# Yubo-Shankui/Bind-Your-Avatar-Implementation

Measured on AMD Instinct MI355X. Metric: denoise-steps/sec, higher is better.
Workload: dtype bf16; 1 GPU; BASELINE.json configs[1]: full transformer.forward, 49x480x720 (13x30x45 latent tokens + 226 text), 2 characters (2 ID + 2 audio), batch 1, random-init 8.6B-param architecture; layers=42, batch=1, launch=eager, parallelism=single GPU

## Files before the change

### bind_your_avatar_implementation_amd/_hip.py

```python
import ctypes
import os

from .build import LIB_PATH as _BUILT_LIB

LIB_PATH = os.environ.get("BYA_HIP_LIB") or _BUILT_LIB

_c = ctypes
_vp, _i32, _i64, _f32 = _c.c_void_p, _c.c_int32, _c.c_int64, _c.c_float


class GemmDesc(_c.Structure):
    _fields_ = [("M", _i32), ("N", _i32), ("K", _i32), ("batch", _i32),
                ("lda", _i32), ("ldw", _i32), ("ldc", _i32), ("ldres", _i32),
                ("a_batch_stride", _i64), ("c_batch_stride", _i64), ("res_batch_stride", _i64),
                ("gate_batch_stride", _i64), ("gate_split", _i32), ("act", _i32),
                ("n_split", _i32), ("c_split_stride", _i64), ("bias_rowscale", _vp), ("alpha", _f32)]


class GemmPlan(_c.Structure):
    _fields_ = [("path", _i32), ("m0", _i32), ("tail", _i32), ("split_k", _i32), ("row_chunks", _i32)]


class QkNormDesc(_c.Structure):
    _fields_ = [("qw", _vp), ("qb", _vp), ("kw", _vp), ("kb", _vp), ("cos", _vp), ("sin", _vp),
                ("text_rows", _i32), ("width", _i32), ("eps", _f32), ("k_scale", _f32)]


MX_KERNEL_FP6 = 16


class MxGemmCall(_c.Structure):
    _fields_ = [("A", _vp), ("a_scales", _vp), ("W", _vp), ("w_scales", _vp), ("bias", _vp), ("C", _vp),
                ("res", _vp), ("gate0", _vp), ("gate1", _vp), ("q_scales", _vp), ("norm", _c.POINTER(QkNormDesc)),
                ("a_fmt", _i32), ("w_fmt", _i32), ("out_fmt", _i32), ("kernel", _i32)]


class AttnDesc(_c.Structure):
    _fields_ = [("head_dim", _i32), ("heads", _i32), ("nb1", _i32), ("nb2", _i32), ("Sq", _i32), ("Skv", _i32),
                ("q_s1", _i64), ("q_s2", _i64), ("q_row", _i64),
                ("k_s1", _i64), ("k_s2", _i64), ("k_row", _i64),
                ("v_s1", _i64), ("v_s2", _i64), ("v_row", _i64),
                ("o_s1", _i64), ("o_s2", _i64), ("o_row", _i64),
                ("scale", _f32), ("scores_prescaled", _i32), ("score_bound", _f32),
                ("bound_dev", _vp), ("bound_slots", _i32), ("bound_heads", _i32), ("bound_bh0", _i32), ("fallback_flags", _vp)]


class AttnMixDesc(_c.Structure):
    _fields_ = [("head_dim", _i32), ("heads", _i32), ("n_id", _i32), ("n_grp", _i32), ("Sq", _i32), ("Skv", _i32),
                ("q_grp", _i64), ("q_row", _i64), ("k_id", _i64), ("k_grp", _i64), ("k_row", _i64),
                ("v_id", _i64), ("v_grp", _i64), ("v_row", _i64), ("z_grp", _i64), ("z_row", _i64), ("scale", _f32)]


class AttnPlan(_c.Structure):
    _fields_ = [("variant", _i32), ("grid", _i32), ("q_tile", _i32), ("stream_k", _i32), ("sk_rem", _i32), ("sk_cut", _i32),
                ("o_wide", _i32), ("second_launch", _i32)]


class AttnMixPlan(_c.Structure):
    _fields_ = [("form", _i32), ("head_dim", _i32), ("grid", _i32), ("row_chunks", _i32), ("lds_bytes", _i32), ("big_lds", _i32)]


class AttnTinyPlan(_c.Structure):
    _fields_ = [("instance", _i32), ("grid", _i32), ("waves", _i64)]


class RowGemmPlan(_c.Structure):
    _fields_ = [("form", _i32), ("ln", _i32), ("res", _i32), ("act", _i32), ("grid", _i32), ("crosses_row_block", _i32),
                ("work_items", _i64)]


class GroupAttnPlan(_c.Structure):
    _fields_ = [("P", _i32), ("G", _i32), ("wide", _i32), ("blocks", _i32), ("tiles", _i64)]


class LayerNormPlan(_c.Structure):
    _fields_ = [("kernel", _i32), ("vec", _i32), ("nv", _i32), ("modulated", _i32), ("rows_per_wave", _i32), ("grid", _i32),
                ("waves", _i64)]


class QkNormRopePlan(_c.Structure):
    _fields_ = [("stats", _i32), ("only", _i32), ("grid", _i32), ("slots", _i32), ("pairs", _i64), ("waves", _i64)]


class RouterChainPlan(_c.Structure):
    _fields_ = [("tiles", _i32), ("tp0", _i32), ("grid", _i32), ("passes", _i32), ("tiles_last", _i32), ("wgs_last", _i32)]


class StepPlan(_c.Structure):
    _fields_ = [("kernel", _i32), ("grid", _i32), ("rounds", _i32), ("reserved", _i32), ("items", _i64), ("items_per_round", _i64)]


class SchedCoef(_c.Structure):
    _fields_ = [("guidance", _f32), ("sqrt_alpha", _f32), ("sqrt_beta", _f32), ("k_sample", _f32),
                ("k_denoised", _f32), ("k_noise", _f32), ("k_cur", _f32), ("k_old", _f32)]


SIGNATURES = {
    "bya_abi_version": [],
    "bya_set_option": [_i32, _i32],
    "bya_get_option": [_i32, _c.POINTER(_i32)],
    "bya_mfma_calibration": [_vp, _i64, _vp, _i32, _vp],
    "bya_gemm_bf16": [_vp, _vp, _vp, _vp, _vp, _vp, _vp, _c.POINTER(GemmDesc), _vp],
    "bya_gemm_skinny_bf16": [_vp, _vp, _vp, _vp, _vp, _c.POINTER(GemmDesc), _vp],
    "bya_gemm_qkv_norm_rope": [_vp, _vp, _vp, _vp, _c.POINTER(GemmDesc), _c.POINTER(QkNormDesc), _vp],
    "bya_gemm_bf16_plan": [_vp, _vp, _vp, _vp, _vp, _vp, _vp, _c.POINTER(GemmDesc), _c.POINTER(GemmPlan)],
    "bya_gemm_qkv_norm_rope_plan": [_vp, _vp, _vp, _vp, _c.POINTER(GemmDesc), _c.POINTER(QkNormDesc), _c.POINTER(GemmPlan)],
    "bya_set_gemm_workspace": [_vp, _i64],
    "bya_gemm_workspace_bytes": [_c.POINTER(_i64)],
    "bya_gemm_workspace_status": [_c.POINTER(_i32), _vp],
    "bya_quantize_rows_fp8": [_vp, _vp, _vp, _i32, _i32, _i64, _i64, _vp],
    "bya_gemm_fp8": [_vp, _vp, _vp, _vp, _vp, _vp, _vp, _vp, _vp, _c.POINTER(GemmDesc), _vp],
    "bya_gemm_fp8_plan": [_vp, _vp, _vp, _vp, _vp, _vp, _vp, _vp, _vp, _c.POINTER(GemmDesc), _c.POINTER(GemmPlan)],
    "bya_gemm_fp8_qkv_norm_rope": [_vp, _vp, _vp, _vp, _vp, _vp, _c.POINTER(GemmDesc), _c.POINTER(QkNormDesc), _vp],
    "bya_gemm_fp8_qkv_norm_rope_plan": [_vp, _vp, _vp, _vp, _vp, _vp, _c.POINTER(GemmDesc), _c.POINTER(QkNormDesc),
                                        _c.POINTER(GemmPlan)],
    "bya_layernorm_fp8": [_vp, _vp, _vp, _vp, _vp, _vp, _vp, _vp, _vp, _i64, _i32, _i32, _i64, _i64, _i64, _i64, _i64, _i64,
                          _f32, _vp],
    "bya_quantize_mx": [_vp, _vp, _vp, _i32, _i32, _i64, _i32, _vp],
    "bya_layernorm_mx": [_vp, _vp, _vp, _vp, _vp, _vp, _vp, _vp, _vp, _i64, _i32, _i32, _i64, _i64, _i64, _i64, _i64, _i64,
                         _f32, _i32, _vp],
    "bya_gemm_mx": [_vp, _vp, _vp, _vp, _vp, _vp, _vp, _vp, _vp, _c.POINTER(GemmDesc), _i32, _vp],
    "bya_gemm_mx_plan": [_vp, _vp, _vp, _vp, _vp, _vp, _vp, _vp, _vp, _c.POINTER(GemmDesc), _i32, _c.POINTER(GemmPlan)],
    "bya_gemm_mx_mixed": [_vp, _vp, _vp, _vp, _vp, _vp, _vp, _vp, _vp, _c.POINTER(GemmDesc), _i32, _i32, _vp],
    "bya_gemm_mx_mixed_plan": [_vp, _vp, _vp, _vp, _vp, _vp, _vp, _vp, _vp, _c.POINTER(GemmDesc), _i32, _i32,
                               _c.POINTER(GemmPlan)],
    "bya_gemm_mx_quant": [_vp, _vp, _vp, _vp, _vp, _vp, _vp, _c.POINTER(GemmDesc), _i32, _i32, _i32, _vp],
    "bya_gemm_mx_quant_plan": [_vp, _vp, _vp, _vp, _vp, _vp, _vp, _c.POINTER(GemmDesc), _i32, _i32, _i32,
                               _c.POINTER(GemmPlan)],
    "bya_gemm_mx_qkv_norm_rope": [_vp, _vp, _vp, _vp, _vp, _vp, _i32, _i32, _c.POINTER(GemmDesc), _c.POINTER(QkNormDesc), _vp],
    "bya_gemm_mx_qkv_norm_rope_plan": [_vp, _vp, _vp, _vp, _vp, _vp, _i32, _i32, _c.POINTER(GemmDesc), _c.POINTER(QkNormDesc),
                                       _c.POINTER(GemmPlan)],
    "bya_gemm_mx_qkv_norm_rope_on": [_vp, _vp, _vp, _vp, _vp, _vp, _i32, _i32, _c.POINTER(GemmDesc), _c.POINTER(QkNormDesc), _i32,
                                     _vp],
    "bya_gemm_mx_qkv_norm_rope_on_plan": [_vp, _vp, _vp, _vp, _vp, _vp, _i32, _i32, _c.POINTER(GemmDesc), _c.POINTER(QkNormDesc),
                                          _i32, _c.POINTER(GemmPlan)],
    "bya_gemm_mx_call": [_c.POINTER(MxGemmCall), _c.POINTER(GemmDesc), _vp],
    "bya_gemm_mx_call_plan": [_c.POINTER(MxGemmCall), _c.POINTER(GemmDesc), _c.POINTER(GemmPlan)],
    "bya_linear_small_m": [_vp, _vp, _vp, _vp, _i32, _i32, _i32, _i32, _i32, _vp],
    "bya_linear_small_m_plan": [_vp, _vp, _vp, _i32, _i32, _i32, _i32, _c.POINTER(StepPlan)],
    "bya_timestep_features": [_vp, _vp, _i32, _i32, _i32, _f32, _vp],
    "bya_layernorm": [_vp, _vp, _vp, _vp, _vp, _vp, _vp, _vp, _i64, _i32, _i32, _i64, _i64, _i64, _i64, _i64, _i64,
                      _f32, _vp],
    "bya_layernorm_plan": [_vp, _vp, _vp, _vp, _vp, _vp, _vp, _vp, _i64, _i32, _i32, _i64, _i64, _i64, _i64, _i64, _i64,
                           _i32, _c.POINTER(LayerNormPlan)],
    "bya_qknorm_rope_plan": [_vp, _vp, _vp, _vp, _vp, _vp, _vp, _vp, _i32, _i32, _i32, _i64, _i64, _i32, _vp, _i32,
                             _c.POINTER(QkNormRopePlan)],
    "bya_qknorm_rope": [_vp, _vp, _vp, _vp, _vp, _vp, _vp, _vp, _i32, _i32, _i32, _i64, _i64, _i32, _f32, _f32, _vp, _i32, _vp],
    "bya_attn_fwd": [_vp, _vp, _vp, _vp, _c.POINTER(AttnDesc), _vp],
    "bya_attn_variant": [_c.POINTER(AttnDesc)],
    "bya_attn_plan": [_c.POINTER(AttnDesc), _vp, _i32, _c.POINTER(AttnPlan)],
    "bya_attn_fwd_mx": [_vp, _vp, _vp, _vp, _vp, _c.POINTER(AttnDesc), _i32, _i64, _i64, _i64, _i64, _i64, _i64, _vp],
    "bya_attn_mx_plan": [_c.POINTER(AttnDesc), _vp, _vp, _i32, _i64, _i64, _i64, _i64, _i64, _i64, _i32, _c.POINTER(AttnPlan)],
    "bya_set_attn_workspace": [_vp, _i64],
    "bya_attn_workspace_bytes": [_c.POINTER(_i64)],
    "bya_attn_workspace_status": [_c.POINTER(_i32), _vp],
    "bya_attn_kv_mix": [_vp, _vp, _vp, _vp, _vp, _vp, _vp, _c.POINTER(AttnMixDesc), _vp],
    "bya_attn_kv_mix_plan": [_vp, _vp, _c.POINTER(AttnMixDesc), _c.POINTER(AttnMixPlan)],
    "bya_attn_kv_mix_mx": [_vp, _vp, _vp, _vp, _vp, _vp, _vp, _vp, _c.POINTER(AttnMixDesc), _i32, _i64, _i64, _i64, _i64, _vp],
    "bya_attn_kv_mix_mx_plan": [_vp, _vp, _vp, _c.POINTER(AttnMixDesc), _i32, _i64, _i64, _i64, _i64, _c.POINTER(AttnMixPlan)],
    "bya_attn_tiny": [_vp, _vp, _vp, _vp, _i32, _i32, _i64, _i64, _i64, _i64, _i64, _i64, _f32, _vp],
    "bya_attn_tiny_plan": [_vp, _vp, _vp, _vp, _i32, _i32, _i64, _i64, _i64, _i64, _c.POINTER(AttnTinyPlan)],
    "bya_router_scores": [_vp, _vp, _vp, _vp, _vp, _vp, _i32, _i64, _i32, _i32, _f32, _vp],
    "bya_router_scores_plan": [_vp, _vp, _vp, _vp, _vp, _vp, _i32, _i64, _i32, _i32, _c.POINTER(StepPlan)],
    "bya_router_head": [_vp, _vp, _vp, _vp, _i32, _i64, _i32, _vp],
    "bya_forcing_max_over_frames": [_vp, _vp, _i32, _i64, _i32, _vp],
    "bya_masked_combine": [_vp, _vp, _vp, _vp, _i32, _f32, _i32, _i32, _i64, _i32, _i64, _i64, _i64, _vp],
    "bya_routed_mix": [_vp, _vp, _vp, _vp, _vp, _i32, _i32, _i32, _i64, _i32, _i64, _vp],
    "bya_patchify": [_vp, _vp, _i32, _i32, _i32, _i32, _i32, _vp],
    "bya_unpatchify": [_vp, _vp, _i32, _i32, _i32, _i32, _i32, _vp],
    "bya_act_add": [_vp, _vp, _vp, _i64, _i32, _vp],
    "bya_act_add_plan": [_vp, _vp, _vp, _i64, _i32, _c.POINTER(StepPlan)],
    "bya_rowgemm512": [_vp, _vp, _vp, _vp, _vp, _vp, _i32, _i32, _i32, _i32, _i32, _i32, _f32, _i32, _i32, _vp],
    "bya_rowgemm512_plan": [_vp, _vp, _vp, _vp, _vp, _vp, _i32, _i32, _i32, _i32, _i32, _i32, _i32, _c.POINTER(RowGemmPlan)],
    "bya_router_group_attn_plan": [_vp, _vp, _vp, _vp, _vp, _i32, _i32, _i32, _i32, _i64, _i64, _i64, _i64,
                                   _c.POINTER(GroupAttnPlan)],
    "bya_router_mlp_fused_plan": [_vp, _vp, _vp, _vp, _vp, _vp, _vp, _i32, _i32, _i32, _i32, _c.POINTER(RouterChainPlan)],
    "bya_router_group_attn_out_plan": [_vp, _vp, _vp, _vp, _vp, _vp, _vp, _i32, _i32, _i32, _i32, _i64, _i64, _i64, _i64, _i32,
                                       _c.POINTER(RouterChainPlan)],
    "bya_router_group_attn": [_vp, _vp, _vp, _vp, _vp, _i32, _i32, _i32, _i32, _i64, _i64, _i64, _i64, _f32, _f32, _vp],
    "bya_router_mlp_fused": [_vp, _vp, _vp, _vp, _vp, _vp, _vp, _i32, _i32, _i32, _f32, _i32, _vp],
    "bya_router_group_attn_out": [_vp, _vp, _vp, _vp, _vp, _vp, _vp, _i32, _i32, _i32, _i32, _i64, _i64, _i64, _i64, _f32, _f32,
                                  _i32, _vp],
    "bya_masks_to_routing_logits": [_vp, _vp, _i32, _i32, _i32, _i32, _i32, _i32, _i32, _vp],
    "bya_vae_patches": [_vp, _vp, _vp] + [_i32] * 14 + [_vp],
    "bya_vae_groupnorm_stats": [_vp, _vp, _vp, _i64, _i32, _i32, _vp],
    "bya_vae_norm_act": [_vp, _vp, _vp, _vp, _vp, _vp, _vp, _i64, _i32, _i32, _i32, _f32, _i32, _i32, _i32, _i32, _i32, _i32,
                         _i32, _i64, _i32, _vp],
    "bya_vae_conv3d": [_vp, _vp, _vp, _vp, _vp, _i32, _i32, _i32, _i32, _i32, _i32, _i64, _i64, _i64, _vp],
    "bya_vae_upsample_pad": [_vp, _vp, _i32, _i32, _i32, _i32, _i32, _vp],
    "bya_allgather_kv": [_vp, _vp, _vp, _vp, _i64, _i64, _vp, _vp],
    "bya_alltoall_router": [_vp, _vp, _vp, _vp, _i32, _vp, _vp],
    "bya_p2p_push": [_vp, _i32, _i64, _vp, _i32, _i32, _vp, _vp],
    "bya_p2p_wait": [_vp, _i32, _vp, _i64, _vp],
    "bya_p2p_exchange": [_vp, _i32, _i64, _vp, _i32, _i32, _vp, _vp, _i64, _vp],
    "bya_p2p_poison": [_vp, _i32, _vp, _i64, _vp],
    "bya_p2p_alloc": [_i64, _i32, _c.POINTER(_vp)],
    "bya_p2p_free": [_vp],
    "bya_p2p_ipc_export": [_vp, _vp],
    "bya_p2p_ipc_import": [_vp, _c.POINTER(_vp)],
    "bya_p2p_ipc_release": [_vp],
    "bya_cfg_scheduler_step": [_vp, _i32, _i64, _vp, _vp, _vp, _vp, _vp, _i64, _c.POINTER(SchedCoef), _vp],
    "bya_cfg_scheduler_step_plan": [_vp, _i32, _i64, _vp, _vp, _i64, _c.POINTER(SchedCoef), _c.POINTER(StepPlan)],
}

OPTIONS = {"gemm_splitk": 0, "gemm_splitk_min": 1, "gemm_tile": 2, "gemm_variant": 3, "attn_streamk": 4, "fp8_kernel": 5,
           "p2p_groups": 6, "reference_forms": 7, "mx_kernel": 8}
REFERENCE_FORMS = {"rowgemm_chunked": 1, "kv_mix_generic": 2, "ln_generic": 4, "router_scores_wave": 8, "attn_narrow_store": 16}
def _named_value(var, v, table):
    if v not in table:
        raise ValueError(f"{var}={v!r}: expected one of {sorted(table)}")
    return table[v]


ENV_OPTIONS = {
    "BYA_GEMM_SPLITK": ("gemm_splitk", int),
    "BYA_GEMM_SPLITK_MIN": ("gemm_splitk_min", int),
    "BYA_GEMM_TILE": ("gemm_tile", int),
    "BYA_GEMM_VARIANT": ("gemm_variant", lambda v: {"w8": 1, "no128": 2}.get(v, 0)),
    "BYA_ATTN_STREAMK": ("attn_streamk", int),
    "BYA_FP8_KERNEL": ("fp8_kernel", lambda v: 1 if v.startswith("1") else 0),
    "BYA_P2P_GROUPS": ("p2p_groups", int),
    "BYA_MX_KERNEL": ("mx_kernel", lambda v: _named_value("BYA_MX_KERNEL", v, {"0": 0, "1": 1, "p256": 1, "2": 2, "always": 2})),
}

GEMM_PATHS = {0: "t128x64", 1: "t128x128", 2: "t256x128", 3: "t256x256", 4: "p256", 5: "p128", 6: "p128s", 7: "w8_256"}

ATTN_VARIANTS = {0: "d64_running_max", 1: "d64_prescaled_running_max", 2: "d64_static_bound", 3: "d128_running_max",
                 4: "d64_static_bound_w4", 5: "d64_device_bound_w4"}
KV_MIX_FORMS = {0: "mix32", 1: "one_tile"}
TINY_INSTANCES = {0: "tiny8<2>", 1: "tiny8<3>", 2: "tiny8<13>", 3: "tiny8<25>", 4: "generic<2>", 5: "generic<4>",
                  6: "generic<16>", 7: "generic<32>"}

ROWGEMM_FORMS = {0: "chunk_balanced", 1: "w_stationary"}

ROUTER_SCORES_KERNELS = {0: "wave", 1: "lds"}

LN_KERNELS = {0: "generic", 1: "rows"}
LN_OUT_KINDS = {"bf16": 0, "fp8": 1, "mxfp8": 2, "mxfp6": 3}

ERRORS = {-1: "BYA_ERR_SHAPE", -2: "BYA_ERR_ALIGN", -3: "BYA_ERR_LAUNCH", -4: "BYA_ERR_UNSUPPORTED"}

_lib = None


def load():
    global _lib
    if _lib is not None:
        return _lib
    import torch
    if not os.path.exists(LIB_PATH):
        raise RuntimeError(
            f"{LIB_PATH} is missing: the Bind-Your-Avatar MI355X engine has no fallback path. "
            "Build it with `python -m bind_your_avatar_implementation_amd.build`.")
    lib = ctypes.CDLL(LIB_PATH)
    for name, argtypes in SIGNATURES.items():
        fn = getattr(lib, name)
        fn.argtypes = argtypes
        fn.restype = _i32
    _lib = lib
    apply_env_options()
    return lib


def set_option(name, value):
    check(load().bya_set_option(OPTIONS[name], int(value)), f"bya_set_option({name}={value})")


def get_option(name):
    v = _i32(0)
    check(load().bya_get_option(OPTIONS[name], _c.byref(v)), f"bya_get_option({name})")
    return v.value


OPTION_DEFAULTS = {"gemm_splitk": 0, "gemm_splitk_min": 0, "gemm_tile": -1, "gemm_variant": 0, "attn_streamk": 1, "fp8_kernel": 0,
                   "p2p_groups": 0, "reference_forms": 0, "mx_kernel": 0}


def apply_env_options():
    for var, (name, parse) in ENV_OPTIONS.items():
        v = os.environ.get(var)
        set_option(name, parse(v) if v not in (None, "") else OPTION_DEFAULTS[name])


class ByaError(RuntimeError):
    pass


def check(rc, what):
    if rc != 0:
        raise ByaError(f"{what} failed: {ERRORS.get(rc, rc)}")
```

### bind_your_avatar_implementation_amd/csrc/attn.hip

```cpp
#include "attn_common.h"
#include "attn_mix32.h"
#include "gemm_persistent.h"
#include "routing_weights.h"
#include <stdlib.h>
#include "options.h"

namespace {

constexpr int ATTN_RING = 2;
constexpr int Q_PER_WAVE = 32;
constexpr int Q_PER_BLOCK = 128;

template <int D, bool IS_V>
__device__ __forceinline__ void stage_kv(const bf16_t* __restrict__ src, long long row_stride, int kv0, int kv_max,
                                         char* lds_tile, int wave, int lane) {
    constexpr int ROW_BYTES = D * 2;
    constexpr int ROWS_PER_INSTR = 1024 / ROW_BYTES;
    constexpr int CHUNKS = ROW_BYTES / 16;
    constexpr int INSTR_PER_WAVE = (KV_TILE / ROWS_PER_INSTR) / 4;
#pragma unroll
    for (int q = 0; q < INSTR_PER_WAVE; ++q) {
        const int rbase = (wave * INSTR_PER_WAVE + q) * ROWS_PER_INSTR;
        const int rl = rbase + lane / CHUNKS;
        const int slot = lane % CHUNKS;
// ... 204 lines not shown
            asm volatile("s_barrier" ::: "memory");
            if (t + 2 < ntiles) stage(t + 2);
        } else {
        asm volatile("s_waitcnt vmcnt(0)" ::: "memory");
        __syncthreads();
        if (t + 1 < ntiles && (!(BYA_ATTN_ABLATE & 8) || t == 0)) stage(t + 1);
        }
        const char* kt = smem + slot * 2 * TILE_BYTES;
        uint32_t vbase[DT];
#pragma unroll
        for (int d = 0; d < DT; ++d) vbase[d] = lds0 + slot * 2 * TILE_BYTES + TILE_BYTES + voff[d];
        slot = (slot + 1 == RING) ? 0 : slot + 1;
        int tz = t;
#if defined(__HIP_DEVICE_COMPILE__)
        asm volatile("" : "+s"(tz));
#endif
        attn_tile<D, false, PRESCALED, BOUNDED>(kt, vbase, qf, oacc, ones, mfrag, m_run, l_run, tz == 0, KV_TILE, r, hf,
                                                BOUNDED ? p.score_bound : p.scale_log2);
    }
    if (nfull < ntiles) {
        asm volatile("s_waitcnt vmcnt(0)" ::: "memory");
        __syncthreads();
        const char* kt = smem + slot * 2 * TILE_BYTES;
        uint32_t vbase[DT];
#pragma unroll
        for (int d = 0; d < DT; ++d) vbase[d] = lds0 + slot * 2 * TILE_BYTES + TILE_BYTES + voff[d];
        attn_tile<D, true, PRESCALED, BOUNDED>(kt, vbase, qf, oacc, ones, mfrag, m_run, l_run, nfull == 0,
                                               p.Skv - nfull * KV_TILE, r, hf, BOUNDED ? p.score_bound : p.scale_log2);
    }

    const auto lsw = __builtin_amdgcn_permlane32_swap(__float_as_uint(l_run), __float_as_uint(l_run), false, false);
    const float l_tot = __uint_as_float(lsw[0]) + __uint_as_float(lsw[1]);
    const float inv = 1.0f / l_tot;
    if constexpr (MX) {
        static_assert(D == 64, "one MX block per 32-column tile, two per head");
        const long long row = q_valid ? q0 + r : 0;
        uint8_t* crow = reinterpret_cast<uint8_t*>(p.o) + b1 * p.o_s1 + b2 * p.o_s2 + row * p.o_row + (long long)head * 2 * mx_block_bytes(mx->fmt);
        uint8_t* srow = mx->scales + b1 * mx->s1 + b2 * mx->s2 + row * mx->row + 2 * head;
        if (mx->fmt == MX_E4M3) store_mx_head<MX_E4M3>(crow, srow, oacc[0], oacc[1], inv, hf, q_valid);
        else store_mx_head<MX_E2M3>(crow, srow, oacc[0], oacc[1], inv, hf, q_valid);
    } else {
    bf16_t* orow = O + (long long)(q_valid ? q0 + r : 0) * p.o_row;
#pragma unroll
    for (int d = 0; d < DT; ++d) store_o_tile(orow + d * 32, oacc[d], inv, hf, q_valid, p.o_wide != 0);
    }
}

template <int D>
__device__ __forceinline__ void attn_mix_body(const MixArgs& p, char* smem) {
    constexpr int ROW_BYTES = D * 2, TILE_BYTES = KV_TILE * ROW_BYTES, DSTEPS = D / 16, DT = D / 32;
    const int tid = threadIdx.x, lane = tid & 63;
    const int wave = __builtin_amdgcn_readfirstlane(tid >> 6);
    const int r = lane & 31, hf = lane >> 5;
    int bid = blockIdx.x;
    const int qt = bid % p.nqt; bid /= p.nqt;
    const int head = bid % p.heads;
    const int grp = bid / p.heads;
    const bf16_t* Q = p.q + grp * p.q_grp + (long long)head * D;
    bf16_t* Z = p.z + grp * p.z_grp + (long long)head * D;
    const int q0 = qt * Q_PER_BLOCK + wave * Q_PER_WAVE;
    int qrow = q0 + r;
    const bool q_valid = qrow < p.Sq;
    qrow = q_valid ? qrow : p.Sq - 1;
    bf16x8 qf[DSTEPS];
#pragma unroll
    for (int s = 0; s < DSTEPS; ++s)
        qf[s] = __builtin_bit_cast(bf16x8, *reinterpret_cast<const u32x4*>(Q + (long long)qrow * p.q_row + s * 16 + hf * 8));
    float w[4];
    routing_weights_of(p.mode, p.n_id, p.af, p.r + ((long long)grp * p.Sq + qrow) * p.n_id, w);
    if (p.wsum && head == 0 && hf == 0 && q_valid) {
        float ws = 0.f;
        for (int i = 0; i < p.n_id; ++i) ws += w[i];
        p.wsum[(long long)grp * p.Sq + qrow] = ws;
    }

    const int g = lane >> 4, li = lane & 15, tq = li >> 2, tp = li & 3;
    uint32_t voff[DT];
#pragma unroll
    for (int d = 0; d < DT; ++d) {
        const int row = 4 * hf + tq;
        const int chunk = 4 * d + 2 * (g & 1) + (tp >> 1);
        voff[d] = row * ROW_BYTES + ((chunk ^ vswz<D>(row)) << 4) + (tp & 1) * 8;
    }
    const uint32_t lds0 = (uint32_t)(uintptr_t)LDS_PTR(smem);
    bf16x8 ones;
#pragma unroll
    for (int e = 0; e < 8; ++e) ones[e] = (__bf16)((hf == 0 && e < 2) ? 1.0f : 0.0f);

    f32x16 zacc[DT];
#pragma unroll
    for (int d = 0; d < DT; ++d)
#pragma unroll
        for (int i = 0; i < 16; ++i) zacc[d][i] = 0.f;
    for (int id = 0; id < p.n_id; ++id) {
        char* st = smem + (id & 1) * 2 * TILE_BYTES;
        auto stage_id = [&](int j) {
            char* dst = smem + (j & 1) * 2 * TILE_BYTES;
            stage_kv<D, false>(p.k + j * p.k_id + grp * p.k_grp + (long long)head * D, p.k_row, 0, p.Skv - 1, dst, wave, lane);
            stage_kv<D, true>(p.v + j * p.v_id + grp * p.v_grp + (long long)head * D, p.v_row, 0, p.Skv - 1, dst + TILE_BYTES, wave, lane);
        };
        if (id == 0) {
            stage_id(0);
            if (p.n_id > 1) stage_id(1);
        }
        if (id != 1) {
            asm volatile("s_waitcnt vmcnt(0)" ::: "memory");
            __syncthreads();
        }
        if (id >= 1 && id + 1 < p.n_id) {
            if (id == 1) __syncthreads();
            stage_id(id + 1);
        }
        f32x16 oacc[DT];
#pragma unroll
        for (int d = 0; d < DT; ++d)
#pragma unroll
            for (int i = 0; i < 16; ++i) oacc[d][i] = 0.f;
        bf16x8 mfrag;
#pragma unroll
        for (int e = 0; e < 8; ++e) mfrag[e] = (__bf16)0.0f;
        float m_run = 0.f, l_run = 0.f;
        uint32_t vbase[DT];
#pragma unroll
        for (int d = 0; d < DT; ++d) vbase[d] = lds0 + (id & 1) * 2 * TILE_BYTES + TILE_BYTES + voff[d];
        attn_tile<D, true, false>(st, vbase, qf, oacc, ones, mfrag, m_run, l_run, true, p.Skv, r, hf, p.scale_log2);
        const auto lsw = __builtin_amdgcn_permlane32_swap(__float_as_uint(l_run), __float_as_uint(l_run), false, false);
        const float sc = w[id] / (__uint_as_float(lsw[0]) + __uint_as_float(lsw[1]));
#pragma unroll
        for (int d = 0; d < DT; ++d)
#pragma unroll
            for (int i = 0; i < 16; ++i) zacc[d][i] = fmaf(sc, oacc[d][i], zacc[d][i]);
    }
    if (q_valid) {
        bf16_t* zrow = Z + (long long)(q0 + r) * p.z_row;
#pragma unroll
        for (int d = 0; d < DT; ++d)
#pragma unroll
            for (int gq = 0; gq < 4; ++gq) {
                u32x2 o;
                o[0] = pack2bf(zacc[d][gq * 4 + 0], zacc[d][gq * 4 + 1]);
                o[1] = pack2bf(zacc[d][gq * 4 + 2], zacc[d][gq * 4 + 3]);
                *reinterpret_cast<u32x2*>(zrow + d * 32 + gq * 8 + hf * 4) = o;
            }
    }
}

__global__ __launch_bounds__(256, 2) void attn_kv_mix32_kernel_d64(MixArgs p) {
    extern __shared__ __attribute__((aligned(16))) char smem[];
    attn_mix32_body<64>(p, smem);
}
__global__ __launch_bounds__(256) void attn_kv_mix32_kernel_d128(MixArgs p) {
    extern __shared__ __attribute__((aligned(16))) char smem[];
    attn_mix32_body<128>(p, smem);
}

__global__ __launch_bounds__(256, 2) void attn_kv_mix_kernel_d64(MixArgs p) {
    extern __shared__ __attribute__((aligned(16))) char smem[];
    attn_mix_body<64>(p, smem);
}
__global__ __launch_bounds__(256) void attn_kv_mix_kernel_d128(MixArgs p) {
    extern __shared__ __attribute__((aligned(16))) char smem[];
    attn_mix_body<128>(p, smem);
}


__global__ __launch_bounds__(256, 4) void attn_fwd_kernel_d64(AttnArgs p) {
    extern __shared__ __attribute__((aligned(16))) char smem[];
    attn_fwd_body<64, false>(p, smem);
}
__global__ __launch_bounds__(256, 4) void attn_fwd_kernel_d64_prescaled(AttnArgs p) {
    extern __shared__ __attribute__((aligned(16))) char smem[];
    attn_fwd_body<64, true>(p, smem);
}
template <bool PRESCALED>
__global__ __launch_bounds__(256, 4) void attn_fwd_mx_kernel_d64(AttnMxArgs pm) {
    extern __shared__ __attribute__((aligned(16))) char smem[];
    attn_fwd_body<64, PRESCALED, false, true>(pm.a, smem, &pm.mx);
}
__global__ __launch_bounds__(256) void attn_fwd_kernel_d128(AttnArgs p) {
    extern __shared__ __attribute__((aligned(16))) char smem[];
    attn_fwd_body<128, false>(p, smem);
}

inline float static_bound_limit() { return BYA_ATTN_BOUND_LIMIT; }

inline int attn_variant_of(const bya_attn_desc* d) {
    if (d->head_dim == 128) return d->scores_prescaled ? BYA_ERR_UNSUPPORTED : BYA_ATTN_D128;
    if (d->head_dim != 64) return BYA_ERR_UNSUPPORTED;
    if (!d->scores_prescaled) return BYA_ATTN_D64_RUNNING_MAX;
    if (d->bound_dev && d->fallback_flags) return BYA_ATTN_D64_DEVICE_BOUND_W4;
    if (!(d->score_bound > 0.f && d->score_bound <= static_bound_limit())) return BYA_ATTN_D64_PRESCALED;
    return BYA_ATTN_D64_STATIC_BOUND_W4;
}

int attn_args_of(const void* q, const void* k, const void* v, void* o, const bya_attn_desc* d, AttnArgs& a) {
    if (!q || !k || !v || !o || !d) return BYA_ERR_SHAPE;
    if (d->head_dim != 64 && d->head_dim != 128) return BYA_ERR_UNSUPPORTED;
    if (d->heads <= 0 || d->nb1 <= 0 || d->nb2 <= 0 || d->Sq <= 0 || d->Skv <= 0) return BYA_ERR_SHAPE;
    if ((d->q_row | d->k_row | d->v_row | d->q_s1 | d->q_s2 | d->k_s1 | d->k_s2 | d->v_s1 | d->v_s2) % 8) return BYA_ERR_ALIGN;
    if ((d->o_row | d->o_s1 | d->o_s2) % 4) return BYA_ERR_ALIGN;
    if (((uintptr_t)q | (uintptr_t)k | (uintptr_t)v) & 15) return BYA_ERR_ALIGN;
    if ((uintptr_t)o & 7) return BYA_ERR_ALIGN;
    a.q = (const bf16_t*)q; a.k = (const bf16_t*)k; a.v = (const bf16_t*)v; a.o = (bf16_t*)o;
    a.heads = d->heads; a.nb1 = d->nb1; a.nb2 = d->nb2; a.Sq = d->Sq; a.Skv = d->Skv;
    a.nqt = (d->Sq + Q_PER_BLOCK - 1) / Q_PER_BLOCK;
    a.q_s1 = d->q_s1; a.q_s2 = d->q_s2; a.q_row = d->q_row;
    a.k_s1 = d->k_s1; a.k_s2 = d->k_s2; a.k_row = d->k_row;
    a.v_s1 = d->v_s1; a.v_s2 = d->v_s2; a.v_row = d->v_row;
    a.o_s1 = d->o_s1; a.o_s2 = d->o_s2; a.o_row = d->o_row;
    a.o_wide = !((uintptr_t)o & 15) && (d->o_s1 | d->o_s2 | d->o_row) % 8 == 0 && !bya_ref_form(BYA_REF_ATTN_NARROW_STORE);
    a.scale_log2 = d->scale * 1.4426950408889634f;
    a.prescaled = d->scores_prescaled;
    if (a.prescaled && d->head_dim != 64) return BYA_ERR_UNSUPPORTED;
    a.score_bound = (a.prescaled && d->score_bound > 0.f && d->score_bound <= static_bound_limit()) ? d->score_bound : 0.f;
    a.sk_part = nullptr; a.sk_flags = nullptr;
    a.bound_dev = nullptr; a.bound_slots = 0; a.bound_heads = 0; a.bound_bh0 = 0; a.bound_limit = BYA_ATTN_BOUND_LIMIT;
    a.fallback = nullptr; a.only_flagged = nullptr;
    if (d->bound_dev && a.prescaled) {
        if (!d->fallback_flags || d->bound_slots < 1 || d->bound_slots > 64 || d->bound_bh0 < 0 ||
            d->bound_bh0 + d->nb1 * d->nb2 * d->heads > d->bound_heads) return BYA_ERR_SHAPE;
        if (((uintptr_t)d->bound_dev | (uintptr_t)d->fallback_flags) & 3) return BYA_ERR_ALIGN;
        a.bound_dev = d->bound_dev; a.bound_slots = d->bound_slots; a.bound_heads = d->bound_heads; a.bound_bh0 = d->bound_bh0;
        a.fallback = d->fallback_flags;
    }
    return BYA_OK;
}

void attn_plan_of(const AttnArgs& a, int D, int ws_present, bya_attn_plan_info* p) {
    const int nbh = a.nb1 * a.nb2 * a.heads;
    p->grid = (nbh * a.nqt + 7) / 8 * 8;
    p->q_tile = Q_PER_BLOCK;
    p->stream_k = 0; p->sk_rem = 0; p->sk_cut = 0;
    p->o_wide = a.o_wide;
    p->second_launch = 0;
    if (D == 128) { p->variant = BYA_ATTN_D128; return; }
    if (!a.prescaled) { p->variant = BYA_ATTN_D64_RUNNING_MAX; return; }
    if (!a.bound_dev && !(a.score_bound > 0.f)) { p->variant = BYA_ATTN_D64_PRESCALED; return; }
    p->variant = a.bound_dev ? BYA_ATTN_D64_DEVICE_BOUND_W4 : BYA_ATTN_D64_STATIC_BOUND_W4;
    p->second_launch = a.bound_dev ? 1 : 0;
    bya_attn_w4_plan w;
    bya_plan_attn_w4(&a, ws_present, &w);
    p->grid = w.grid; p->q_tile = w.q_tile; p->stream_k = w.stream_k; p->sk_rem = w.sk_rem; p->sk_cut = w.sk_cut;
}

template <int D>
int launch_attn(const AttnArgs& a, hipStream_t s) {
    bya_attn_plan_info pl;
    attn_plan_of(a, D, -1, &pl);
    const int nbh = a.nb1 * a.nb2 * a.heads;
    dim3 grid((nbh * a.nqt + 7) / 8 * 8);
    const size_t lds = (size_t)ATTN_RING * 2 * KV_TILE * D * 2;
    switch (pl.variant) {
        case BYA_ATTN_D64_DEVICE_BOUND_W4: {
            const int rc = bya_launch_attn_w4(&a, s);
            if (rc != BYA_OK) return rc;
            AttnArgs b = a;
            b.bound_dev = nullptr; b.score_bound = 0.f; b.only_flagged = a.fallback; b.fallback = nullptr;
            BYA_LAUNCH(attn_fwd_kernel_d64_prescaled, grid, dim3(256), lds, s, b);
            break;
        }
        case BYA_ATTN_D64_STATIC_BOUND_W4: return bya_launch_attn_w4(&a, s);
        case BYA_ATTN_D64_PRESCALED: BYA_LAUNCH(attn_fwd_kernel_d64_prescaled, grid, dim3(256), lds, s, a); break;
        case BYA_ATTN_D64_RUNNING_MAX: BYA_LAUNCH(attn_fwd_kernel_d64, grid, dim3(256), lds, s, a); break;
        default: BYA_LAUNCH(attn_fwd_kernel_d128, grid, dim3(256), lds, s, a); break;
    }
    return hipGetLastError() == hipSuccess ? BYA_OK : BYA_ERR_LAUNCH;
}

int attn_mx_args_of(const void* q, const void* k, const void* v, void* codes, void* scales, const bya_attn_desc* d, int out_fmt,
                    int64_t c_s1, int64_t c_s2, int64_t c_row, int64_t sc_s1, int64_t sc_s2, int64_t sc_row, AttnMxArgs& m) {
    if (!q || !k || !v || !codes || !scales || !d) return BYA_ERR_SHAPE;
    if (d->head_dim != 64) return BYA_ERR_UNSUPPORTED;
    if (out_fmt != MX_E4M3 && out_fmt != MX_E2M3) return BYA_ERR_UNSUPPORTED;
    if (d->o_s1 || d->o_s2 || d->o_row) return BYA_ERR_SHAPE;
    const int rc = attn_args_of(q, k, v, reinterpret_cast<void*>((uintptr_t)16), d, m.a);
    if (rc != BYA_OK) return rc;
    const long long row_bytes = (long long)d->heads * 2 * mx_block_bytes(out_fmt);
    if (c_row < row_bytes || sc_row < 2LL * d->heads || c_s1 < 0 || c_s2 < 0 || sc_s1 < 0 || sc_s2 < 0) return BYA_ERR_SHAPE;
    if (((uintptr_t)codes | (uintptr_t)c_s1 | (uintptr_t)c_s2 | (uintptr_t)c_row) & 3) return BYA_ERR_ALIGN;
    m.a.o = static_cast<bf16_t*>(codes); m.a.o_s1 = c_s1; m.a.o_s2 = c_s2; m.a.o_row = c_row; m.a.o_wide = 0;
    m.mx.scales = static_cast<uint8_t*>(scales); m.mx.s1 = sc_s1; m.mx.s2 = sc_s2; m.mx.row = sc_row; m.mx.fmt = out_fmt;
    return BYA_OK;
}

int launch_attn_mx(const AttnMxArgs& m, int fmt, hipStream_t s) {
    const AttnArgs& a = m.a;
    bya_attn_plan_info pl;
    attn_plan_of(a, 64, -1, &pl);
    const int nbh = a.nb1 * a.nb2 * a.heads;
    const dim3 grid((nbh * a.nqt + 7) / 8 * 8), block(256);
    const size_t lds = (size_t)ATTN_RING * 2 * KV_TILE * 64 * 2;
    auto running = [&](const AttnMxArgs& x, bool prescaled) {
        if (prescaled) BYA_LAUNCH(attn_fwd_mx_kernel_d64<true>, grid, block, lds, s, x);
        else BYA_LAUNCH(attn_fwd_mx_kernel_d64<false>, grid, block, lds, s, x);
    };
    switch (pl.variant) {
        case BYA_ATTN_D64_DEVICE_BOUND_W4: {
            const int rc = bya_launch_attn_w4_mx(&m, fmt, s);
            if (rc != BYA_OK) return rc;
            AttnMxArgs b = m;
            b.a.bound_dev = nullptr; b.a.score_bound = 0.f; b.a.only_flagged = a.fallback; b.a.fallback = nullptr;
            running(b, true);
            break;
        }
        case BYA_ATTN_D64_STATIC_BOUND_W4: return bya_launch_attn_w4_mx(&m, fmt, s);
        case BYA_ATTN_D64_PRESCALED: running(m, true); break;
        case BYA_ATTN_D64_RUNNING_MAX: running(m, false); break;
        default: return BYA_ERR_UNSUPPORTED;
    }
    return hipGetLastError() == hipSuccess ? BYA_OK : BYA_ERR_LAUNCH;
}

int mix_plan_of(const void* z, const bya_attn_mix_desc* d, int has_af, uintptr_t qkv, bya_attn_kv_mix_plan_info* p) {
    if (!z || !d) return BYA_ERR_SHAPE;
    if (d->head_dim != 64 && d->head_dim != 128) return BYA_ERR_UNSUPPORTED;
    if (d->heads <= 0 || d->n_id < 1 || d->n_id > 4 || d->n_grp <= 0 || d->Sq <= 0 || d->Skv <= 0 || d->Skv > KV_TILE) return BYA_ERR_SHAPE;
    if (has_af && d->n_id < 2) return BYA_ERR_SHAPE;
    if ((d->q_grp | d->q_row | d->k_id | d->k_grp | d->k_row | d->v_id | d->v_grp | d->v_row) % 8) return BYA_ERR_ALIGN;
    if ((d->z_grp | d->z_row) % 4) return BYA_ERR_ALIGN;
    if (qkv & 15) return BYA_ERR_ALIGN;
    if ((uintptr_t)z & 7) return BYA_ERR_ALIGN;
    p->head_dim = d->head_dim;
    if (d->Skv <= 32 && !bya_ref_form(BYA_REF_KV_MIX_GENERIC) && !((uintptr_t)z & 15) && (d->z_grp | d->z_row) % 8 == 0) {
        const int n32 = (d->Sq + 31) / 32;
        const int nqc = (n32 + 11) / 12;
        p->form = BYA_KV_MIX_MIX32;
        p->row_chunks = nqc < 1 ? 1 : nqc;
        p->lds_bytes = (d->n_id * 2 + 4) * 32 * d->head_dim * 2;
        p->big_lds = p->lds_bytes > 64 * 1024;
    } else {
        p->form = BYA_KV_MIX_ONE_TILE;
        p->row_chunks = (d->Sq + Q_PER_BLOCK - 1) / Q_PER_BLOCK;
        p->lds_bytes = 2 * 2 * KV_TILE * d->head_dim * 2;
        p->big_lds = 0;
    }
    p->grid = (int32_t)((long long)p->row_chunks * d->heads * d->n_grp);
    return BYA_OK;
}

int mix_mx_plan_of(const void* codes, const void* scales, const bya_attn_mix_desc* d, int has_af, uintptr_t qkv, int out_fmt,
                   int64_t c_grp, int64_t c_row, int64_t sc_grp, int64_t sc_row, bya_attn_kv_mix_plan_info* p) {
    if (!codes || !scales || !d) return BYA_ERR_SHAPE;
    if (out_fmt != MX_E4M3 && out_fmt != MX_E2M3) return BYA_ERR_UNSUPPORTED;
    if (d->z_grp || d->z_row) return BYA_ERR_SHAPE;
    const int rc = mix_plan_of(reinterpret_cast<const void*>((uintptr_t)16), d, has_af, qkv, p);
    if (rc != BYA_OK) return rc;
    if (p->form != BYA_KV_MIX_MIX32) return BYA_ERR_UNSUPPORTED;
    const long long blocks = (long long)d->heads * d->head_dim / 32;
    if (((uintptr_t)codes | (uintptr_t)c_grp | (uintptr_t)c_row) & 3) return BYA_ERR_ALIGN;
    if (c_row < blocks * mx_block_bytes(out_fmt) || sc_row < blocks || c_grp < 0 || sc_grp < 0) return BYA_ERR_SHAPE;
    return BYA_OK;
}

}

extern "C" int bya_attn_variant(const bya_attn_desc* d) {
    if (!d) return BYA_ERR_SHAPE;
    return attn_variant_of(d);
}

extern "C" int bya_attn_plan(const bya_attn_desc* d, const void* o, int32_t workspace_assumed, bya_attn_plan_info* plan) {
    if (!plan) return BYA_ERR_SHAPE;
    AttnArgs a;
    const void* const aligned = reinterpret_cast<const void*>((uintptr_t)16);
    const int rc = attn_args_of(aligned, aligned, aligned, const_cast<void*>(o), d, a);
    if (rc != BYA_OK) return rc;
    attn_plan_of(a, d->head_dim, workspace_assumed, plan);
    return BYA_OK;
}

extern "C" int bya_attn_fwd(const void* q, const void* k, const void* v, void* o, const bya_attn_desc* d,
                            hipStream_t stream) {
    AttnArgs a;
    const int rc = attn_args_of(q, k, v, o, d, a);
    if (rc != BYA_OK) return rc;
    return d->head_dim == 64 ? launch_attn<64>(a, stream) : launch_attn<128>(a, stream);
}

extern "C" int bya_attn_mx_plan(const bya_attn_desc* d, const void* codes, const void* scales, int32_t out_fmt, int64_t c_s1,
                               int64_t c_s2, int64_t c_row, int64_t sc_s1, int64_t sc_s2, int64_t sc_row,
                               int32_t workspace_assumed, bya_attn_plan_info* plan) {
    if (!plan) return BYA_ERR_SHAPE;
    AttnMxArgs m;
    const void* const aligned = reinterpret_cast<const void*>((uintptr_t)16);
    const int rc = attn_mx_args_of(aligned, aligned, aligned, const_cast<void*>(codes), const_cast<void*>(scales), d, out_fmt,
                                   c_s1, c_s2, c_row, sc_s1, sc_s2, sc_row, m);
    if (rc != BYA_OK) return rc;
    attn_plan_of(m.a, 64, workspace_assumed, plan);
    return BYA_OK;
}

extern "C" int bya_attn_fwd_mx(const void* q, const void* k, const void* v, void* codes, void* scales, const bya_attn_desc* d,
                              int32_t out_fmt, int64_t c_s1, int64_t c_s2, int64_t c_row, int64_t sc_s1, int64_t sc_s2,
                              int64_t sc_row, hipStream_t stream) {
    AttnMxArgs m;
    const int rc = attn_mx_args_of(q, k, v, codes, scales, d, out_fmt, c_s1, c_s2, c_row, sc_s1, sc_s2, sc_row, m);
    if (rc != BYA_OK) return rc;
    return launch_attn_mx(m, out_fmt, stream);
}

extern "C" int bya_attn_kv_mix_plan(const void* z, const void* af, const bya_attn_mix_desc* d, bya_attn_kv_mix_plan_info* plan) {
    if (!plan) return BYA_ERR_SHAPE;
    bya_attn_kv_mix_plan_info p;
    const int rc = mix_plan_of(z, d, af != nullptr, 0, &p);
    if (rc == BYA_OK) *plan = p;
    return rc;
}

extern "C" int bya_attn_kv_mix(const void* q, const void* k, const void* v, const void* r, const void* af, void* z, float* wsum,
                               const bya_attn_mix_desc* d, hipStream_t stream) {
    if (!q || !k || !v || !r || !z || !d) return BYA_ERR_SHAPE;
    bya_attn_kv_mix_plan_info pl;
    const int prc = mix_plan_of(z, d, af != nullptr, (uintptr_t)q | (uintptr_t)k | (uintptr_t)v, &pl);
    if (prc != BYA_OK) return prc;
    MixArgs a;
    mix_args_of(q, k, v, r, af, wsum, d, pl.row_chunks, a);
    a.z = (bf16_t*)z; a.z_grp = d->z_grp; a.z_row = d->z_row;
    const dim3 grid((unsigned)pl.grid);
    const size_t lds = (size_t)pl.lds_bytes;
    if (pl.form == BYA_KV_MIX_MIX32) {
        if (pl.big_lds) {
            static std::atomic<unsigned long long> big64{0}, big128{0};
            const int rc = d->head_dim == 64
                ? bya_allow_big_lds(reinterpret_cast<const void*>(attn_kv_mix32_kernel_d64), 160 * 1024, big64)
                : bya_allow_big_lds(reinterpret_cast<const void*>(attn_kv_mix32_kernel_d128), 160 * 1024, big128);
            if (rc != BYA_OK) return rc;
        }
        if (d->head_dim == 64) BYA_LAUNCH(attn_kv_mix32_kernel_d64, grid, dim3(256), lds, stream, a);
        else BYA_LAUNCH(attn_kv_mix32_kernel_d128, grid, dim3(256), lds, stream, a);
        return hipGetLastError() == hipSuccess ? BYA_OK : BYA_ERR_LAUNCH;
    }
    if (d->head_dim == 64) BYA_LAUNCH(attn_kv_mix_kernel_d64, grid, dim3(256), lds, stream, a);
    else BYA_LAUNCH(attn_kv_mix_kernel_d128, grid, dim3(256), lds, stream, a);
    return hipGetLastError() == hipSuccess ? BYA_OK : BYA_ERR_LAUNCH;
}

extern "C" int bya_attn_kv_mix_mx_plan(const void* codes, const void* scales, const void* af, const bya_attn_mix_desc* d,
                                      int32_t out_fmt, int64_t c_grp, int64_t c_row, int64_t sc_grp, int64_t sc_row,
                                      bya_attn_kv_mix_plan_info* plan) {
    if (!plan) return BYA_ERR_SHAPE;
    bya_attn_kv_mix_plan_info p;
    const int rc = mix_mx_plan_of(codes, scales, d, af != nullptr, 0, out_fmt, c_grp, c_row, sc_grp, sc_row, &p);
    if (rc == BYA_OK) *plan = p;
    return rc;
}

extern "C" int bya_attn_kv_mix_mx(const void* q, const void* k, const void* v, const void* r, const void* af, void* codes,
                                  void* scales, float* wsum, const bya_attn_mix_desc* d, int32_t out_fmt, int64_t c_grp,
                                  int64_t c_row, int64_t sc_grp, int64_t sc_row, hipStream_t stream) {
    if (!q || !k || !v || !r) return BYA_ERR_SHAPE;
    bya_attn_kv_mix_plan_info pl;
    const int prc = mix_mx_plan_of(codes, scales, d, af != nullptr, (uintptr_t)q | (uintptr_t)k | (uintptr_t)v, out_fmt, c_grp,
                                   c_row, sc_grp, sc_row, &pl);
    if (prc != BYA_OK) return prc;
    ByaMixMxOut out;
    out.codes = static_cast<uint8_t*>(codes); out.scales = static_cast<uint8_t*>(scales);
    out.c_grp = c_grp; out.c_row = c_row; out.s_grp = sc_grp; out.s_row = sc_row; out.fmt = out_fmt;
    return bya_launch_attn_kv_mix32_mx(q, k, v, r, af, wsum, *d, pl, out, stream);
}
```

### bind_your_avatar_implementation_amd/csrc/attn_mix32.h

```cpp
#pragma once
#include "attn_common.h"
#include "routing_weights.h"

struct ByaMixMxOut { uint8_t* codes; uint8_t* scales; long long c_grp, c_row, s_grp, s_row; int fmt; };

namespace {

#ifndef BYA_ATTN_ABLATE
#define BYA_ATTN_ABLATE 0
#endif

template <int OFF>
__device__ __forceinline__ s16x4 lds_tr_read(uint32_t addr) {
    s16x4 v;
    asm volatile("ds_read_b64_tr_b16 %0, %1 offset:%2" : "=v"(v) : "v"(addr), "i"(OFF));
    return v;
}

template <int OFF>
__device__ __forceinline__ bf16x8 lds_read128(uint32_t addr) {
    bf16x8 v;
    asm volatile("ds_read_b128 %0, %1 offset:%2" : "=v"(v) : "v"(addr), "i"(OFF));
    return v;
}

template <int N>
__device__ __forceinline__ void lgkm_wait() {
    asm volatile("s_waitcnt lgkmcnt(%0)" ::"i"(N) : "memory");
    __builtin_amdgcn_sched_barrier(0);
}

template <int D>
struct VFrag {
    s16x4 lo[D / 32], hi[D / 32];
};

template <int D, int KS>
__device__ __forceinline__ void v_issue(VFrag<D>& f, const uint32_t (&vbase)[D / 32]) {
    constexpr int RB = D * 2;
    if ((BYA_ATTN_ABLATE & 4) && KS >= 2) return;
#pragma unroll
    for (int d = 0; d < D / 32; ++d) {
        f.lo[d] = lds_tr_read<KS * 16 * RB>(vbase[d]);
        f.hi[d] = lds_tr_read<KS * 16 * RB + 8 * RB>(vbase[d]);
    }
}

template <int D>
__device__ __forceinline__ void pv_mfma(const VFrag<D>& f, const bf16x8& pf, f32x16 (&oacc)[D / 32]) {
    typedef __attribute__((ext_vector_type(8))) short s16x8;
#pragma unroll
    for (int d = 0; d < D / 32; ++d) {
        const s16x8 both = {f.lo[d][0], f.lo[d][1], f.lo[d][2], f.lo[d][3], f.hi[d][0], f.hi[d][1], f.hi[d][2], f.hi[d][3]};
        oacc[d] = __builtin_amdgcn_mfma_f32_32x32x16_bf16(__builtin_bit_cast(bf16x8, both), pf, oacc[d], 0, 0, 0);
    }
}

struct MixArgs {
    const bf16_t* q; const bf16_t* k; const bf16_t* v; bf16_t* z; const bf16_t* r; const bf16_t* af; float* wsum;
    int heads, n_id, n_grp, Sq, Skv, nqt, mode;
    long long q_grp, q_row, k_id, k_grp, k_row, v_id, v_grp, v_row, z_grp, z_row;
    float scale_log2;
};
struct MixMxArgs { MixArgs a; ByaMixMxOut mx; };

inline void mix_args_of(const void* q, const void* k, const void* v, const void* r, const void* af, float* wsum,
                        const bya_attn_mix_desc* d, int row_chunks, MixArgs& a) {
    a.q = (const bf16_t*)q; a.k = (const bf16_t*)k; a.v = (const bf16_t*)v; a.z = nullptr;
    a.r = (const bf16_t*)r; a.af = (const bf16_t*)af; a.wsum = wsum;
    a.heads = d->heads; a.n_id = d->n_id; a.n_grp = d->n_grp; a.Sq = d->Sq; a.Skv = d->Skv;
    a.nqt = row_chunks; a.mode = af ? 1 : 0;
    a.q_grp = d->q_grp; a.q_row = d->q_row; a.k_id = d->k_id; a.k_grp = d->k_grp; a.k_row = d->k_row;
    a.v_id = d->v_id; a.v_grp = d->v_grp; a.v_row = d->v_row; a.z_grp = 0; a.z_row = 0;
    a.scale_log2 = d->scale * 1.4426950408889634f;
}

template <int D>
__device__ __forceinline__ void stage_kv32(const bf16_t* __restrict__ src, long long row_stride, int kv_max, char* lds_tile,
                                           int wave, int lane, bool is_v) {
    constexpr int ROW_BYTES = D * 2, ROWS_PER_INSTR = 1024 / ROW_BYTES, CHUNKS = ROW_BYTES / 16;
    for (int q = wave; q < 32 / ROWS_PER_INSTR; q += 4) {
        const int rbase = q * ROWS_PER_INSTR;
        const int rl = rbase + lane / CHUNKS;
        const int slot = lane % CHUNKS;
        const int chunk = slot ^ (is_v ? vswz<D>(rl) : kswz<D>(rl));
        const int gr = rl < kv_max ? rl : kv_max;
        const bf16_t* g = src + (long long)gr * row_stride + chunk * 8;
        __builtin_amdgcn_global_load_lds(GLOBAL_PTR(g), LDS_PTR(lds_tile + rbase * ROW_BYTES), 16, 0, 0);
    }
}

template <int D, bool MX = false>
__device__ __forceinline__ void attn_mix32_body(const MixArgs& p, char* smem, const ByaMixMxOut* mx = nullptr) {
    constexpr int ROW_BYTES = D * 2, KV_BYTES = 32 * ROW_BYTES, DSTEPS = D / 16, DT = D / 32;
    const int tid = threadIdx.x, lane = tid & 63;
    const int wave = __builtin_amdgcn_readfirstlane(tid >> 6);
    const int r = lane & 31, hf = lane >> 5;
    int bid = blockIdx.x;
    const int head = bid % p.heads; bid /= p.heads;
    const int chunk = bid % p.nqt;
    const int grp = bid / p.nqt;
    const int n32 = (p.Sq + 31) >> 5;
    const int t0 = (int)((long long)n32 * chunk / p.nqt), t1 = (int)((long long)n32 * (chunk + 1) / p.nqt);
    const bf16_t* Q = p.q + grp * p.q_grp + (long long)head * D;
    bf16_t* Z = nullptr;
    if constexpr (!MX) Z = p.z + grp * p.z_grp + (long long)head * D;

    for (int id = 0; id < p.n_id; ++id) {
        stage_kv32<D>(p.k + id * p.k_id + grp * p.k_grp + (long long)head * D, p.k_row, p.Skv - 1, smem + id * 2 * KV_BYTES,
                      wave, lane, false);
        stage_kv32<D>(p.v + id * p.v_id + grp * p.v_grp + (long long)head * D, p.v_row, p.Skv - 1,
                      smem + id * 2 * KV_BYTES + KV_BYTES, wave, lane, true);
    }
    const int g = lane >> 4, li = lane & 15, tq = li >> 2, tp = li & 3;
    uint32_t voff[DT];
#pragma unroll
    for (int d = 0; d < DT; ++d) {
        const int row = 4 * hf + tq;
        const int ch = 4 * d + 2 * (g & 1) + (tp >> 1);
        voff[d] = row * ROW_BYTES + ((ch ^ vswz<D>(row)) << 4) + (tp & 1) * 8;
    }
    const uint32_t lds0 = (uint32_t)(uintptr_t)LDS_PTR(smem);
    uint32_t koff[DSTEPS];
#pragma unroll
    for (int s = 0; s < DSTEPS; ++s) koff[s] = r * ROW_BYTES + (((2 * s + hf) ^ kswz<D>(r)) << 4);
    const float c = p.scale_log2;
    asm volatile("s_waitcnt vmcnt(0)" ::: "memory");
    __syncthreads();

    for (int t = t0 + wave; t < t1; t += 4) {
        int qrow = t * 32 + r;
        const bool q_valid = qrow < p.Sq;
        qrow = q_valid ? qrow : p.Sq - 1;
        bf16x8 qf[DSTEPS];
#pragma unroll
        for (int s = 0; s < DSTEPS; ++s)
            qf[s] = __builtin_bit_cast(bf16x8, *reinterpret_cast<const u32x4*>(Q + (long long)qrow * p.q_row + s * 16 + hf * 8));
        float w[4];
        routing_weights_of(p.mode, p.n_id, p.af, p.r + ((long long)grp * p.Sq + qrow) * p.n_id, w);
        if (p.wsum && head == 0 && hf == 0 && q_valid) {
            float ws = 0.f;
            for (int i = 0; i < p.n_id; ++i) ws += w[i];
            p.wsum[(long long)grp * p.Sq + qrow] = ws;
        }
        char* zb = smem + p.n_id * 2 * KV_BYTES + wave * KV_BYTES;
        constexpr int CHUNKS = ROW_BYTES / 16;
        f32x16 zacc[DT];
        for (int id = 0; id < p.n_id; ++id) {
            const uint32_t kb = lds0 + id * 2 * KV_BYTES, vb = kb + KV_BYTES;
            bf16x8 kf[DSTEPS];
#pragma unroll
            for (int s = 0; s < DSTEPS; ++s) kf[s] = lds_read128<0>(kb + koff[s]);
            f32x16 sacc;
#pragma unroll
            for (int i = 0; i < 16; ++i) sacc[i] = 0.f;
            lgkm_wait<0>();
#pragma unroll
            for (int s = 0; s < DSTEPS; ++s) sacc = __builtin_amdgcn_mfma_f32_32x32x16_bf16(kf[s], qf[s], sacc, 0, 0, 0);
            VFrag<D> fa, fb;
            uint32_t vbase[DT];
#pragma unroll
            for (int d = 0; d < DT; ++d) vbase[d] = vb + voff[d];
            v_issue<D, 0>(fa, vbase);
            v_issue<D, 1>(fb, vbase);
            float mx = -INFINITY;
#pragma unroll
            for (int i = 0; i < 16; ++i) {
                const int kv = (i & 3) + 8 * (i >> 2) + 4 * hf;
                if (kv >= p.Skv) sacc[i] = -INFINITY;
                mx = fmaxf(mx, sacc[i]);
            }
            {
                const auto sw = __builtin_amdgcn_permlane32_swap(__float_as_uint(mx), __float_as_uint(mx), false, false);
                mx = fmaxf(__uint_as_float(sw[0]), __uint_as_float(sw[1]));
            }
            const float m_hi = bf2f(f2bf(mx));
            const float m_lo = bf2f(f2bf(mx - m_hi));
            const float m_new = m_hi + m_lo;
            float psum = 0.f;
            bf16x8 pf[2];
#pragma unroll
            for (int tt = 0; tt < 2; ++tt)
#pragma unroll
                for (int e = 0; e < 8; ++e) {
                    const float pv = __builtin_amdgcn_exp2f((sacc[tt * 8 + e] - m_new) * c);
                    psum += pv;
                    pf[tt][e] = (__bf16)pv;
                }
            const auto lsw = __builtin_amdgcn_permlane32_swap(__float_as_uint(psum), __float_as_uint(psum), false, false);
            const float sc = w[id] / (__uint_as_float(lsw[0]) + __uint_as_float(lsw[1]));
            f32x16 oacc[DT];
#pragma unroll
            for (int d = 0; d < DT; ++d)
#pragma unroll
                for (int i = 0; i < 16; ++i) oacc[d][i] = 0.f;
            lgkm_wait<2 * DT>();
            pv_mfma<D>(fa, pf[0], oacc);
            lgkm_wait<0>();
            pv_mfma<D>(fb, pf[1], oacc);
#pragma unroll
            for (int d = 0; d < DT; ++d)
#pragma unroll
                for (int i = 0; i < 16; ++i) zacc[d][i] = id == 0 ? fmaf(sc, oacc[d][i], 0.f) : fmaf(sc, oacc[d][i], zacc[d][i]);
        }
#pragma unroll
        for (int d = 0; d < DT; ++d)
#pragma unroll
            for (int gq = 0; gq < 4; ++gq) {
                u32x2 o;
                o[0] = pack2bf(zacc[d][gq * 4 + 0], zacc[d][gq * 4 + 1]);
                o[1] = pack2bf(zacc[d][gq * 4 + 2], zacc[d][gq * 4 + 3]);
                *reinterpret_cast<u32x2*>(zb + r * ROW_BYTES + (((4 * d + gq) ^ (r & 7)) << 4) + 8 * hf) = o;
            }
        __builtin_amdgcn_fence(__ATOMIC_RELEASE, "wavefront");
        __builtin_amdgcn_wave_barrier();
        __builtin_amdgcn_fence(__ATOMIC_ACQUIRE, "wavefront");
        if constexpr (MX) {
#pragma nounroll
            for (int j = 0; j < 32 * CHUNKS / 64; ++j) {
                const int idx = j * 64 + lane, row = idx / CHUNKS, ch = idx % CHUNKS;
                float v[8];
                unpack8(*reinterpret_cast<const u32x4*>(zb + row * ROW_BYTES + ((ch ^ (row & 7)) << 4)), v);
                float amax = 0.f;
#pragma unroll
                for (int e = 0; e < 8; ++e) amax = fmaxf(amax, fabsf(v[e]));
                amax = quad_amax(amax);
                if (t * 32 + row < p.Sq) {
                    const long long grow = t * 32 + row;
                    uint8_t* crow = mx->codes + grp * mx->c_grp + grow * mx->c_row;
                    uint32_t sb;
                    if (mx->fmt == MX_E4M3) sb = mx_quant8<MX_E4M3>(v, amax, crow + head * D + 8 * ch);
                    else sb = mx_quant8<MX_E2M3>(v, amax, crow + head * (D * 3 / 4) + 6 * ch);
                    if ((ch & 3) == 0) mx->scales[grp * mx->s_grp + grow * mx->s_row + head * (D / 32) + (ch >> 2)] = (uint8_t)sb;
                }
            }
        } else {
#pragma unroll
        for (int j = 0; j < 32 * CHUNKS / 64; ++j) {
            const int idx = j * 64 + lane, row = idx / CHUNKS, ch = idx % CHUNKS;
            const u32x4 o = *reinterpret_cast<const u32x4*>(zb + row * ROW_BYTES + ((ch ^ (row & 7)) << 4));
            if (t * 32 + row < p.Sq) *reinterpret_cast<u32x4*>(Z + (long long)(t * 32 + row) * p.z_row + ch * 8) = o;
        }
        }
        __builtin_amdgcn_wave_barrier();
    }
}

}

int bya_launch_attn_kv_mix32_mx(const void* q, const void* k, const void* v, const void* r, const void* af, float* wsum,
                                const bya_attn_mix_desc& desc, const bya_attn_kv_mix_plan_info& plan, const ByaMixMxOut& out,
                                hipStream_t stream);
```

### bind_your_avatar_implementation_amd/csrc/router.hip

```cpp
#include "bya_common.h"
#include "../../include/bya.h"
#include <stdlib.h>
#include "options.h"

namespace {

constexpr int R_HEADS = 16, R_TOK = 32, R_HD = 128, R_QK = R_HEADS * R_HD, R_FEAT = R_HEADS * R_TOK;

__global__ __launch_bounds__(256) void router_scores_kernel(const bf16_t* __restrict__ qr, const bf16_t* __restrict__ kr,
                                                            const bf16_t* __restrict__ ln_w, const bf16_t* __restrict__ ln_b,
                                                            const bf16_t* __restrict__ pos, bf16_t* __restrict__ out,
                                                            int n_id, long long N, float eps) {
    const int lane = threadIdx.x & 63;
    const long long tiles = (N + 15) / 16;
    const long long wid = (long long)blockIdx.x * 4 + (threadIdx.x >> 6);
    if (wid >= tiles * n_id) return;
    const int id = (int)(wid / tiles);
    const long long n0 = (wid % tiles) * 16;
    const int c = lane & 15, g = lane >> 4;
    long long n = n0 + c;
    const bool valid = n < N;
    n = valid ? n : N - 1;
    const bf16_t* qrow = qr + n * R_QK + g * 8;
    const bf16_t* krow0 = kr + ((long long)id * R_TOK + c) * R_QK + g * 8;
// ... 152 lines not shown
                for (int h = 0; h < R_HEADS; ++h)
                    o[h] = bf2f(f2bf((acc[h][j][e] - mean) * rstd * wv[h] + bv[h])) + pv[h];
                *reinterpret_cast<u32x4*>(orow + f0) = pack8(o);
                *reinterpret_cast<u32x4*>(orow + f0 + 8) = pack8(o + 8);
            }
    }
}

__global__ __launch_bounds__(256) void router_head_kernel(const bf16_t* __restrict__ x, const bf16_t* __restrict__ w,
                                                          const bf16_t* __restrict__ b, bf16_t* __restrict__ r, int n_id,
                                                          long long N, int D) {
    const int lane = threadIdx.x & 63;
    const long long row = (long long)blockIdx.x * 4 + (threadIdx.x >> 6);
    if (row >= N * n_id) return;
    const int id = (int)(row / N);
    const long long n = row % N;
    float acc = 0.f;
    for (int k0 = lane * 8; k0 < D; k0 += 512) {
        float xv[8], wv[8];
        unpack8(*reinterpret_cast<const u32x4*>(x + row * D + k0), xv);
        unpack8(*reinterpret_cast<const u32x4*>(w + k0), wv);
#pragma unroll
        for (int e = 0; e < 8; ++e) acc += xv[e] * wv[e];
    }
    acc = wave_sum(acc);
    if (lane == 0) {
        const float z = bf2f(f2bf(acc + bf2f(b[0])));
        r[n * n_id + id] = f2bf(1.0f / (1.0f + __expf(-z)));
    }
}

template <int MAXL>
__global__ __launch_bounds__(256) void attn_tiny_kernel(const bf16_t* __restrict__ q, const bf16_t* __restrict__ k,
                                                        const bf16_t* __restrict__ v, bf16_t* __restrict__ o, int L,
                                                        int heads, long long n_outer, long long n_inner,
                                                        long long outer_stride, long long seq_stride, long long ld_qkv,
                                                        long long ld_o, float scale) {
    const int lane = threadIdx.x & 63;
    const long long wid = (long long)blockIdx.x * 4 + (threadIdx.x >> 6);
    const long long total = n_outer * n_inner * heads;
    if (wid >= total) return;
    const int h = (int)(wid % heads);
    const long long gseq = wid / heads;
    const long long row0 = (gseq / n_inner) * outer_stride + (gseq % n_inner);
    float qv[MAXL], kv[MAXL], vv[MAXL];
#pragma unroll
    for (int e = 0; e < MAXL; ++e) {
        if (e < L) {
            const long long row = row0 + e * seq_stride;
            qv[e] = bf2f(q[row * ld_qkv + h * 64 + lane]) * scale;
            kv[e] = bf2f(k[row * ld_qkv + h * 64 + lane]);
            vv[e] = bf2f(v[row * ld_qkv + h * 64 + lane]);
        }
    }
#pragma unroll
    for (int i = 0; i < MAXL; ++i) {
        if (i < L) {
            float s[MAXL];
            float mx = -INFINITY;
#pragma unroll
            for (int j = 0; j < MAXL; ++j) {
                if (j < L) { s[j] = wave_sum(qv[i] * kv[j]); mx = fmaxf(mx, s[j]); }
            }
            float den = 0.f, acc = 0.f;
#pragma unroll
            for (int j = 0; j < MAXL; ++j) {
                if (j < L) { const float pj = __expf(s[j] - mx); den += pj; acc += pj * vv[j]; }
            }
            o[(row0 + i * seq_stride) * ld_o + h * 64 + lane] = f2bf(acc / den);
        }
    }
}


__device__ __forceinline__ float reduce8(float v) {
    int t = __builtin_amdgcn_update_dpp(0, __builtin_bit_cast(int, v), 0xB1, 0xF, 0xF, true);
    v += __builtin_bit_cast(float, t);
    t = __builtin_amdgcn_update_dpp(0, __builtin_bit_cast(int, v), 0x4E, 0xF, 0xF, true);
    v += __builtin_bit_cast(float, t);
    t = __builtin_amdgcn_update_dpp(0, __builtin_bit_cast(int, v), 0x141, 0xF, 0xF, true);
    return v + __builtin_bit_cast(float, t);
}

template <int L>
__global__ __launch_bounds__(256) void attn_tiny8_kernel(const bf16_t* __restrict__ q, const bf16_t* __restrict__ k,
                                                         const bf16_t* __restrict__ v, bf16_t* __restrict__ o,
                                                         int hgroups, long long n_outer, long long n_inner,
                                                         long long outer_stride, long long seq_stride, long long ld_qkv,
                                                         long long ld_o, float scale) {
    const int lane = threadIdx.x & 63;
    const long long wid = (long long)blockIdx.x * 4 + (threadIdx.x >> 6);
    if (wid >= n_outer * n_inner * hgroups) return;
    const int hgrp = (int)(wid % hgroups);
    const long long gseq = wid / hgroups;
    const long long row0 = (gseq / n_inner) * outer_stride + (gseq % n_inner);
    const int col = hgrp * 512 + lane * 8;
    constexpr bool Q_IN_REGS = L <= 16;
    uint32_t kq[L][4], vq[L][4], qq[Q_IN_REGS ? L : 1][4];
#pragma unroll
    for (int e = 0; e < L; ++e) {
        const long long off = (row0 + e * seq_stride) * ld_qkv + col;
        const u32x4 b = *reinterpret_cast<const u32x4*>(k + off);
        const u32x4 c = *reinterpret_cast<const u32x4*>(v + off);
#pragma unroll
        for (int w = 0; w < 4; ++w) { kq[e][w] = b[w]; vq[e][w] = c[w]; }
        if (Q_IN_REGS) {
            const u32x4 a = *reinterpret_cast<const u32x4*>(q + off);
#pragma unroll
            for (int w = 0; w < 4; ++w) qq[e][w] = a[w];
        }
    }
#pragma unroll
    for (int i = 0; i < L; ++i) {
        if (!Q_IN_REGS) {
            const u32x4 a = *reinterpret_cast<const u32x4*>(q + (row0 + i * seq_stride) * ld_qkv + col);
#pragma unroll
            for (int w = 0; w < 4; ++w) qq[0][w] = a[w];
        }
        float s[L];
        float mx = -INFINITY;
#pragma unroll
        for (int j = 0; j < L; ++j) {
            float d = 0.f;
#pragma unroll
            for (int w = 0; w < 4; ++w)
            {
                const uint32_t qa = qq[Q_IN_REGS ? i : 0][w], kb = kq[j][w];
                d = __builtin_amdgcn_fdot2_f32_bf16(__builtin_bit_cast(bf16x2, qa), __builtin_bit_cast(bf16x2, kb), d,
                                                    false);
            }
            s[j] = reduce8(d) * scale;
            mx = fmaxf(mx, s[j]);
        }
        float den = 0.f, acc[8];
#pragma unroll
        for (int e = 0; e < 8; ++e) acc[e] = 0.f;
#pragma unroll
        for (int j = 0; j < L; ++j) {
            const float pj = __expf(s[j] - mx);
            den += pj;
#pragma unroll
            for (int w = 0; w < 4; ++w) {
                acc[2 * w] = fmaf(pj, bflo(vq[j][w]), acc[2 * w]);
                acc[2 * w + 1] = fmaf(pj, bfhi(vq[j][w]), acc[2 * w + 1]);
            }
        }
        const float inv = 1.0f / den;
#pragma unroll
        for (int e = 0; e < 8; ++e) acc[e] *= inv;
        *reinterpret_cast<u32x4*>(o + (row0 + i * seq_stride) * ld_o + col) = pack8(acc);
    }
}

inline int ok() { const hipError_t e = hipGetLastError(); return e == hipSuccess ? BYA_OK : -(1000 + (int)e); }

}

static int scores_plan_of(const void* qr, const void* kr, const void* ln_w, const void* ln_b, const void* pos_emb, const void* out,
                          int32_t n_id, int64_t N, int32_t heads, int32_t face_tokens, bya_step_plan_info* p) {
    if (!qr || !kr || !ln_w || !ln_b || !pos_emb || !out || n_id <= 0 || N <= 0) return BYA_ERR_SHAPE;
    if (heads != R_HEADS || face_tokens != R_TOK) return BYA_ERR_UNSUPPORTED;
    if (((uintptr_t)qr | (uintptr_t)kr | (uintptr_t)ln_w | (uintptr_t)ln_b | (uintptr_t)pos_emb | (uintptr_t)out) & 15)
        return BYA_ERR_ALIGN;
    p->items = (N + 15) / 16;
    p->reserved = 0;
    if (N >= 4096 && n_id <= 256 && !bya_ref_form(BYA_REF_ROUTER_SCORES_WAVE)) {
        p->kernel = BYA_ROUTER_SCORES_LDS;
        p->grid = 256 / n_id * n_id;
        p->items_per_round = (long long)(p->grid / n_id) * 8;
        p->rounds = (int32_t)((p->items + p->items_per_round - 1) / p->items_per_round);
    } else {
        p->kernel = BYA_ROUTER_SCORES_WAVE;
        p->grid = (int32_t)((p->items * n_id + 3) / 4);
        p->items_per_round = p->items;
        p->rounds = 1;
    }
    return BYA_OK;
}

extern "C" int bya_router_scores_plan(const void* qr, const void* kr, const void* ln_w, const void* ln_b, const void* pos_emb,
                                      const void* out, int32_t n_id, int64_t N, int32_t heads, int32_t face_tokens,
                                      bya_step_plan_info* plan) {
    if (!plan) return BYA_ERR_SHAPE;
    bya_step_plan_info p;
    const int rc = scores_plan_of(qr, kr, ln_w, ln_b, pos_emb, out, n_id, N, heads, face_tokens, &p);
    if (rc == BYA_OK) *plan = p;
    return rc;
}

extern "C" int bya_router_scores(const void* qr, const void* kr, const void* ln_w, const void* ln_b,
                                 const void* pos_emb, void* out, int32_t n_id, int64_t N, int32_t heads,
                                 int32_t face_tokens, float eps, hipStream_t stream) {
    bya_step_plan_info pl;
    const int rc = scores_plan_of(qr, kr, ln_w, ln_b, pos_emb, out, n_id, N, heads, face_tokens, &pl);
    if (rc != BYA_OK) return rc;
    if (pl.kernel == BYA_ROUTER_SCORES_LDS) {
        static std::atomic<unsigned long long> big{0};
        if (bya_allow_big_lds(reinterpret_cast<const void*>(router_scores_lds_kernel), 160 * 1024, big) != BYA_OK) return BYA_ERR_LAUNCH;
        BYA_LAUNCH(router_scores_lds_kernel, dim3((unsigned)pl.grid), dim3(512), (size_t)R_TOK * R_QK * 2, stream,
                   (const bf16_t*)qr, (const bf16_t*)kr, (const bf16_t*)ln_w, (const bf16_t*)ln_b,
                   (const bf16_t*)pos_emb, (bf16_t*)out, n_id, (long long)N, eps);
        return ok();
    }
    BYA_LAUNCH(router_scores_kernel, dim3((unsigned)pl.grid), dim3(256), 0, stream,
                       (const bf16_t*)qr, (const bf16_t*)kr, (const bf16_t*)ln_w, (const bf16_t*)ln_b,
                       (const bf16_t*)pos_emb, (bf16_t*)out, n_id, (long long)N, eps);
    return ok();
}

extern "C" int bya_router_head(const void* x, const void* w, const void* b, void* r, int32_t n_id, int64_t N,
                               int32_t D, hipStream_t stream) {
    if (!x || !w || !b || !r || n_id <= 0 || N <= 0 || D <= 0 || D % 512) return BYA_ERR_SHAPE;
    if (((uintptr_t)x | (uintptr_t)w) & 15) return BYA_ERR_ALIGN;
    const long long rows = (long long)N * n_id;
    BYA_LAUNCH(router_head_kernel, dim3((unsigned)((rows + 3) / 4)), dim3(256), 0, stream, (const bf16_t*)x,
                       (const bf16_t*)w, (const bf16_t*)b, (bf16_t*)r, n_id, (long long)N, D);
    return ok();
}

static int tiny_plan_of(const void* q, const void* k, const void* v, const void* o, int32_t L, int32_t heads, int64_t n_outer,
                        int64_t n_inner, int64_t ld_qkv, int64_t ld_o, bya_attn_tiny_plan_info* p) {
    if (!q || !k || !v || !o || L <= 0 || L > 32 || heads <= 0 || n_outer <= 0 || n_inner <= 0) return BYA_ERR_SHAPE;
    if (heads % 8 == 0 && (L == 2 || L == 3 || L == 13 || L == 25) && ld_qkv % 8 == 0 && ld_o % 8 == 0 &&
        !(((uintptr_t)q | (uintptr_t)k | (uintptr_t)v | (uintptr_t)o) & 15)) {
        p->instance = L == 2 ? BYA_TINY8_2 : L == 3 ? BYA_TINY8_3 : L == 13 ? BYA_TINY8_13 : BYA_TINY8_25;
        p->waves = (long long)n_outer * n_inner * (heads / 8);
    } else {
        p->instance = L <= 2 ? BYA_TINY_GENERIC_2 : L <= 4 ? BYA_TINY_GENERIC_4 : L <= 16 ? BYA_TINY_GENERIC_16 : BYA_TINY_GENERIC_32;
        p->waves = (long long)n_outer * n_inner * heads;
    }
    p->grid = (int32_t)((p->waves + 3) / 4);
    return BYA_OK;
}

extern "C" int bya_attn_tiny_plan(const void* q, const void* k, const void* v, const void* o, int32_t L, int32_t heads,
                                  int64_t n_outer, int64_t n_inner, int64_t ld_qkv, int64_t ld_o, bya_attn_tiny_plan_info* plan) {
    if (!plan) return BYA_ERR_SHAPE;
    bya_attn_tiny_plan_info p;
    const int rc = tiny_plan_of(q, k, v, o, L, heads, n_outer, n_inner, ld_qkv, ld_o, &p);
    if (rc == BYA_OK) *plan = p;
    return rc;
}

extern "C" int bya_attn_tiny(const void* q, const void* k, const void* v, void* o, int32_t L, int32_t heads,
                             int64_t n_outer, int64_t n_inner, int64_t outer_stride, int64_t seq_stride,
                             int64_t ld_qkv, int64_t ld_o, float scale, hipStream_t stream) {
    bya_attn_tiny_plan_info pl;
    const int rc = tiny_plan_of(q, k, v, o, L, heads, n_outer, n_inner, ld_qkv, ld_o, &pl);
    if (rc != BYA_OK) return rc;
#define TINY_ARGS (const bf16_t*)q, (const bf16_t*)k, (const bf16_t*)v, (bf16_t*)o
#define TINY_TAIL (long long)n_outer, (long long)n_inner, (long long)outer_stride, (long long)seq_stride, \
                  (long long)ld_qkv, (long long)ld_o, scale
    const dim3 grid((unsigned)pl.grid);
    const int hgroups = heads / 8;
    switch (pl.instance) {
        case BYA_TINY8_2: BYA_LAUNCH((attn_tiny8_kernel<2>), grid, dim3(256), 0, stream, TINY_ARGS, hgroups, TINY_TAIL); break;
        case BYA_TINY8_3: BYA_LAUNCH((attn_tiny8_kernel<3>), grid, dim3(256), 0, stream, TINY_ARGS, hgroups, TINY_TAIL); break;
        case BYA_TINY8_13: BYA_LAUNCH((attn_tiny8_kernel<13>), grid, dim3(256), 0, stream, TINY_ARGS, hgroups, TINY_TAIL); break;
        case BYA_TINY8_25: BYA_LAUNCH((attn_tiny8_kernel<25>), grid, dim3(256), 0, stream, TINY_ARGS, hgroups, TINY_TAIL); break;
        case BYA_TINY_GENERIC_2: BYA_LAUNCH((attn_tiny_kernel<2>), grid, dim3(256), 0, stream, TINY_ARGS, L, heads, TINY_TAIL); break;
        case BYA_TINY_GENERIC_4: BYA_LAUNCH((attn_tiny_kernel<4>), grid, dim3(256), 0, stream, TINY_ARGS, L, heads, TINY_TAIL); break;
        case BYA_TINY_GENERIC_16: BYA_LAUNCH((attn_tiny_kernel<16>), grid, dim3(256), 0, stream, TINY_ARGS, L, heads, TINY_TAIL); break;
        default: BYA_LAUNCH((attn_tiny_kernel<32>), grid, dim3(256), 0, stream, TINY_ARGS, L, heads, TINY_TAIL); break;
    }
#undef TINY_ARGS
#undef TINY_TAIL
    return ok();
}
```

### bind_your_avatar_implementation_amd/engine.py

```python
import contextlib
import os

import torch

from . import ops
from .parallel import RouterPartition, SeqShard


def _key(tensors):
    return tuple((t.data_ptr(), t._version, tuple(t.shape)) for t in tensors)


FP8_LINEARS = ("qkv", "out", "ff1", "ff2", "pq", "aq")
FP8_DEFAULT = ("qkv", "out", "ff1", "ff2")
MX_CROSS_OUT = ("po", "ao")


def _linears_of(keep, allowed, what):
    keep = set(FP8_LINEARS if keep == "all" else keep.split(",")) if isinstance(keep, str) else set(keep)
    unknown = keep - set(allowed)
    if unknown:
        raise ValueError(f"{what} linears {sorted(unknown)}: expected a subset of {allowed}")
    return keep


def fp8_linears_of(model):
    return _linears_of(getattr(model, "_fp8_linears", None) or os.environ.get("BYA_FP8_LINEARS") or FP8_DEFAULT, FP8_LINEARS, "fp8")


def mx_linears_of(model):
    return _linears_of(getattr(model, "_mx_linears", None) or FP8_DEFAULT, FP8_LINEARS + MX_CROSS_OUT, "MX")


def mx_call_kernel(fmt, w_fmt, persistent_gemm, persistent_gemm_mxfp6=False):
    if fmt == "mxfp6" and persistent_gemm_mxfp6:
        return 16 + (2 if persistent_gemm_mxfp6 == "always" else 1)
    if not persistent_gemm or (fmt, w_fmt) != ("mxfp8", "mxfp4"):
        return 0
    return 2 if persistent_gemm == "always" else 1


class DenoiseEngine:
    MAX_ID = 4
    n_id = None

    def _count_ids(self, id_cond, audio_embeds):
        if self.m.is_train_face and id_cond is not None:
            n = len(id_cond)
        elif audio_embeds is not None and audio_embeds.ndim == 5:
            n = audio_embeds.shape[1]
        else:
            n = 2
        if not 2 <= n <= self.MAX_ID:
            raise ValueError(f"{n} identities: the engine runs 2..{self.MAX_ID} (the reference itself exactly 2)")
        return n

    def __init__(self, model):
        p = model.proj_out.weight
        if not p.is_cuda:
            raise RuntimeError("the Bind-Your-Avatar MI355X engine needs its parameters on a GPU "
                               "(there is no CPU fallback); call model.to('cuda')")
        if p.dtype != torch.bfloat16:
            raise RuntimeError(f"engine computes in bf16 (MFMA, fp32 accumulate); parameters are {p.dtype}")
        ops._hip.load()
        ops.ensure_gemm_workspace(p.device)
        self.m = model
        self.cfg = model.config
        self.dev = p.device
        self.D = model.inner_dim
        self.H = self.cfg.num_attention_heads
        self.L = len(model.transformer_blocks)
        self.Tt_max = self.cfg.max_text_seq_length
        self.cache_invariants = False
        self.k_scale = (self.cfg.attention_head_dim ** -0.5) * 1.4426950408889634
        self.mix_before_projection = os.environ.get("BYA_MIX_BEFORE_PROJECTION", "1") != "0"
        self.fused_attn_mix = self.mix_before_projection and os.environ.get("BYA_FUSED_ATTN_MIX", "1") != "0"
        self.fp8_weights = bool(getattr(model, "_fp8_weights", False)) or os.environ.get("BYA_FP8_WEIGHTS") == "1"
        self.fuse_ln_quant = os.environ.get("BYA_FP8_FUSED_LN", "1") != "0"
        self.fp8_fuse_qk_norm = self.fp8_weights and bool(getattr(model, "_fp8_fuse_qk_norm", False))
        self.mx_fmt = getattr(model, "_mx_weights", None)
        self.mx_wfmt = None
        if self.mx_fmt is not None:
            self.mx_wfmt = getattr(model, "_mx_weight_format", None) or self.mx_fmt
            ops.mx_fmt_pair(self.mx_fmt, self.mx_wfmt)
            if self.fp8_weights:
                raise ValueError("fp8 weights (enable_fp8_weights / BYA_FP8_WEIGHTS) and MX weights (enable_mx_weights) "
                                 "are both requested: enable one of them")
        self.mx_fuse_quant = self.mx_fmt is not None and bool(getattr(model, "_mx_fuse_activation_quant", True))
        self.mx_fuse_attn_quant = self.mx_fmt is not None and bool(getattr(model, "_mx_fuse_attention_quant", False))
        self.mx_fuse_qk_norm = self.mx_fmt is not None and bool(getattr(model, "_mx_fuse_qk_norm", False))
        self.mx_fuse_cross_quant = self.mx_fmt is not None and bool(getattr(model, "_mx_fuse_cross_attention_quant", True))
        pg = getattr(model, "_mx_persistent_gemm", False)
        mx8 = self.mx_fmt == "mxfp8" and self.mx_wfmt == "mxfp8"
        self.mx_kernel = (2 if pg == "always" else 1) if (pg and mx8) else 0
        self.mx_call_kernel = mx_call_kernel(self.mx_fmt, self.mx_wfmt, pg, getattr(model, "_mx_persistent_gemm_mxfp6", False))
        self.side_stream_conditioning = os.environ.get("BYA_INVARIANTS_SIDE_STREAM", "1") != "0"
        self.sp_allgather = os.environ.get("BYA_SP_ALLGATHER", "0") == "1"
        self.router_fused_attn = os.environ.get("BYA_ROUTER_FUSED_ATTN", "1") != "0"
        self.router_chain = os.environ.get("BYA_ROUTER_CHAIN", "1")
        self.verify_exchanges = os.environ.get("BYA_SP_VERIFY", "0") == "1"
        self.sp_overlap_v = os.environ.get("BYA_SP_OVERLAP_V", "1") != "0"
        self.sp_shard_mods = os.environ.get("BYA_SP_SHARD_MODS", "1") != "0"
        if os.environ.get("BYA_SP_OVERLAP_V") == "all":
            self.SP_OVERLAP_V_MIN_ROWS = 0
        self.router_replicated = os.environ.get("BYA_ROUTER_REPLICATED", "0") == "1"
        self.qkn_epilogue = os.environ.get("BYA_QKN_EPILOGUE", "1") != "0"
        self._inv_cache = {}
        self._side = None
        self._ws_key, self._ws = None, None
        self._parts = {}
        if model.is_train_audio and not model.is_train_face:
            raise RuntimeError("audio injection needs the face router's logits (models/transformer.py:860)")
        self._pack()

    def _fingerprint(self):
        ptrs = vers = n = 0
        for group in (self.m.parameters(), self.m.buffers()):
            for t in group:
                n += 1
                ptrs += t.data_ptr()
                if not t.is_inference():
                    vers += t._version
        return (n, ptrs, vers)

    def refresh_if_stale(self):
        if self._fingerprint() == self._fp:
            return False
        self._pack()
        self._inv_cache = {}
        self.m._graphs = {}
        return True

    def _pack(self):
        m, D = self.m, self.D
        cat = torch.cat
        self._fp = self._fingerprint()
        self.score_bound = []
        for blk in m.transformer_blocks:
            nq, nk = blk.attn1.norm_q, blk.attn1.norm_k
            bq = 8.0 * nq.weight.float().abs().max().item() + nq.bias.float().norm().item()
            bk = 8.0 * nk.weight.float().abs().max().item() + nk.bias.float().norm().item()
            self.score_bound.append(1.02 * bq * bk * self.k_scale if os.environ.get("BYA_ATTN_BOUNDED", "1") != "0" else 0.0)
        self.device_bound = os.environ.get("BYA_ATTN_DEVICE_BOUND", "1") != "0"
        mods_w, mods_b = [], []
        for blk in m.transformer_blocks:
            for nz in (blk.norm1, blk.norm2):
                mods_w.append(nz.linear.weight)
                mods_b.append(nz.linear.bias)
        mods_w.append(m.norm_out.linear.weight)
        mods_b.append(m.norm_out.linear.bias)
        self.mod_w = cat(mods_w).contiguous()
        self.mod_b = cat(mods_b).contiguous()
        self.patch_w = m.patch_embed.proj.weight.reshape(D, -1)
        self.qkv_w = [cat([b.attn1.to_q.weight, b.attn1.to_k.weight, b.attn1.to_v.weight]).contiguous()
                      for b in m.transformer_blocks]
        self.qkv_b = [cat([b.attn1.to_q.bias, b.attn1.to_k.bias, b.attn1.to_v.bias]).contiguous()
                      for b in m.transformer_blocks]
        self.w8 = None
        blocks = m.transformer_blocks
        source = {"qkv": lambda: self.qkv_w,
                  "out": lambda: [b.attn1.to_out[0].weight for b in blocks],
                  "ff1": lambda: [b.ff.net[0].proj.weight for b in blocks],
                  "ff2": lambda: [b.ff.net[2].weight for b in blocks],
                  "pq": lambda: [pc.to_q.weight for pc in m.perceiver_cross_attention] if m.is_train_face else None,
                  "aq": lambda: [al["attn"].to_q.weight for al in m.audio_model.layers] if m.is_train_audio else None,
                  "po": lambda: [pc.to_out.weight for pc in m.perceiver_cross_attention] if m.is_train_face else None,
                  "ao": lambda: [al["attn"].to_out[0].weight for al in m.audio_model.layers] if m.is_train_audio else None}
        if self.fp8_weights:
            keep = fp8_linears_of(m)
            self.w8 = {}
            for k in FP8_LINEARS:
                ws = source[k]() if k in keep else None
                if ws is not None:
                    self.w8[k] = [ops.quantize_rows_fp8(w) for w in ws]
        self.wmx = None
        if self.mx_fmt is not None:
            keep = mx_linears_of(m)
            self.wmx = {}
            for k in FP8_LINEARS + MX_CROSS_OUT:
                ws = source[k]() if k in keep else None
                if ws is not None:
                    self.wmx[k] = [ops.quantize_mx(w.contiguous(), self.mx_wfmt) for w in ws]
        pe = getattr(m.patch_embed, "pos_embedding", None)
        use_pe = (not self.cfg.use_rotary_positional_embeddings) or self.cfg.use_learned_positional_embeddings
        self.pos_embedding = pe[0] if (pe is not None and use_pe) else None
        if m.is_train_face:
            r = m.router
            qk = r.norm_q.weight.numel()
            hd = qk // r.heads
            j = torch.arange(qk, device=self.dev)
            perm = (j % hd) * r.heads + j // hd
            self.r_nq_w, self.r_nq_b = r.norm_q.weight[perm].contiguous(), r.norm_q.bias[perm].contiguous()
            self.r_nk_w, self.r_nk_b = r.norm_k.weight[perm].contiguous(), r.norm_k.bias[perm].contiguous()
            self.r_to_q = [l.weight[:, perm].contiguous() for l in r.to_q]
            self.r_to_k = [l.weight[:, perm].contiguous() for l in r.to_k]
            self.r_pos = r.pos_emb.reshape(-1, r.feat_dim).contiguous()
            self.r_qkv = []
            for st in r.spatial_temporal_layers:
                packed = {}
                for name in ("spatial_attn", "temporal_attn", "multi_id_attn"):
                    a = getattr(st, name)
                    packed[name] = (cat([a.to_q.weight, a.to_k.weight, a.to_v.weight]).contiguous(),
                                    cat([a.to_q.bias, a.to_k.bias, a.to_v.bias]).contiguous())
                if r.feat_dim == 512 and os.environ.get("BYA_ROUTER_ROWGEMM", "1") != "0":
                    for name, ln in (("spatial_attn", st.norm1), ("temporal_attn", st.norm2), ("multi_id_attn", st.norm3)):
                        a = getattr(st, name)
                        w, b = packed[name]
                        if name == "spatial_attn":
                            c = (64 ** -0.5) * 1.4426950408889634
                            F_ = r.feat_dim
                            w, b = w.float().clone(), b.float().clone()
                            w[F_:2 * F_] *= c
                            b[F_:2 * F_] *= c
                        packed["rg_" + name] = (ops.pack_rowgemm512(w, b, ln.weight, ln.bias), ln.eps,
                                                ops.pack_rowgemm512(a.to_out[0].weight, a.to_out[0].bias))
                    packed["rg_mlp"] = (ops.pack_rowgemm512(st.mlp[0].weight, st.mlp[0].bias, st.norm4.weight, st.norm4.bias),
                                        st.norm4.eps, ops.pack_rowgemm512(st.mlp[2].weight, st.mlp[2].bias))
                self.r_qkv.append(packed)
            self.lfe_proj_t = m.local_facial_extractor.proj_out.t().contiguous()
        if m.is_train_audio:
            cw = m.audio_model.audio_proj_model.conv1.weight
            self.conv_w = cw.permute(0, 2, 1).reshape(cw.shape[0], -1).contiguous()
            att = [l["attn"] for l in m.audio_model.layers]
            self.audio_kv_w = cat([w for a in att for w in (a.to_k.weight, a.to_v.weight)]).contiguous()
            self.audio_kv_b = cat([b for a in att for b in (a.to_k.bias, a.to_v.bias)]).contiguous()

    def _shard(self, rank, world, S, Tt, group):
        key = ("seq", rank, world, S, Tt, id(group))
        sh = self._parts.get(key)
        if sh is None:
            sh = self._parts[key] = SeqShard(rank, world, S, Tt, group, getattr(self.m, "_seq_p2p", None) if group is not None else None)
        return sh

    def _router_partition(self, sh, pairs, per_frame):
        key = ("router", sh.rank, sh.world, pairs, per_frame, id(sh.group))
        rp = self._parts.get(key)
        if rp is None:
            rp = self._parts[key] = RouterPartition(sh.rank, sh.world, pairs, per_frame, sh.group, sh.p2p)
        return rp

    def _buf(self, name, *shape):
        t = self._ws.get(name)
        if t is None or tuple(t.shape) != tuple(shape):
            t = torch.empty(*shape, dtype=torch.bfloat16, device=self.dev)
            self._ws[name] = t
        return t

    def _attn_bound(self, i, n_bh, slots=64):
        wc = self.score_bound[i]
        if wc <= ops.ATTN_BOUND_LIMIT or not self.device_bound or wc == 0.0:
            return wc, None
        key = ("qk_stats", slots, n_bh)
        st = self._ws.get(key)
        if st is None:
            st = self._ws[key] = torch.empty(slots, 2, n_bh, dtype=torch.float32, device=self.dev)
            self._ws["qk_flags"] = torch.zeros(max(n_bh, 64), dtype=torch.int32, device=self.dev)
        st.zero_()
        return 0.0, st

    def _qkv_norm_rope(self, i, at, xn, out, split, xq, cos, sin, text_rows, heads, q_view, k_view, stats):
        fused = self.qkn_epilogue and stats is None and not self._quantised("qkv") and xq is None
        if fused and ops.gemm_qkv_norm_rope(xn, self.qkv_w[i], out, self.qkv_b[i], split, at.norm_q.weight, at.norm_q.bias,
                                            at.norm_k.weight, at.norm_k.bias, cos, sin, text_rows, eps=at.norm_q.eps,
                                            k_scale=self.k_scale):
            return
        if self.mx_fuse_qk_norm and stats is None and xq is not None and self.wmx is not None and "qkv" in self.wmx:
            wc, sw = self.wmx["qkv"][i]
            if self.mx_call_kernel:
                norm = dict(qw=at.norm_q.weight, qb=at.norm_q.bias, kw=at.norm_k.weight, kb=at.norm_k.bias, cos=cos, sin=sin,
                            text_rows=text_rows, eps=at.norm_q.eps, k_scale=self.k_scale)
                if ops.gemm_mx_call(xq[0], xq[1].view(*xn.shape[:-1], -1), wc, sw, out, self.mx_call_kernel, self.mx_fmt,
                                    self.mx_wfmt, bias=self.qkv_b[i], split=split, norm=norm):
                    return
            elif ops.gemm_mx_qkv_norm_rope(xq[0], xq[1].view(*xn.shape[:-1], -1), wc, sw, out, self.qkv_b[i], split,
                                         at.norm_q.weight, at.norm_q.bias, at.norm_k.weight, at.norm_k.bias, cos, sin, text_rows,
                                         eps=at.norm_q.eps, k_scale=self.k_scale, fmt=self.mx_fmt, w_fmt=self.mx_wfmt,
                                         kernel=self.mx_kernel):
                return
        if self.fp8_fuse_qk_norm and stats is None and xq is not None and self.w8 is not None and "qkv" in self.w8:
            w8, sw = self.w8["qkv"][i]
            if ops.gemm_fp8_qkv_norm_rope(xq[0].view(*xn.shape), xq[1].view(*xn.shape[:-1]), w8, sw, out, self.qkv_b[i], split,
                                          at.norm_q.weight, at.norm_q.bias, at.norm_k.weight, at.norm_k.bias, cos, sin,
                                          text_rows, eps=at.norm_q.eps, k_scale=self.k_scale):
                return
        self._dit_linear("qkv", i, xn, self.qkv_w[i], out, bias=self.qkv_b[i], split=split, quantised=xq)
        ops.qknorm_rope(q_view, k_view, at.norm_q.weight, at.norm_q.bias, at.norm_k.weight, at.norm_k.bias, cos, sin,
                        heads=heads, text_rows=text_rows, eps=at.norm_q.eps, k_scale=self.k_scale, stats=stats)

    def _dit_linear(self, which, i, a, w, out, quantised=None, **kw):
        if self.wmx is not None and which in self.wmx:
            if quantised is None:
                quantised = ops.quantize_mx(a, self.mx_fmt, *self._amx(a.shape))
            return self._mx_linear(which, i, quantised, a.shape[:-1], out, **kw)
        if self.w8 is None or which not in self.w8:
            return ops.gemm(a, w, out, **kw)
        if quantised is None:
            quantised = ops.quantize_rows_fp8(a, *self._a8(a.shape))
        a8, sa = quantised
        w8, sw = self.w8[which][i]
        return ops.gemm_fp8(a8.view(*a.shape), sa.view(*a.shape[:-1]), w8, sw, out, **kw)

    def _mx_linear(self, which, i, quantised, lead, out, **kw):
        codes, sa = quantised
        wc, sw = self.wmx[which][i]
        if self.mx_call_kernel:
            return ops.gemm_mx_call(codes, sa.view(*lead, -1), wc, sw, out, self.mx_call_kernel, self.mx_fmt, self.mx_wfmt, **kw)
        with self._mx_kernel_option():
            return ops.gemm_mx(codes, sa.view(*lead, -1), wc, sw, out, self.mx_fmt, w_fmt=self.mx_wfmt, **kw)

    def _cross_out(self, which, i, name, shape, mix, w, out, **kw):
        if self.wmx is None or which not in self.wmx:
            z = self._buf(name, *shape)
            mix(z, None)
            return ops.gemm(z, w, out, **kw)
        zq = self._amx(shape)
        if not (self.mx_fuse_cross_quant and mix(None, zq) is not False):
            z = self._buf(name, *shape)
            mix(z, None)
            zq = ops.quantize_mx(z, self.mx_fmt, *zq)
        return self._mx_linear(which, i, zq, shape[:-1], out, **kw)

    def _mx_kernel_option(self):
        return ops.options(mx_kernel=self.mx_kernel) if self.mx_kernel else contextlib.nullcontext()

    def _ff_pair_fused(self):
        return self.mx_fuse_quant and self.wmx is not None and "ff1" in self.wmx and "ff2" in self.wmx

    def _attn_out_fused(self):
        return self.mx_fuse_attn_quant and self.wmx is not None and "out" in self.wmx

    def _joint_attention(self, q, k, v, out, **kw):
        if not self._attn_out_fused():
            ops.self_attention(q, k, v, out, **kw)
            return None
        return ops.self_attention(q, k, v, None, mx_out=(*self._amx(out.shape), self.mx_fmt), **kw)

    def _ff1_mx_quant(self, i, a, out_shape, bias, quantised=None):
        if quantised is None:
            quantised = ops.quantize_mx(a, self.mx_fmt, *self._amx(a.shape))
        codes, sa = quantised
        wc, sw = self.wmx["ff1"][i]
        oc, osc = self._amx(out_shape)
        if self.mx_call_kernel:
            return ops.gemm_mx_call(codes, sa.view(*a.shape[:-1], -1), wc, sw, oc, self.mx_call_kernel, self.mx_fmt, self.mx_wfmt,
                                    out_scales=osc, out_fmt=self.mx_fmt, bias=bias, act="gelu_tanh")
        with self._mx_kernel_option():
            return ops.gemm_mx_quant(codes, sa.view(*a.shape[:-1], -1), wc, sw, oc, osc, self.mx_fmt, w_fmt=self.mx_wfmt,
                                     out_fmt=self.mx_fmt, bias=bias, act="gelu_tanh")

    def _ln_linear(self, which, i, x, xn, norm, w, out, **kw):
        if self._quantised(which) and self.fuse_ln_quant:
            xq = self._layernorm_quant(which, x, xn.shape, norm.weight, norm.bias, eps=norm.eps)
            return self._dit_linear(which, i, xn, w, out, quantised=xq, **kw)
        ops.layernorm(x, xn, norm.weight, norm.bias, eps=norm.eps)
        return self._dit_linear(which, i, xn, w, out, **kw)

    def _quantised(self, which):
        return (self.w8 is not None and which in self.w8) or (self.wmx is not None and which in self.wmx)

    def _layernorm_quant(self, which, x, shape, weight, bias, **kw):
        if self.wmx is not None and which in self.wmx:
            return ops.layernorm_mx(x, *self._amx(shape), self.mx_fmt, weight, bias, **kw)
        return ops.layernorm_fp8(x, *self._a8(shape), weight, bias, **kw)

    def _amx(self, shape):
        key = ("amx", self.mx_fmt, tuple(shape))
        hold = self._ws.get(key)
        if hold is None:
            hold = self._ws[key] = (torch.empty(*shape[:-1], ops.mx_code_bytes(shape[-1], self.mx_fmt), dtype=torch.uint8,
                                                device=self.dev),
                                    torch.empty(*shape[:-1], shape[-1] // 32, dtype=torch.uint8, device=self.dev))
        return hold

    def _a8(self, shape):
        key = ("a8", tuple(shape))
        hold = self._ws.get(key)
        if hold is None:
            hold = self._ws[key] = (torch.empty(*shape, dtype=torch.uint8, device=self.dev),
                                    torch.empty(*shape[:-1], dtype=torch.float32, device=self.dev))
        return hold

    def _linear(self, x, lin_w, lin_b, out, act=None, res=None):
        if x.dim() == 2 and x.shape[0] <= 8 and res is None and act in (None, "silu") and x.is_contiguous() \
                and out.is_contiguous():
            return ops.linear_small_m(x, lin_w, lin_b, out, act_out=act)
        return ops.gemm(x, lin_w, out, bias=lin_b, act=act, res=res)

    @staticmethod
    def _ln(x, out, ln, eps=None):
        return ops.layernorm(x, out, ln.weight, ln.bias, eps=ln.eps if eps is None else eps)

    def _bf(self, t):
        return t.to(device=self.dev, dtype=torch.bfloat16).contiguous()

    def _face_invariants(self, id_cond, id_vit_hidden, B, n_id, after_layer=None):
        with ops.weight_streaming():
            return self._face_invariants_body(id_cond, id_vit_hidden, B, n_id, after_layer)

    def _face_invariants_body(self, id_cond, id_vit_hidden, B, n_id, after_layer=None):
        m = self.m
        lfe = m.local_facial_extractor
        G, dim = n_id * B, lfe.dim
        nq, nt = lfe.num_queries, lfe.num_id_token
        idc = self._bf(torch.cat([id_cond[i] for i in range(n_id)], 0))
        vit = [self._bf(torch.cat([id_vit_hidden[i][k] for i in range(n_id)], 0)) for k in range(5)]
        n_vit = vit[0].shape[1]
        E = lambda *s: torch.empty(*s, dtype=torch.bfloat16, device=self.dev)

        def mapper(seq, x, out_last):
            h = x
            for a, b in ((0, 1), (3, 4)):
                t = E(*h.shape[:-1], seq[a].weight.shape[0])
                self._linear(h, seq[a].weight, seq[a].bias, t)
                self._ln(t, t, seq[b])
                ops.act_add(t, t, act="leaky_relu")
                h = t
            return self._linear(h, seq[6].weight, seq[6].bias, out_last)

        x_tok = mapper(lfe.id_embedding_mapping, idc, E(G, nt * dim)).view(G, nt, dim)
        lat = E(G, nq + nt, dim)
        lat[:, :nq] = lfe.latents.to(torch.bfloat16)
        lat[:, nq:] = x_tok
        n_ctx, n_lat = nt + n_vit, nq + nt
        ctx = E(G, n_ctx, dim)
        ctx[:, :nt] = x_tok
        kvin = E(G, n_ctx + n_lat, dim)
        inner = lfe.heads * lfe.dim_head
        q, kv = E(G, n_lat, inner), E(G, n_ctx + n_lat, 2 * inner)
        ao, f = E(G, n_lat, inner), E(G, n_lat, dim)
        hid = E(G, n_lat, lfe.layers[0][1][1].weight.shape[0])
        for lvl in range(5):
            mapper(getattr(lfe, f"mapping_{lvl}"), vit[lvl], ctx[:, nt:])
            for attn, ff in lfe.layers[lvl * lfe.depth:(lvl + 1) * lfe.depth]:
                self._ln(ctx, kvin[:, :n_ctx], attn.norm1)
                self._ln(lat, kvin[:, n_ctx:], attn.norm2)
                ops.gemm(kvin[:, n_ctx:], attn.to_q.weight, q)
                ops.gemm(kvin, attn.to_kv.weight, kv)
                ops.self_attention(q, kv[:, :, :inner], kv[:, :, inner:], ao, heads=lfe.heads,
                                   head_dim=lfe.dim_head)
                ops.gemm(ao, attn.to_out.weight, lat, res=lat)
                self._ln(lat, f, ff[0])
                ops.gemm(f, ff[1].weight, hid, act="gelu_erf")
                ops.gemm(hid, ff[3].weight, lat, res=lat)
        face_all = E(G, nq, self.lfe_proj_t.shape[0])
        ops.gemm(lat[:, :nq], self.lfe_proj_t, face_all)
        face = face_all.view(n_id, B, nq, -1).transpose(0, 1).contiguous()
        self.last_face_emb = face

        kvs, krs = [], []
        face2d = face.view(B * n_id * nq, -1)
        fn = E(*face2d.shape)
        for l, pc in enumerate(m.perceiver_cross_attention):
            self._ln(face2d, fn, pc.norm1)
            kv_l = E(B * n_id * nq, pc.to_kv.weight.shape[0])
            ops.gemm(fn.view(B * n_id, nq, -1), pc.to_kv.weight, kv_l.view(B * n_id, nq, -1))
            inner_p = pc.to_q.weight.shape[0]
            kn = E(B * n_id * nq, inner_p)
            ops.layernorm(kv_l[:, :inner_p], kn, self.r_nk_w, self.r_nk_b, eps=m.router.norm_k.eps)
            kr_l = E(B * n_id * nq, inner_p)
            ops.gemm(kn.view(B * n_id, nq, -1), self.r_to_k[l], kr_l.view(B * n_id, nq, -1))
            kvs.append(kv_l.view(B, n_id, nq, -1))
            krs.append(kr_l.view(B, n_id, nq, -1))
            if after_layer is not None:
                after_layer(l)
        return kvs, krs

    def _audio_invariants(self, audio_embeds, T, B, n_id):
        with ops.weight_streaming():
            return self._audio_invariants_body(audio_embeds, T, B, n_id)

    def _audio_invariants_body(self, audio_embeds, T, B, n_id):
        am = self.m.audio_model
        ap = am.audio_proj_model
        mono = audio_embeds.dim() == 4
        if mono:
            mute = am.mute_audio_embeds
            if mute is None:
                mute = torch.load("tests/input/ae_mute.pt")
            mute = self._bf(mute[:T * 4 + 1].to(self.dev))
            if mute.shape != audio_embeds.shape[1:]:
                raise AssertionError(f"cur_audio_context_tokens.shape: {tuple(audio_embeds.shape[1:])} frames x blocks x "
                                     f"channels, mute_context_tokens.shape: {tuple(mute.shape)}")
            audio_embeds = torch.stack([self._bf(audio_embeds), mute.unsqueeze(0).expand_as(audio_embeds)], dim=1)
        a = self._bf(audio_embeds).contiguous()
        bs, ni, F, blk, ch = a.shape
        assert bs == B and ni == n_id
        assert 1 + (T - 1) * 4 + (am.window_size - am.window_stride) == F, \
            f"hidden_states_num_frames: {T}, window_size: {am.window_size}, window_stride: {am.window_stride}, " \
            f"audio_embeds.shape[1]: {F}"
        G, per = B * n_id, blk * ch
        nwin = F - am.window_size + 1
        E = lambda *s: torch.empty(*s, dtype=torch.bfloat16, device=self.dev)
        win = torch.as_strided(a, (G, nwin, am.window_size * per), (F * per, per, 1))
        h1, h2 = E(G, nwin, ap.proj1.weight.shape[0]), E(G, nwin, ap.proj2.weight.shape[0])
        ops.gemm(win, ap.proj1.weight, h1, bias=ap.proj1.bias, act="relu")
        ops.gemm(h1, ap.proj2.weight, h2, bias=ap.proj2.bias, act="relu")
        C = ap.proj3.weight.shape[0]
        cur = E(G, nwin, C)
        ops.gemm(h2, ap.proj3.weight, cur, bias=ap.proj3.bias)
        for _ in range(2):
            n = cur.shape[1]
            keep = n % 2
            n_out = (n - keep) // 2
            nxt = E(G, keep + n_out, C)
            if keep:
                nxt[:, 0] = cur[:, 0]
            if n_out > 0:
                pairs = torch.as_strided(cur, (G, n_out, 2 * C), (n * C, 2 * C, 1), cur.storage_offset() + keep * C)
                ops.gemm(pairs, self.conv_w, nxt[:, keep:], bias=ap.conv1.bias)
            cur = nxt
        assert cur.shape[1] == T
        tok = ap.context_tokens
        ctx = E(G * T * tok, ap.output_dim)
        self._ln(cur.view(G * T * tok, ap.output_dim), ctx, ap.norm)
        if mono:
            ctx.view(B, n_id, T, tok, ap.output_dim)[:, 1] += am.mute_learnable_tokens.view(1, 1, tok, ap.output_dim)
        self.last_audio_ctx = ctx.view(B, n_id, T, tok, ap.output_dim)
        rows, inner = G * T * tok, am.layers[0]["attn"].to_k.weight.shape[0]
        kv = E(2 * len(am.layers), rows, inner)
        ops.gemm(ctx, self.audio_kv_w, kv[0], bias=self.audio_kv_b, split=(inner, rows * inner))
        ks = [kv[2 * l].view(B, n_id, T, tok, -1) for l in range(len(am.layers))]
        vs = [kv[2 * l + 1].view(B, n_id, T, tok, -1) for l in range(len(am.layers))]
        return ks, vs

    def _cached(self, name, tensors, fn):
        if not self.cache_invariants:
            return fn()
        key = _key(tensors)
        hit = self._inv_cache.get(name)
        if hit is not None and hit[0] == key:
            return hit[2]
        val = fn()
        self._inv_cache[name] = (key, list(tensors), val)
        return val

    @torch.no_grad()
    def precompute(self, id_cond=None, id_vit_hidden=None, audio_embeds=None, latent_frames=13):
        self.cache_invariants = True
        self._inv_cache = {}
        n_id = self._count_ids(id_cond, audio_embeds)
        if self.m.is_train_face and id_cond is not None:
            B = id_cond[0].shape[0]
            flat = list(id_cond[:n_id]) + [t for i in range(n_id) for t in id_vit_hidden[i]]
            self._cached("face", flat, lambda: self._face_invariants(id_cond, id_vit_hidden, B, n_id))
        if self.m.is_train_audio and audio_embeds is not None:
            self._cached("audio", [audio_embeds],
                         lambda: self._audio_invariants(audio_embeds, latent_frames, audio_embeds.shape[0], n_id))
        return self

    def release(self):
        self.cache_invariants = False
        self._inv_cache = {}

    @torch.no_grad()
    def step(self, *args, **kwargs):
        self.refresh_if_stale()
        with ops.pinned_stream():
            return self._step(*args, **kwargs)

    def _step(self, hidden_states, encoder_hidden_states, timestep, image_rotary_emb, id_cond, id_vit_hidden,
              audio_embeds, af_matrix, routing_logits_forcing, taps=None):
        n_id = self.n_id = self._count_ids(id_cond, audio_embeds)
        m, cfg, D, H = self.m, self.cfg, self.D, self.H
        B, T, C, Hh, Ww = hidden_states.shape
        ht, wt = Hh // 2, Ww // 2
        per_frame, N = ht * wt, T * ht * wt
        Tt = encoder_hidden_states.shape[1]
        S = Tt + N
        sh = self._shard(getattr(m, "_seq_rank", 0), getattr(m, "_seq_world", 1), S, Tt, getattr(m, "_seq_group", None))
        if sh.active and B != 1:
            raise NotImplementedError("sequence-parallel execution shards ONE sample; split a CFG batch over rank groups")
        S_loc, Tt_loc, N_loc, v0, v1 = sh.S_loc, sh.Tt_loc, sh.N_loc, sh.v0, sh.v1
        key = (B, T, C, Hh, Ww, Tt, sh.rank, sh.world, n_id)
        if self._ws_key != key:
            self._ws_key, self._ws = key, {}
            if sh.p2p is not None:
                sh.p2p.drop_tables()
        sh.begin_step()
        buf = self._buf
        hs = self._bf(hidden_states)
        enc_in = self._bf(encoder_hidden_states)
        if not torch.is_tensor(timestep):
            timestep = torch.tensor([timestep] * B)
        ts = timestep.to(device=self.dev, dtype=torch.int64).reshape(-1)
        if ts.numel() == 1 and B > 1:
            ts = ts.expand(B)
        ts = ts.contiguous()
        use_face = m.is_train_face
        use_audio = m.is_train_audio and audio_embeds is not None
        if use_face and m.router.frames * m.router.height * m.router.width != N:
            raise ValueError(f"router positional table is {m.router.frames}x{m.router.height}x{m.router.width} "
                             f"but the latents give {T}x{wt}x{ht} tokens")
        cos = sin = None
        if image_rotary_emb is not None:
            cos = image_rotary_emb[0].to(device=self.dev, dtype=torch.float32)[v0:v1].contiguous()
            sin = image_rotary_emb[1].to(device=self.dev, dtype=torch.float32)[v0:v1].contiguous()

        inv_side, face_marks, audio_mark = None, {}, [None]
        if (use_face or use_audio) and ops._TIMERS is None and self.side_stream_conditioning:
            if self._side is None:
                self._side = torch.cuda.Stream(self.dev)
            inv_side = ops.on_stream(self._side)
        with (inv_side if inv_side is not None else contextlib.nullcontext()):
            audio_res = []

            def audio_now():
                if use_audio and not audio_res:
                    audio_res.append(self._cached("audio", [audio_embeds], lambda: self._audio_invariants(audio_embeds, T, B, n_id)))
                    if inv_side is not None:
                        audio_mark[0] = inv_side.mark()

            def after_face_layer(l):
                if inv_side is not None:
                    face_marks[l] = inv_side.mark()
                if l == 0:
                    audio_now()
            if use_face:
                flat_face = list(id_cond[:n_id]) + [t for i in range(n_id) for t in id_vit_hidden[i]]
                face_kv, router_k = self._cached("face", flat_face,
                                                 lambda: self._face_invariants(id_cond, id_vit_hidden, B, n_id, after_face_layer))
            audio_now()
            if use_audio:
                audio_k, audio_v = audio_res[0]
        if use_audio:
            af = self._bf(af_matrix)
        forced = None
        if routing_logits_forcing is not None and use_face:
            f_in = self._bf(routing_logits_forcing).reshape(T, per_frame, n_id)
            forced = ops.forcing_max_over_frames(f_in, buf("forced", 1, N, n_id).view(T, per_frame, n_id), T, per_frame,
                                                 n_id).view(1, N, n_id)[:, v0:v1].contiguous()

        tfeat = ops.timestep_features(ts, buf("tfeat", B, D), cfg.flip_sin_to_cos, float(cfg.freq_shift))
        te = m.time_embedding
        e1 = ops.linear_small_m(tfeat, te.linear_1.weight, te.linear_1.bias, buf("e1", B, te.linear_1.weight.shape[0]),
                                act_out="silu")
        emb = ops.linear_small_m(e1, te.linear_2.weight, te.linear_2.bias, buf("emb", B, te.linear_2.weight.shape[0]))
        Nm = self.mod_w.shape[0]
        if sh.active and sh.p2p is not None and B == 1 and self.sp_shard_mods:
            W, r = sh.world, sh.rank
            cut = [(Nm * j // W) // 8 * 8 for j in range(W)] + [Nm]
            part = buf("mods_part", 1, cut[r + 1] - cut[r])
            ops.linear_small_m(emb, self.mod_w[cut[r]:cut[r + 1]], self.mod_b[cut[r]:cut[r + 1]], part, silu_in=True)
            mods = sh.p2p.symmetric(f"mods:{(1, Nm)}", (1, Nm), torch.bfloat16)
            sh._exchange(("mods", Nm), [(part[0], j, f"mods:{(1, Nm)}", cut[r]) for j in range(W)])
        else:
            mods = ops.linear_small_m(emb, self.mod_w, self.mod_b, buf("mods", B, Nm), silu_in=True)
        mbs = mods.stride(0)

        x = buf("x", B, S_loc, D)
        xv = x[:, Tt_loc:]
        pe = self.pos_embedding
        if pe is not None and pe.shape[0] != S:
            raise ValueError("learned positional embeddings need the configured sample height/width/frames")
        if Tt_loc:
            tp = m.patch_embed.text_proj
            ops.gemm(enc_in[:, sh.r0:sh.r0 + Tt_loc], tp.weight, x[:, :Tt_loc], bias=tp.bias,
                     res=None if pe is None else pe[sh.r0:sh.r0 + Tt_loc])
        cols = ops.patchify(hs, buf("cols", B, N, C * 4))
        ops.gemm(cols[:, v0:v1], self.patch_w, xv, bias=m.patch_embed.proj.bias,
                 res=None if pe is None else pe[Tt + v0:Tt + v1])
        if taps is not None:
            taps["emb"], taps["embed"] = emb.clone(), x.clone()

        xn = buf("xn", B, S_loc, D)
        qkv = buf("qkv", 3, B, S_loc, D)
        q, k, v = qkv[0], qkv[1], qkv[2]
        ff = buf("ff", B, S_loc, 4 * D)
        head_parallel = sh.active and H % sh.world == 0 and not self.sp_allgather
        if head_parallel:
            W = sh.world
            Dl = D // W
            qkvb = buf("qkv_blocks", 3 * W, S_loc, Dl)
            qh, kh, vh = buf("q_heads", S, Dl), buf("k_heads", S, Dl), buf("v_heads", S, Dl)
            oh = buf("o_heads", S, Dl)
        elif sh.active:
            k_full, v_full = buf("k_full", 1, S, D), buf("v_full", 1, S, D)
        r_logits = None
        for i, blk in enumerate(m.transformer_blocks):
            for half, nz in enumerate((blk.norm1, blk.norm2)):
                mo = mods[:, (2 * i + half) * 6 * D:]
                ln_kw = dict(eps=nz.norm.eps, shift0=mo[:, 3 * D:], scale0=mo[:, 4 * D:], shift1=mo, scale1=mo[:, D:],
                             split=Tt_loc, mod_batch_stride=mbs)
                xq = None
                if self._quantised(("qkv", "ff1")[half]) and self.fuse_ln_quant:
                    xq = self._layernorm_quant(("qkv", "ff1")[half], x, xn.shape, nz.norm.weight, nz.norm.bias, **ln_kw)
                else:
                    ops.layernorm(x, xn, nz.norm.weight, nz.norm.bias, **ln_kw)
                if half == 0:
                    at = blk.attn1
                    if head_parallel:
                        if sh.p2p is None:
                            self._dit_linear("qkv", i, xn[0], self.qkv_w[i], qkvb[0], bias=self.qkv_b[i], split=(Dl, S_loc * Dl),
                                             quantised=None if xq is None else (xq[0][0], xq[1][0]))
                        qk_kw = dict(heads=H // W, text_rows=Tt_loc if cos is not None else S_loc, eps=at.norm_q.eps,
                                     k_scale=self.k_scale)
                        if sh.p2p is not None:
                            sb, st = self._attn_bound(i, H, slots=max(1, 64 // W))
                            if (self.sp_overlap_v and st is None and xq is None and not self._quantised("qkv")
                                    and S_loc >= self.SP_OVERLAP_V_MIN_ROWS):
                                ops.gemm(xn[0], self.qkv_w[i][2 * D:], qkvb[2 * W], bias=self.qkv_b[i][2 * D:], split=(Dl, S_loc * Dl))
                                sh.push_v_heads(qkvb[2 * W:])
                                if not (self.qkn_epilogue and ops.gemm_qkv_norm_rope(
                                        xn[0], self.qkv_w[i][:2 * D], qkvb[0], self.qkv_b[i][:2 * D], (Dl, S_loc * Dl), at.norm_q.weight,
                                        at.norm_q.bias, at.norm_k.weight, at.norm_k.bias, cos, sin, qk_kw["text_rows"], eps=at.norm_q.eps,
                                        k_scale=self.k_scale, tensors=2)):
                                    ops.gemm(xn[0], self.qkv_w[i][:2 * D], qkvb[0], bias=self.qkv_b[i][:2 * D], split=(Dl, S_loc * Dl))
                                    ops.qknorm_rope(qkvb[:W], qkvb[W:2 * W], at.norm_q.weight, at.norm_q.bias, at.norm_k.weight,
                                                    at.norm_k.bias, cos, sin, heads=H // W, text_rows=qk_kw["text_rows"],
                                                    eps=at.norm_q.eps, k_scale=self.k_scale)
                                qh_, kh_, vh_ = sh.rows_to_heads_qk(qkvb[:2 * W])
                                st_all = None
                            else:
                                self._qkv_norm_rope(i, at, xn[0], qkvb[0], (Dl, S_loc * Dl), None if xq is None else (xq[0][0], xq[1][0]),
                                                    cos, sin, qk_kw["text_rows"], H // W, qkvb[:W], qkvb[W:2 * W], st)
                                qh_, kh_, vh_, st_all = sh.rows_to_heads_qkv(qkvb, st)
                            ops.self_attention(qh_[None], kh_[None], vh_[None], oh[None], heads=H // W, tag="joint", prescaled=True,
                                               score_bound=sb, bound=None if st is None else (st_all, sh.rank * (H // W), self._ws["qk_flags"]))
                            xo = sh.heads_to_rows(oh)
                            self._dit_linear("out", i, xo[None], at.to_out[0].weight, x, bias=at.to_out[0].bias, res=x,
                                             gate0=mo[:, 5 * D:], gate1=mo[:, 2 * D:], gate_split=Tt_loc, gate_batch_stride=mbs)
                            continue
                        pending = [sh.rows_to_heads(qkvb[2 * W:], vh, async_op=True)]
                        ops.qknorm_rope(qkvb[:W], None, at.norm_q.weight, at.norm_q.bias, at.norm_k.weight, at.norm_k.bias,
                                        cos, sin, **qk_kw)
                        pending.append(sh.rows_to_heads(qkvb[:W], qh, async_op=True))
                        ops.qknorm_rope(None, qkvb[W:2 * W], at.norm_q.weight, at.norm_q.bias, at.norm_k.weight,
                                        at.norm_k.bias, cos, sin, **qk_kw)
                        pending.append(sh.rows_to_heads(qkvb[W:2 * W], kh, async_op=True))
                        for h in pending:
                            if h is not None:
                                h.wait()
                        ops.self_attention(qh[None], kh[None], vh[None], oh[None], heads=H // W, tag="joint", prescaled=True,
                                           score_bound=self.score_bound[i])
                        sh.heads_to_rows(oh, xn[0])
                        self._dit_linear("out", i, xn, at.to_out[0].weight, x, bias=at.to_out[0].bias, res=x, gate0=mo[:, 5 * D:],
                                 gate1=mo[:, 2 * D:], gate_split=Tt_loc, gate_batch_stride=mbs)
                        continue
                    sb, st = self._attn_bound(i, B * H) if not sh.active else (self.score_bound[i], None)
                    self._qkv_norm_rope(i, at, xn, q, (D, B * S_loc * D), xq, cos, sin, Tt_loc if cos is not None else S_loc,
                                        H, q, k, st)
                    if sh.active:
                        if sh.p2p is not None:
                            sh.gather_rows_many([k[0], v[0]], [k_full[0], v_full[0]])
                        else:
                            sh.gather_rows(k[0], k_full[0])
                            sh.gather_rows(v[0], v_full[0])
                        oq = self._joint_attention(q, k_full, v_full, xn, heads=H, tag="joint", prescaled=True,
                                                   score_bound=self.score_bound[i])
                    else:
                        oq = self._joint_attention(q, k, v, xn, heads=H, tag="joint", prescaled=True, score_bound=sb,
                                                   bound=None if st is None else (st, 0, self._ws["qk_flags"]))
                    self._dit_linear("out", i, xn, at.to_out[0].weight, x, bias=at.to_out[0].bias, res=x, gate0=mo[:, 5 * D:],
                             gate1=mo[:, 2 * D:], gate_split=Tt_loc, gate_batch_stride=mbs, quantised=oq)
                else:
                    fq = None
                    if self._ff_pair_fused():
                        fq = self._ff1_mx_quant(i, xn, ff.shape, blk.ff.net[0].proj.bias, xq)
                    else:
                        self._dit_linear("ff1", i, xn, blk.ff.net[0].proj.weight, ff, bias=blk.ff.net[0].proj.bias,
                                         act="gelu_tanh", quantised=xq)
                    self._dit_linear("ff2", i, ff, blk.ff.net[2].weight, x, bias=blk.ff.net[2].bias, res=x, gate0=mo[:, 5 * D:],
                             gate1=mo[:, 2 * D:], gate_split=Tt_loc, gate_batch_stride=mbs, quantised=fq)
            if taps is not None:
                taps[f"block{i}"] = x.clone()

            if use_face and i % m.cross_attn_interval == 0:
                ca = i // m.cross_attn_interval
                ops.on_stream.need(face_marks.pop(ca, None))
                pc = m.perceiver_cross_attention[ca]
                inner_p = pc.to_q.weight.shape[0]
                hd_p = inner_p // 16
                lat = buf("lat", B, N_loc, D)
                qp = self._ln_linear("pq", ca, xv, lat, pc.norm2, pc.to_q.weight, buf("qp", B, N_loc, inner_p))
                kv_l = face_kv[ca]
                ntok = kv_l.shape[2]
                fuse_face = self.fused_attn_mix and taps is None
                pout = None if fuse_face else buf("pout", B, n_id, N_loc, inner_p)

                def perceiver_attention():
                    if fuse_face:
                        return
                    ops.attention(qp, kv_l, kv_l[..., inner_p:], pout, head_dim=hd_p, heads=16, nb1=B, nb2=n_id, Sq=N_loc,
                                  Skv=ntok, q_strides=(N_loc * inner_p, 0, inner_p),
                                  k_strides=(n_id * ntok * 2 * inner_p, ntok * 2 * inner_p, 2 * inner_p),
                                  v_strides=(n_id * ntok * 2 * inner_p, ntok * 2 * inner_p, 2 * inner_p),
                                  o_strides=(n_id * N_loc * inner_p, N_loc * inner_p, inner_p), scale=hd_p ** -0.5)
                if forced is None:
                    r_logits = self._router(qp, router_k[ca], ca, B, T, per_frame, n_id, sh, taps, perceiver_attention)
                else:
                    perceiver_attention()
                    r_logits = forced
                if fuse_face:
                    kvs_p = (ntok * 2 * inner_p, 0, 2 * inner_p)

                    def face_mix(z, mx):
                        for b in range(B):
                            rb = r_logits[b if r_logits.shape[0] > 1 else 0]
                            to = dict(z_strides=(0, inner_p)) if mx is None else dict(mx_out=(mx[0][b], mx[1][b], self.mx_fmt))
                            if ops.attn_kv_mix(qp[b], kv_l[b], kv_l[b][..., inner_p:], rb, None, None if z is None else z[b],
                                               head_dim=hd_p, heads=16, n_id=n_id, n_grp=1, Sq=N_loc, Skv=ntok,
                                               q_strides=(0, inner_p), k_strides=kvs_p, v_strides=kvs_p, scale=hd_p ** -0.5,
                                               **to) is False:
                                return False
                    self._cross_out("po", ca, "zmix_p", (B, N_loc, inner_p), face_mix, pc.to_out.weight, xv, res=xv,
                                    alpha=m.local_face_scale)
                elif self.mix_before_projection:
                    z = ops.routed_mix(pout, r_logits, None, "face", buf("zmix_p", B, N_loc, inner_p))
                    self._dit_linear("po", ca, z, pc.to_out.weight, xv, res=xv, alpha=m.local_face_scale)
                else:
                    feat = buf("feat", B, n_id, N_loc, D)
                    self._dit_linear("po", ca, pout.view(B * n_id, N_loc, inner_p), pc.to_out.weight, feat.view(B * n_id, N_loc, D))
                    if taps is not None:
                        taps[f"id_feat{ca}"] = feat[0].clone()
                    ops.masked_combine(xv, feat, r_logits, None, "face", alpha=m.local_face_scale)
                if taps is not None:
                    taps[f"face{i}"] = xv.clone()

            if use_audio and i % m.audio_attn_interval == 0:
                ops.on_stream.need(audio_mark[0])
                audio_mark[0] = None
                al = m.audio_model.layers[i // m.audio_attn_interval]
                at = al["attn"]
                an = buf("lat", B, N_loc, D)
                qa = self._ln_linear("aq", i // m.audio_attn_interval, xv, an, al["norm_q"], at.to_q.weight,
                                     buf("qa", B, N_loc, D), bias=at.to_q.bias)
                ka, va = audio_k[i // m.audio_attn_interval], audio_v[i // m.audio_attn_interval]
                ntok = ka.shape[3]
                fuse_audio = self.fused_attn_mix and taps is None
                kvs = (T * ntok * D, ntok * D, D)
                if fuse_audio:
                    wsum = self._ws.get("wsum")
                    if wsum is None or wsum.numel() != B * N_loc:
                        wsum = self._ws["wsum"] = torch.empty(B, N_loc, dtype=torch.float32, device=self.dev)
                    ai = i // m.audio_attn_interval

                    def audio_mix(z, mx):
                        for b in range(B):
                            rb = r_logits[b if r_logits.shape[0] > 1 else 0]
                            if not sh.active:
                                to = dict(z_strides=(per_frame * D, D)) if mx is None else dict(mx_out=(mx[0][b], mx[1][b], self.mx_fmt))
                                if ops.attn_kv_mix(qa[b], ka[b], va[b], rb, af[b], None if z is None else z[b], wsum[b],
                                                   head_dim=64, heads=H, n_id=n_id, n_grp=T, Sq=per_frame, Skv=ntok,
                                                   q_strides=(per_frame * D, D), k_strides=kvs, v_strides=kvs, scale=64 ** -0.5,
                                                   **to) is False:
                                    return False
                                continue
                            for f, start, length in sh.frame_segments(per_frame):
                                to = dict(z_strides=(0, D)) if mx is None else \
                                    dict(mx_out=(mx[0][b, start:], mx[1][b, start:], self.mx_fmt))
                                if ops.attn_kv_mix(qa[b, start:], ka[b, :, f], va[b, :, f], rb[start:start + length], af[b],
                                                   None if z is None else z[b, start:], wsum[b, start:], head_dim=64, heads=H,
                                                   n_id=n_id, n_grp=1, Sq=length, Skv=ntok, q_strides=(0, D),
                                                   k_strides=(kvs[0], 0, D), v_strides=(kvs[0], 0, D), scale=64 ** -0.5,
                                                   **to) is False:
                                    return False
                    self._cross_out("ao", ai, "zmix_a", (B, N_loc, D), audio_mix, at.to_out[0].weight, xv,
                                    bias=at.to_out[0].bias, res=xv, bias_rowscale=wsum)
                    continue
                ao = buf("ao", B, n_id, N_loc, D)
                for b in range(B):
                    if not sh.active:
                        ops.attention(qa[b], ka[b], va[b], ao[b], head_dim=64, heads=H, nb1=n_id, nb2=T, Sq=per_frame,
                                      Skv=ntok, q_strides=(0, per_frame * D, D), k_strides=kvs, v_strides=kvs,
                                      o_strides=(N_loc * D, per_frame * D, D), scale=64 ** -0.5)
                    else:
                        for f, start, length in sh.frame_segments(per_frame):
                            ops.attention(qa[b, start:], ka[b, :, f], va[b, :, f], ao[b, :, start:], head_dim=64,
                                          heads=H, nb1=n_id, nb2=1, Sq=length, Skv=ntok, q_strides=(0, 0, D),
                                          k_strides=kvs, v_strides=kvs, o_strides=(N_loc * D, 0, D), scale=64 ** -0.5)
                if self.mix_before_projection:
                    wsum = self._ws.get("wsum")
                    if wsum is None or wsum.numel() != B * N_loc:
                        wsum = self._ws["wsum"] = torch.empty(B, N_loc, dtype=torch.float32, device=self.dev)
                    z = ops.routed_mix(ao, r_logits, af, "audio", buf("zmix_a", B, N_loc, D), wsum)
                    self._dit_linear("ao", i // m.audio_attn_interval, z, at.to_out[0].weight, xv, bias=at.to_out[0].bias, res=xv,
                                     bias_rowscale=wsum)
                else:
                    feat = buf("feat", B, n_id, N_loc, D)
                    self._dit_linear("ao", i // m.audio_attn_interval, ao.view(B * n_id, N_loc, D), at.to_out[0].weight,
                                     feat.view(B * n_id, N_loc, D), bias=at.to_out[0].bias)
                    ops.masked_combine(xv, feat, r_logits, af, "audio")
                if taps is not None:
                    taps[f"audio{i}"] = xv.clone()

        if inv_side is not None:
            inv_side.join()
        xf = buf("lat", B, N_loc, D)
        ops.layernorm(xv, xf, m.norm_final.weight, m.norm_final.bias, eps=m.norm_final.eps)
        mo = mods[:, 2 * self.L * 6 * D:]
        xo = buf("qa", B, N_loc, D)
        ops.layernorm(xf, xo, m.norm_out.norm.weight, m.norm_out.norm.bias, eps=m.norm_out.norm.eps, shift0=mo,
                      scale0=mo[:, D:], shift1=mo, scale1=mo[:, D:], split=0, mod_batch_stride=mbs)
        co = m.proj_out.weight.shape[0]
        y = ops.gemm(xo, m.proj_out.weight, buf("y", B, N_loc, co), bias=m.proj_out.bias)
        if sh.active:
            y = sh.gather_video_rows(y, out=buf("y_full", B, N, co), in_place=True)
            if self.verify_exchanges:
                sh.verify_gathered(y)
        out = torch.empty(B, T, co // 4, Hh, Ww, dtype=torch.bfloat16, device=self.dev)
        ops.unpatchify(y, out)
        if sh.p2p is not None:
            sh.p2p.poison(out)
        return out

    def _r_lnlin(self, x, tmp, ln, pk, key, w, b, out, act=None):
        rg = pk.get(key)
        if rg is not None:
            return ops.rowgemm512(x, rg[0], out, act=act, eps=rg[1])
        self._ln(x, tmp, ln)
        return ops.gemm(tmp, w, out, bias=b, act=act)

    def _r_group_attn(self, x, tmp, qkv, out, ln, pk, name, L, heads, n_outer, n_inner, outer_stride, seq_stride):
        rg = pk.get("rg_" + name)
        hd = 64
        if rg is not None and L <= 32 and heads == 8 and self.router_fused_attn:
            return ops.router_group_attn(x, rg[0], out, L, n_outer, n_inner, outer_stride, seq_stride, eps=rg[1],
                                         scale=hd ** -0.5)
        F = x.shape[1]
        self._r_lnlin(x, tmp, ln, pk, "rg_" + name, *pk[name], qkv)
        return ops.attn_tiny(qkv, qkv[:, F:], qkv[:, 2 * F:], out, L, heads, n_outer, n_inner, outer_stride, seq_stride,
                             3 * F, F, hd ** -0.5)

    SP_OVERLAP_V_MIN_ROWS = 4096

    ROUTER_CHAIN_ROWS = {"mlp": (6000, 24000), "multi_id_attn": (6000, 24000), "temporal_attn": (1, 0)}

    def _chain_ok(self, rows, kind):
        lo, hi = self.ROUTER_CHAIN_ROWS[kind]
        return self.router_chain == "all" or (self.router_chain != "0" and lo <= rows <= hi)

    def _r_attn_block(self, x, tmp, qkv, a, ln, pk, name, to_out, L, heads, n_outer, n_inner, outer_stride, seq_stride):
        rg = pk.get("rg_" + name)
        if rg is not None and L <= 16 and heads == 8 and self.router_fused_attn and self._chain_ok(x.shape[0], name):
            return ops.router_group_attn_out(x, rg[0], rg[2], L, n_outer, n_inner, outer_stride, seq_stride, eps=rg[1],
                                             scale=64 ** -0.5)
        self._r_group_attn(x, tmp, qkv, a, ln, pk, name, L, heads, n_outer, n_inner, outer_stride, seq_stride)
        return self._r_linres(a, pk, "rg_" + name, to_out, x)

    def _r_mlp_block(self, x, tmp, h, st, pk):
        rg = pk.get("rg_mlp")
        if rg is not None and rg[0]["w"].shape[0] == 512 and self._chain_ok(x.shape[0], "mlp"):
            return ops.router_mlp_fused(x, rg[0], rg[2], eps=rg[1])
        self._r_lnlin(x, tmp, st.norm4, pk, "rg_mlp", st.mlp[0].weight, st.mlp[0].bias, h, act="gelu_erf")
        return self._r_linres(h, pk, "rg_mlp", st.mlp[2], x)

    def _r_linres(self, a, pk, key, lin, x):
        rg = pk.get(key)
        if rg is not None:
            return ops.rowgemm512(a, rg[2], x, res=x)
        return ops.gemm(a, lin.weight, x, bias=lin.bias, res=x)

    def _router(self, qp, kr, ca, B, T, per_frame, n_id, sh, taps, overlap):
        m, buf = self.m, self._buf
        r = m.router
        N, N_loc = T * per_frame, sh.N_loc
        F = r.feat_dim
        qk = qp.shape[-1]
        if sh.active and n_id * T >= sh.world and per_frame >= sh.world and not self.router_replicated:
            return self._router_sharded(qp, kr, ca, T, per_frame, n_id, sh, taps, overlap)
        overlap()
        qn = buf("r_qn", B, N_loc, qk)
        ops.layernorm(qp, qn, self.r_nq_w, self.r_nq_b, eps=r.norm_q.eps)
        qr = ops.gemm(qn, self.r_to_q[ca], buf("r_qr", B, N_loc, qk))
        rs = buf("r_s_loc", B, n_id, N_loc, F)
        pos = self.r_pos[sh.v0:sh.v1]
        for b in range(B):
            ops.router_scores(qr[b], kr[b].contiguous(), r.norm.weight, r.norm.bias, pos, rs[b], n_id, N_loc,
                              eps=r.norm.eps)
        if sh.active:
            rs = sh.gather_video_rows(rs, out=buf("r_s_full", B, n_id, N, F))
        R = B * n_id * N
        rs2, rn = rs.view(R, F), buf("r_n", R, F)
        qkv, ra, rh = buf("r_qkv", R, 3 * F), buf("r_a", R, F), buf("r_h", R, F)
        hd = 64
        heads = F // hd
        for st, pk in zip(r.spatial_temporal_layers, self.r_qkv):
            self._r_lnlin(rs2, rn, st.norm1, pk, "rg_spatial_attn", *pk["spatial_attn"], qkv)
            ops.attention(qkv, qkv[:, F:], qkv[:, 2 * F:], ra, head_dim=hd, heads=heads, nb1=B * n_id * T, nb2=1,
                          Sq=per_frame, Skv=per_frame, q_strides=(per_frame * 3 * F, 0, 3 * F),
                          k_strides=(per_frame * 3 * F, 0, 3 * F), v_strides=(per_frame * 3 * F, 0, 3 * F),
                          o_strides=(per_frame * F, 0, F), scale=hd ** -0.5, prescaled="rg_spatial_attn" in pk)
            self._r_linres(ra, pk, "rg_spatial_attn", st.spatial_attn.to_out[0], rs2)
            self._r_attn_block(rs2, rn, qkv, ra, st.norm2, pk, "temporal_attn", st.temporal_attn.to_out[0], T, heads,
                               B * n_id, per_frame, N, per_frame)
            self._r_attn_block(rs2, rn, qkv, ra, st.norm3, pk, "multi_id_attn", st.multi_id_attn.to_out[0], n_id, heads,
                               B, N, n_id * N, N)
            self._r_mlp_block(rs2, rn, rh, st, pk)
        logits = buf("r_logits", B, N, n_id)
        fp = r.final_proj[0]
        rs4 = rs2.view(B, n_id, N, F)
        for b in range(B):
            ops.router_head(rs4[b], fp.weight, fp.bias, logits[b], n_id, N)
        if taps is not None:
            for b in range(B):
                taps[f"router{ca}_b{b}"] = logits[b:b + 1].clone()
        return logits if not sh.active else logits[:, sh.v0:sh.v1].contiguous()

    def _router_sharded(self, qp, kr, ca, T, per_frame, n_id, sh, taps, overlap):
        m, buf = self.m, self._buf
        r = m.router
        N, N_loc, F = T * per_frame, sh.N_loc, r.feat_dim
        pairs = n_id * T
        rp = self._router_partition(sh, pairs, per_frame)
        qk = qp.shape[-1]
        qn = buf("r_qn", 1, N_loc, qk)
        ops.layernorm(qp, qn, self.r_nq_w, self.r_nq_b, eps=r.norm_q.eps)
        qr = ops.gemm(qn, self.r_to_q[ca], buf("r_qr", 1, N_loc, qk))
        rs_loc = buf("r_s_loc", 1, n_id, N_loc, F)
        ops.router_scores(qr[0], kr[0].contiguous(), r.norm.weight, r.norm.bias, self.r_pos[sh.v0:sh.v1], rs_loc[0],
                          n_id, N_loc, eps=r.norm.eps)
        if rp.p2p is not None:
            xa = rp.tokens_to_a(rs_loc[0], sh.v0, T)
        else:
            rs_full = sh.gather_video_rows(rs_loc, out=buf("r_s_full", 1, n_id, N, F))
            xa = buf("rp_xa", rp.nPA, per_frame, F)
            xa.copy_(rs_full.view(pairs, per_frame, F)[rp.pa0:rp.pa1])
        RA, RB = rp.nPA * per_frame, pairs * rp.nLB
        rn_a, qkv_a, ra_a = buf("rp_rn_a", RA, F), buf("rp_qkv_a", RA, 3 * F), buf("rp_ra_a", RA, F)
        xb = rp.recv_buf("rp_xb", (pairs, rp.nLB, F), xa)
        rn_b, qkv_b, ra_b, rh_b = buf("rp_rn_b", RB, F), buf("rp_qkv_b", RB, 3 * F), buf("rp_ra_b", RB, F), buf("rp_rh_b", RB, F)
        hd = 64
        heads = F // hd
        nblk = len(r.spatial_temporal_layers)
        for bi, (st, pk) in enumerate(zip(r.spatial_temporal_layers, self.r_qkv)):
            xa2 = xa.view(RA, F)
            self._r_lnlin(xa2, rn_a, st.norm1, pk, "rg_spatial_attn", *pk["spatial_attn"], qkv_a)
            ops.attention(qkv_a, qkv_a[:, F:], qkv_a[:, 2 * F:], ra_a, head_dim=hd, heads=heads, nb1=rp.nPA, nb2=1,
                          Sq=per_frame, Skv=per_frame, q_strides=(per_frame * 3 * F, 0, 3 * F),
                          k_strides=(per_frame * 3 * F, 0, 3 * F), v_strides=(per_frame * 3 * F, 0, 3 * F),
                          o_strides=(per_frame * F, 0, F), scale=hd ** -0.5, prescaled="rg_spatial_attn" in pk)
            self._r_linres(ra_a, pk, "rg_spatial_attn", st.spatial_attn.to_out[0], xa2)
            rp.a_to_b(xa, xb, overlap=overlap if bi == 0 else None)
            xb2 = xb.view(RB, F)
            self._r_attn_block(xb2, rn_b, qkv_b, ra_b, st.norm2, pk, "temporal_attn", st.temporal_attn.to_out[0], T, heads,
                               n_id, rp.nLB, T * rp.nLB, rp.nLB)
            self._r_attn_block(xb2, rn_b, qkv_b, ra_b, st.norm3, pk, "multi_id_attn", st.multi_id_attn.to_out[0], n_id, heads,
                               1, T * rp.nLB, 0, T * rp.nLB)
            self._r_mlp_block(xb2, rn_b, rh_b, st, pk)
            if bi + 1 < nblk:
                xa = rp.b_to_a(xb, xa)
        fp = r.final_proj[0]
        lb = buf("rp_logits_b", T * rp.nLB, n_id)
        ops.router_head(xb.view(n_id, T * rp.nLB, F), fp.weight, fp.bias, lb, n_id, T * rp.nLB)
        logits = rp.gather_b_rows(lb.view(T, rp.nLB, n_id), out=buf("rp_logits", T, per_frame, n_id)).view(1, N, n_id)
        if taps is not None:
            taps[f"router{ca}_b0"] = logits.clone()
        return logits[:, sh.v0:sh.v1].contiguous()
```

### bind_your_avatar_implementation_amd/ops.py

```python
import ctypes
import os

import torch

from . import _hip
from ._hip import AttnDesc, AttnMixDesc, GemmDesc, check

ACT = {None: 0, "none": 0, "gelu_tanh": 1, "gelu_erf": 2, "relu": 3, "silu": 4, "leaky_relu": 5,
       "gelu_tanh_ieee": 6}


_PINNED_STREAM = None


def _stream():
    if _PINNED_STREAM is not None:
        return _PINNED_STREAM
    return torch.cuda.current_stream().cuda_stream


class pinned_stream:

    def __enter__(self):
        global _PINNED_STREAM
# ... 1054 lines not shown
            "sk_rem": p.sk_rem, "sk_cut": p.sk_cut, "o_wide": p.o_wide, "second_launch": p.second_launch}
    if mx is not None:
        plan["mx_out"] = mx_out[2]
    return plan


def attention_plan_key(plan):
    tail = "/" + plan["mx_out"] if plan.get("mx_out") else ("/wide" if plan["o_wide"] else "/narrow")
    return plan["variant"] + ("+streamk" if plan["stream_k"] else "") + tail


def attn_kv_mix_plan(z, af=None, *, head_dim, heads, n_id, n_grp, Sq, Skv, q_strides, k_strides, v_strides, z_strides=None,
                     scale=1.0, mx_out=None):
    lib = _hip.load()
    p = _hip.AttnMixPlan()
    if mx_out is not None:
        mx = _mix_mx_out(mx_out, z, z_strides, heads, head_dim, n_grp, Sq, plan=True)
        d = _mix_desc(head_dim, heads, n_id, n_grp, Sq, Skv, q_strides, k_strides, v_strides, (0, 0), scale)
        rc = lib.bya_attn_kv_mix_mx_plan(_plan_p(mx[0]), _plan_p(mx[1]), _plan_p(af), ctypes.byref(d), mx[2], *mx[3], ctypes.byref(p))
        if rc == -4:
            return None
        check(rc, "bya_attn_kv_mix_mx_plan")
    else:
        d = _mix_desc(head_dim, heads, n_id, n_grp, Sq, Skv, q_strides, k_strides, v_strides, z_strides, scale)
        check(lib.bya_attn_kv_mix_plan(_plan_p(z), _plan_p(af), ctypes.byref(d), ctypes.byref(p)), "bya_attn_kv_mix_plan")
    plan = {"form": KV_MIX_FORMS[p.form], "head_dim": p.head_dim, "grid": p.grid, "row_chunks": p.row_chunks,
            "lds_bytes": p.lds_bytes, "big_lds": p.big_lds}
    if mx_out is not None:
        plan["mx_out"] = mx_out[2]
    return plan


def _mix_mx_out(mx_out, z, z_strides, heads, head_dim, n_grp, Sq, plan=False):
    if z is not None or z_strides is not None:
        raise ValueError("attn_kv_mix: with mx_out there is no bf16 output -- pass z=None and no z_strides")
    codes, scales, fmt = mx_out
    code = mx_fmt_code(fmt)
    strides = []
    for t, name, width in ((codes, "codes", mx_code_bytes(heads * head_dim, fmt)), (scales, "scales", heads * head_dim // 32)):
        if t.dtype != torch.uint8:
            raise TypeError(f"attn_kv_mix: mx_out {name}: expected uint8, got {t.dtype}")
        if not (t.is_cuda or (plan and t.is_meta)):
            raise ValueError(f"attn_kv_mix: mx_out {name}: expected a device tensor")
        ok = t.dim() in (2, 3) and t.stride(-1) == 1 and t.shape[-1] >= width
        if ok and t.dim() == 2:
            ok = t.shape[0] >= n_grp * Sq
            grp, row = Sq * t.stride(0), t.stride(0)
        elif ok:
            ok = t.shape[0] >= n_grp and t.shape[1] >= Sq
            grp, row = t.stride(0), t.stride(1)
        if not ok:
            raise ValueError(f"attn_kv_mix: mx_out {name} must be uint8 [{n_grp * Sq}, >= {width}] or [{n_grp}, {Sq}, >= {width}] "
                             f"with a contiguous last dimension, got {tuple(t.shape)} strides {tuple(t.stride())}")
        strides += [grp, row]
    return codes, scales, code, tuple(strides)


def attn_tiny_plan(q, k, v, out, L, heads, n_outer, n_inner, ld_qkv, ld_o):
    lib = _hip.load()
    p, a = _hip.AttnTinyPlan(), _plan_p
    check(lib.bya_attn_tiny_plan(a(q), a(k), a(v), a(out), L, heads, n_outer, n_inner, ld_qkv, ld_o, ctypes.byref(p)),
          "bya_attn_tiny_plan")
    return {"instance": TINY_INSTANCES[p.instance], "grid": p.grid, "waves": p.waves}


def _mix_desc(head_dim, heads, n_id, n_grp, Sq, Skv, q_strides, k_strides, v_strides, z_strides, scale):
    d = AttnMixDesc()
    d.head_dim, d.heads, d.n_id, d.n_grp, d.Sq, d.Skv = head_dim, heads, n_id, n_grp, Sq, Skv
    d.q_grp, d.q_row = q_strides
    d.k_id, d.k_grp, d.k_row = k_strides
    d.v_id, d.v_grp, d.v_row = v_strides
    d.z_grp, d.z_row = z_strides
    d.scale = float(scale)
    return d


def attention(q, k, v, out, *, head_dim, heads, nb1, nb2, Sq, Skv, q_strides, k_strides, v_strides, o_strides=None,
              scale, tag="other", prescaled=False, score_bound=0.0, bound=None, mx_out=None):
    lib = _hip.load()
    mx = None
    if mx_out is not None:
        if out is not None:
            raise ValueError("attention: with mx_out there is no bf16 output -- pass out=None")
        mx = _attn_mx_out(mx_out, heads, head_dim, nb1, nb2, Sq, o_strides)
        o_strides = (0, 0, 0)
    for t in (q, k, v) + (() if mx is not None else (out,)):
        assert t.dtype == torch.bfloat16 and t.is_cuda
    d = _attn_desc(head_dim, heads, nb1, nb2, Sq, Skv, q_strides, k_strides, v_strides, o_strides, scale, prescaled,
                   score_bound, bound)
    if prescaled and (score_bound > 0 or bound is not None) and q.device.index not in _ATTN_WS:
        ensure_attn_workspace(q.device)
    var = ATTN_VARIANT_NAMES.get(lib.bya_attn_variant(ctypes.byref(d)), "rejected")
    ATTN_VARIANTS[tag, var] = ATTN_VARIANTS.get((tag, var), 0) + 1
    label = ("bya_attn_fwd_mx:" if mx is not None else "bya_attn_fwd:") + tag
    if _SHAPE_LABELS:
        label += f":{nb1}x{nb2}x{heads}h_q{Sq}_kv{Skv}_d{head_dim}" + (f">{mx_out[2]}" if mx is not None else "")
    tok = _begin(label, 4.0 * nb1 * nb2 * heads * Sq * Skv * head_dim)
    if mx is not None:
        check(lib.bya_attn_fwd_mx(_p(q), _p(k), _p(v), _p(mx[0]), _p(mx[1]), ctypes.byref(d), mx[2], *mx[3], _stream()),
              "bya_attn_fwd_mx")
    else:
        check(lib.bya_attn_fwd(_p(q), _p(k), _p(v), _p(out), ctypes.byref(d), _stream()), "bya_attn_fwd")
    _end(tok)
    return (mx[0], mx[1]) if mx is not None else out


def self_attention(q, k, v, out, heads, head_dim=64, scale=None, tag="other", prescaled=False, score_bound=0.0, bound=None,
                   mx_out=None):
    b, S, _, q_bs, q_ld = _mat(q, "q")
    _, Skv, _, k_bs, k_ld = _mat(k, "k")
    _, _, _, v_bs, v_ld = _mat(v, "v")
    o_strides = None
    if mx_out is None:
        _, _, _, o_bs, o_ld = _mat(out, "out")
        o_strides = (o_bs, 0, o_ld)
    scale = head_dim ** -0.5 if scale is None else scale
    return attention(q, k, v, out, head_dim=head_dim, heads=heads, nb1=b, nb2=1, Sq=S, Skv=Skv,
                     q_strides=(q_bs, 0, q_ld), k_strides=(k_bs, 0, k_ld), v_strides=(v_bs, 0, v_ld),
                     o_strides=o_strides, scale=scale, tag=tag, prescaled=prescaled, score_bound=score_bound, bound=bound,
                     mx_out=mx_out)


def attn_kv_mix(q, k, v, r, af, z, wsum=None, *, head_dim, heads, n_id, n_grp, Sq, Skv, q_strides, k_strides, v_strides,
                z_strides=None, scale, mx_out=None):
    lib = _hip.load()
    mx = None
    if mx_out is not None:
        mx = _mix_mx_out(mx_out, z, z_strides, heads, head_dim, n_grp, Sq)
        z_strides = (0, 0)
    d = _mix_desc(head_dim, heads, n_id, n_grp, Sq, Skv, q_strides, k_strides, v_strides, z_strides, scale)
    for t in (q, k, v, r) + (() if mx is not None else (z,)):
        assert t.dtype == torch.bfloat16 and t.is_cuda
    assert r.is_contiguous() and r.numel() == n_grp * Sq * n_id
    assert af is None or (af.is_contiguous() and af.dtype == torch.bfloat16 and af.numel() == n_id * n_id)
    assert wsum is None or (wsum.dtype == torch.float32 and wsum.is_contiguous() and wsum.numel() >= n_grp * Sq)
    flops = 4.0 * n_id * n_grp * heads * Sq * Skv * head_dim
    if mx is not None:
        tok = _begin("bya_attn_kv_mix_mx")
        rc = lib.bya_attn_kv_mix_mx(_p(q), _p(k), _p(v), _p(r), _p(af), _p(mx[0]), _p(mx[1]), _p(wsum), ctypes.byref(d), mx[2],
                                    *mx[3], _stream())
        if rc == -4:
            return False
        check(rc, "bya_attn_kv_mix_mx")
        if tok is not None:
            _FLOPS[tok[0]] = _FLOPS.get(tok[0], 0.0) + flops
        _end(tok)
        return mx[0], mx[1]
    tok = _begin("bya_attn_kv_mix", flops)
    check(lib.bya_attn_kv_mix(_p(q), _p(k), _p(v), _p(r), _p(af), _p(z), _p(wsum), ctypes.byref(d), _stream()), "bya_attn_kv_mix")
    _end(tok)
    return z


def attn_tiny(q, k, v, out, L, heads, n_outer, n_inner, outer_stride, seq_stride, ld_qkv, ld_o, scale):
    lib = _hip.load()
    tok = _begin("bya_attn_tiny")
    check(lib.bya_attn_tiny(_p(q), _p(k), _p(v), _p(out), L, heads, n_outer, n_inner, outer_stride, seq_stride,
                            ld_qkv, ld_o, float(scale), _stream()), "bya_attn_tiny")
    _end(tok)
    return out


def router_scores(qr, kr, ln_w, ln_b, pos_emb, out, n_id, N, eps=1e-5):
    lib = _hip.load()
    for t in (qr, kr, ln_w, ln_b, pos_emb, out):
        assert t.is_contiguous() and t.dtype == torch.bfloat16
    tok = _begin("bya_router_scores", 2.0 * n_id * N * 32 * qr.shape[-1])
    check(lib.bya_router_scores(_p(qr), _p(kr), _p(ln_w), _p(ln_b), _p(pos_emb), _p(out), n_id, N, 16, 32,
                                float(eps), _stream()), "bya_router_scores")
    _end(tok)
    return out


def router_scores_plan(qr, kr, ln_w, ln_b, pos_emb, out, n_id, N):
    lib = _hip.load()
    p, a = _hip.StepPlan(), _plan_p
    check(lib.bya_router_scores_plan(a(qr), a(kr), a(ln_w), a(ln_b), a(pos_emb), a(out), n_id, N, 16, 32, ctypes.byref(p)),
          "bya_router_scores_plan")
    return _step_plan(p, _hip.ROUTER_SCORES_KERNELS[p.kernel])


def router_head(x, w, b, r, n_id, N):
    lib = _hip.load()
    assert x.is_contiguous() and r.is_contiguous()
    tok = _begin("bya_router_head")
    check(lib.bya_router_head(_p(x), _p(w), _p(b), _p(r), n_id, N, x.shape[-1], _stream()), "bya_router_head")
    _end(tok)
    return r


def forcing_max_over_frames(forcing, out, frames, per_frame, n_id):
    lib = _hip.load()
    assert forcing.is_contiguous() and out.is_contiguous() and forcing.dtype == out.dtype == torch.bfloat16
    tok = _begin("bya_forcing_max_over_frames")
    check(lib.bya_forcing_max_over_frames(_p(forcing), _p(out), frames, per_frame, n_id, _stream()),
          "bya_forcing_max_over_frames")
    _end(tok)
    return out


def masked_combine(x, feat, r, af, mode, alpha=1.0):
    lib = _hip.load()
    b, N, D, x_bs, x_row = _mat(x, "x")
    assert feat.is_contiguous() and feat.shape[0] == b and feat.shape[2] == N and feat.shape[3] == D
    n_id = feat.shape[1]
    assert r.is_contiguous() and r.shape[-2:] == (N, n_id) and r.dtype == torch.bfloat16
    r_bs = 0 if r.shape[0] == 1 else N * n_id
    if af is not None:
        assert af.is_contiguous() and af.dtype == torch.bfloat16 and af.shape == (b, n_id, n_id)
    tok = _begin("bya_masked_combine")
    check(lib.bya_masked_combine(_p(x), _p(feat), _p(r), _p(af), {"face": 0, "audio": 1}[mode], float(alpha), b,
                                 n_id, N, D, x_row, x_bs, r_bs, _stream()), "bya_masked_combine")
    _end(tok)
    return x


def routed_mix(feat, r, af, mode, z, wsum=None):
    lib = _hip.load()
    b, n_id, N, D = feat.shape
    assert feat.is_contiguous() and z.is_contiguous() and z.shape == (b, N, D)
    assert r.is_contiguous() and r.shape[-2:] == (N, n_id) and r.dtype == torch.bfloat16
    r_bs = 0 if r.shape[0] == 1 else N * n_id
    if wsum is not None:
        assert wsum.dtype == torch.float32 and wsum.is_contiguous() and wsum.numel() == b * N
    tok = _begin("bya_routed_mix")
    check(lib.bya_routed_mix(_p(feat), _p(r), _p(af), _p(z), _p(wsum), {"face": 0, "audio": 1}[mode], b, n_id, N, D,
                             r_bs, _stream()), "bya_routed_mix")
    _end(tok)
    return z


def patchify(x, cols):
    lib = _hip.load()
    b, t, c, h, w = x.shape
    assert x.is_contiguous() and cols.is_contiguous() and x.dtype == cols.dtype == torch.bfloat16
    tok = _begin("bya_patchify")
    check(lib.bya_patchify(_p(x), _p(cols), b, t, c, h, w, _stream()), "bya_patchify")
    _end(tok)
    return cols


def unpatchify(y, out):
    lib = _hip.load()
    b, t, c, h, w = out.shape
    assert y.is_contiguous() and out.is_contiguous() and y.dtype == out.dtype == torch.bfloat16
    tok = _begin("bya_unpatchify")
    check(lib.bya_unpatchify(_p(y), _p(out), b, t, c, h, w, _stream()), "bya_unpatchify")
    _end(tok)
    return out


def act_add(x, out, act=None, res=None):
    lib = _hip.load()
    assert x.is_contiguous() and out.is_contiguous() and (res is None or res.is_contiguous())
    tok = _begin("bya_act_add")
    check(lib.bya_act_add(_p(x), _p(res), _p(out), x.numel(), ACT[act], _stream()), "bya_act_add")
    _end(tok)
    return out


def act_add_plan(x, out, act=None, res=None):
    lib = _hip.load()
    p, a = _hip.StepPlan(), _plan_p
    check(lib.bya_act_add_plan(a(x), a(res), a(out), x.numel(), ACT[act], ctypes.byref(p)), "bya_act_add_plan")
    return _step_plan(p, "act_add")


def _sched_pred(pred, n):
    n_pred = pred.shape[0] if pred.numel() != n else 1
    assert pred.dtype == torch.bfloat16 and n_pred in (1, 2) and pred.numel() == n_pred * n
    if n_pred == 1:
        assert pred.is_contiguous()
        return 1, n
    assert pred[0].is_contiguous() and pred.stride(0) >= n
    return 2, pred.stride(0)


def cfg_scheduler_step_plan(pred, sample, coef, out=None):
    lib = _hip.load()
    p, a = _hip.StepPlan(), _plan_p
    n = sample.numel()
    n_pred, stride = _sched_pred(pred, n)
    c = _hip.SchedCoef(**{k: float(v) for k, v in coef.items()})
    check(lib.bya_cfg_scheduler_step_plan(a(pred), n_pred, stride, a(sample), a(sample if out is None else out), n, ctypes.byref(c),
                                          ctypes.byref(p)), "bya_cfg_scheduler_step_plan")
    return _step_plan(p, "cfg_scheduler_step")


def cfg_scheduler_step(pred, sample, coef, old_x0=None, noise=None, x0_out=None, out=None):
    import ctypes
    lib = _hip.load()
    n = sample.numel()
    n_pred, pred_stride = _sched_pred(pred, n)
    assert sample.dtype == torch.bfloat16 and sample.is_contiguous()
    for t, dt in ((old_x0, torch.float32), (noise, torch.bfloat16), (x0_out, torch.float32)):
        assert t is None or (t.dtype == dt and t.is_contiguous() and t.numel() == n)
    if out is None:
        out = torch.empty_like(sample)
    c = _hip.SchedCoef(**{k: float(v) for k, v in coef.items()})
    tok = _begin("bya_cfg_scheduler_step")
    check(lib.bya_cfg_scheduler_step(_p(pred), n_pred, pred_stride, _p(sample), _p(old_x0), _p(noise), _p(out), _p(x0_out), n,
                                     ctypes.byref(c), _stream()), "bya_cfg_scheduler_step")
    _end(tok)
    return out


def masks_to_routing_logits(masks, frames=13, h=30, w=45, out=None):
    lib = _hip.load()
    assert masks.dtype == torch.uint8 and masks.is_contiguous() and masks.dim() == 4
    n_id, Ti, Hi, Wi = masks.shape
    if out is None:
        out = torch.empty(1, frames * h * w, n_id, dtype=torch.bfloat16, device=masks.device)
    tok = _begin("bya_masks_to_routing_logits")
    check(lib.bya_masks_to_routing_logits(_p(masks), _p(out), n_id, Ti, Hi, Wi, frames, h, w, _stream()),
          "bya_masks_to_routing_logits")
    _end(tok)
    return out


def pack_rowgemm512(weight, bias, ln_weight=None, ln_bias=None):
    w32 = weight.float()
    b32 = bias.float() if bias is not None else torch.zeros(weight.shape[0], device=weight.device)
    if ln_weight is None:
        return dict(w=weight.to(torch.bfloat16).contiguous(), colsum=None, cvec=b32.contiguous(), ln=False)
    wg = (w32 * ln_weight.float()[None, :]).to(torch.bfloat16).contiguous()
    return dict(w=wg, colsum=wg.float().sum(1).contiguous(), cvec=(w32 @ ln_bias.float() + b32).contiguous(), ln=True)


def rowgemm512(x, pack, out, res=None, act=None, eps=1e-5, nsplit=0):
    lib = _hip.load()
    M, K = x.shape
    N = pack["w"].shape[0]
# ... 186 lines not shown
```

### include/bya.h

```cpp
#ifndef BYA_H
#define BYA_H

#include <stdint.h>

#ifdef __cplusplus
extern "C" {
#endif
#if defined(__GNUC__) || defined(__clang__)
#pragma GCC visibility push(default)
#endif

#ifndef __HIP_PLATFORM_AMD__
typedef struct ihipStream_t* hipStream_t;
#endif

enum { BYA_ACT_NONE = 0, BYA_ACT_GELU_TANH = 1, BYA_ACT_GELU_ERF = 2, BYA_ACT_RELU = 3, BYA_ACT_SILU = 4,
       BYA_ACT_LEAKY_RELU = 5,
       BYA_ACT_GELU_TANH_IEEE = 6  };

int bya_abi_version(void);

enum bya_option {
    BYA_OPT_GEMM_SPLITK = 0,
    BYA_OPT_GEMM_SPLITK_MIN = 1,
// ... 117 lines not shown
int bya_gemm_mx_qkv_norm_rope(const void* A, const void* a_scales, const void* W, const void* w_scales, const void* bias,
                              void* C, int32_t fmt, int32_t w_fmt, const bya_gemm_desc* desc, const bya_qknorm_desc* norm,
                              hipStream_t stream);
int bya_gemm_mx_qkv_norm_rope_plan(const void* A, const void* a_scales, const void* W, const void* w_scales,
                                   const void* bias, const void* C, int32_t fmt, int32_t w_fmt, const bya_gemm_desc* desc,
                                   const bya_qknorm_desc* norm, bya_gemm_plan* plan);
int bya_gemm_mx_qkv_norm_rope_on(const void* A, const void* a_scales, const void* W, const void* w_scales, const void* bias,
                                 void* C, int32_t fmt, int32_t w_fmt, const bya_gemm_desc* desc, const bya_qknorm_desc* norm,
                                 int32_t kernel, hipStream_t stream);
int bya_gemm_mx_qkv_norm_rope_on_plan(const void* A, const void* a_scales, const void* W, const void* w_scales,
                                      const void* bias, const void* C, int32_t fmt, int32_t w_fmt, const bya_gemm_desc* desc,
                                      const bya_qknorm_desc* norm, int32_t kernel, bya_gemm_plan* plan);
#define BYA_MX_KERNEL_FP6 16
typedef struct bya_mx_gemm_call {
    const void *A, *a_scales, *W, *w_scales, *bias;
    void* C;
    const void *res, *gate0, *gate1;
    void* q_scales;
    const bya_qknorm_desc* norm;
    int32_t a_fmt, w_fmt, out_fmt, kernel;
} bya_mx_gemm_call;
int bya_gemm_mx_call(const bya_mx_gemm_call* call, const bya_gemm_desc* desc, hipStream_t stream);
int bya_gemm_mx_call_plan(const bya_mx_gemm_call* call, const bya_gemm_desc* desc, bya_gemm_plan* plan);

int bya_linear_small_m(const void* x, const void* W, const void* bias, void* out, int32_t M, int32_t N,
                       int32_t K, int32_t silu_in, int32_t act_out, hipStream_t stream);

#define BYA_ROUTER_SCORES_WAVE 0
#define BYA_ROUTER_SCORES_LDS 1
typedef struct bya_step_plan_info {
    int32_t kernel;
    int32_t grid;
    int32_t rounds;
    int32_t reserved;
    int64_t items;
    int64_t items_per_round;
} bya_step_plan_info;
int bya_linear_small_m_plan(const void* x, const void* W, const void* out, int32_t M, int32_t N, int32_t K, int32_t act_out,
                            bya_step_plan_info* plan);

int bya_timestep_features(const int64_t* timesteps, void* out, int32_t batch, int32_t dim,
                          int32_t flip_sin_to_cos, float freq_shift, hipStream_t stream);

int bya_layernorm(const void* x, void* y, const void* w, const void* b, const void* shift0, const void* scale0,
                  const void* shift1, const void* scale1, int64_t rows_per_batch, int32_t batch, int32_t D,
                  int64_t ldx, int64_t ldy, int64_t x_batch_stride, int64_t y_batch_stride,
                  int64_t mod_batch_stride, int64_t split, float eps, hipStream_t stream);
#define BYA_LN_OUT_BF16 0
#define BYA_LN_OUT_FP8 1
#define BYA_LN_OUT_MX_E4M3 2
#define BYA_LN_OUT_MX_E2M3 3
#define BYA_LN_KERNEL_GENERIC 0
#define BYA_LN_KERNEL_ROWS 1
typedef struct bya_layernorm_plan_info {
    int32_t kernel;
    int32_t vec, nv;
    int32_t modulated;
    int32_t rows_per_wave;
    int32_t grid;
    int64_t waves;
} bya_layernorm_plan_info;
int bya_layernorm_plan(const void* x, const void* y, const void* w, const void* b, const void* shift0, const void* scale0,
                       const void* shift1, const void* scale1, int64_t rows_per_batch, int32_t batch, int32_t D, int64_t ldx,
                       int64_t ldy, int64_t x_batch_stride, int64_t y_batch_stride, int64_t mod_batch_stride, int64_t split,
                       int32_t out_kind, bya_layernorm_plan_info* plan);

int bya_qknorm_rope(void* q, void* k, const void* qw, const void* qb, const void* kw, const void* kb,
                    const float* cos, const float* sin, int32_t batch, int32_t S, int32_t heads, int64_t ld,
                    int64_t batch_stride, int32_t text_rows, float eps, float k_scale, float* stats, int32_t stats_slots,
                    hipStream_t stream);
typedef struct bya_qknorm_rope_plan_info {
    int32_t stats;
    int32_t only;
    int32_t grid;
    int32_t slots;
    int64_t pairs;
    int64_t waves;
} bya_qknorm_rope_plan_info;
int bya_qknorm_rope_plan(const void* q, const void* k, const void* qw, const void* qb, const void* kw, const void* kb,
                         const float* cos, const float* sin, int32_t batch, int32_t S, int32_t heads, int64_t ld,
                         int64_t batch_stride, int32_t text_rows, const float* stats, int32_t stats_slots,
                         bya_qknorm_rope_plan_info* plan);

typedef struct bya_attn_desc {
    int32_t head_dim;
    int32_t heads;
    int32_t nb1, nb2;
    int32_t Sq, Skv;
    int64_t q_s1, q_s2, q_row;
    int64_t k_s1, k_s2, k_row;
    int64_t v_s1, v_s2, v_row;
    int64_t o_s1, o_s2, o_row;
    float scale;
    int32_t scores_prescaled;
    float score_bound;
    const float* bound_dev;
    int32_t bound_slots, bound_heads, bound_bh0;
    int32_t* fallback_flags;
} bya_attn_desc;
#define BYA_ATTN_BOUND_LIMIT 90.0f

int bya_attn_fwd(const void* q, const void* k, const void* v, void* o, const bya_attn_desc* desc,
                 hipStream_t stream);

#define BYA_ATTN_D64_RUNNING_MAX 0
#define BYA_ATTN_D64_PRESCALED 1
#define BYA_ATTN_D64_STATIC_BOUND 2
#define BYA_ATTN_D128 3
#define BYA_ATTN_D64_STATIC_BOUND_W4 4
#define BYA_ATTN_D64_DEVICE_BOUND_W4 5
int bya_attn_variant(const bya_attn_desc* desc);

typedef struct bya_attn_plan_info {
    int32_t variant;
    int32_t grid;
    int32_t q_tile;
    int32_t stream_k;
    int32_t sk_rem;
    int32_t sk_cut;
    int32_t o_wide;
    int32_t second_launch;
} bya_attn_plan_info;
int bya_attn_plan(const bya_attn_desc* desc, const void* o, int32_t workspace_assumed, bya_attn_plan_info* plan);

int bya_attn_fwd_mx(const void* q, const void* k, const void* v, void* codes, void* scales, const bya_attn_desc* desc,
                    int32_t out_fmt, int64_t c_s1, int64_t c_s2, int64_t c_row, int64_t sc_s1, int64_t sc_s2, int64_t sc_row,
                    hipStream_t stream);
int bya_attn_mx_plan(const bya_attn_desc* desc, const void* codes, const void* scales, int32_t out_fmt, int64_t c_s1,
                     int64_t c_s2, int64_t c_row, int64_t sc_s1, int64_t sc_s2, int64_t sc_row, int32_t workspace_assumed,
                     bya_attn_plan_info* plan);

int bya_set_attn_workspace(void* ws, int64_t bytes);
int bya_attn_workspace_bytes(int64_t* bytes);
int bya_attn_workspace_status(int32_t* timeouts, hipStream_t stream);

typedef struct bya_attn_mix_desc {
    int32_t head_dim, heads, n_id, n_grp, Sq, Skv;
    int64_t q_grp, q_row, k_id, k_grp, k_row, v_id, v_grp, v_row, z_grp, z_row;
    float scale;
} bya_attn_mix_desc;
int bya_attn_kv_mix(const void* q, const void* k, const void* v, const void* r, const void* af, void* z, float* wsum,
                    const bya_attn_mix_desc* desc, hipStream_t stream);
#define BYA_KV_MIX_MIX32 0
#define BYA_KV_MIX_ONE_TILE 1
typedef struct bya_attn_kv_mix_plan_info {
    int32_t form;
    int32_t head_dim;
    int32_t grid;
    int32_t row_chunks;
    int32_t lds_bytes;
    int32_t big_lds;
} bya_attn_kv_mix_plan_info;
int bya_attn_kv_mix_plan(const void* z, const void* af, const bya_attn_mix_desc* desc, bya_attn_kv_mix_plan_info* plan);

int bya_attn_kv_mix_mx(const void* q, const void* k, const void* v, const void* r, const void* af, void* codes, void* scales,
                       float* wsum, const bya_attn_mix_desc* desc, int32_t out_fmt, int64_t c_grp, int64_t c_row,
                       int64_t sc_grp, int64_t sc_row, hipStream_t stream);
int bya_attn_kv_mix_mx_plan(const void* codes, const void* scales, const void* af, const bya_attn_mix_desc* desc,
                            int32_t out_fmt, int64_t c_grp, int64_t c_row, int64_t sc_grp, int64_t sc_row,
                            bya_attn_kv_mix_plan_info* plan);

int bya_attn_tiny(const void* q, const void* k, const void* v, void* o, int32_t L, int32_t heads,
                  int64_t n_outer, int64_t n_inner, int64_t outer_stride, int64_t seq_stride, int64_t ld_qkv,
                  int64_t ld_o, float scale, hipStream_t stream);
#define BYA_TINY8_2 0
#define BYA_TINY8_3 1
#define BYA_TINY8_13 2
#define BYA_TINY8_25 3
#define BYA_TINY_GENERIC_2 4
#define BYA_TINY_GENERIC_4 5
#define BYA_TINY_GENERIC_16 6
#define BYA_TINY_GENERIC_32 7
typedef struct bya_attn_tiny_plan_info {
    int32_t instance;
    int32_t grid;
    int64_t waves;
} bya_attn_tiny_plan_info;
int bya_attn_tiny_plan(const void* q, const void* k, const void* v, const void* o, int32_t L, int32_t heads, int64_t n_outer,
                       int64_t n_inner, int64_t ld_qkv, int64_t ld_o, bya_attn_tiny_plan_info* plan);

int bya_router_scores(const void* qr, const void* kr, const void* ln_w, const void* ln_b, const void* pos_emb,
                      void* out, int32_t n_id, int64_t N, int32_t heads, int32_t face_tokens, float eps,
                      hipStream_t stream);
int bya_router_scores_plan(const void* qr, const void* kr, const void* ln_w, const void* ln_b, const void* pos_emb,
                           const void* out, int32_t n_id, int64_t N, int32_t heads, int32_t face_tokens,
                           bya_step_plan_info* plan);
int bya_router_head(const void* x, const void* w, const void* b, void* r, int32_t n_id, int64_t N, int32_t D,
                    hipStream_t stream);

int bya_forcing_max_over_frames(const void* forcing, void* out, int32_t frames, int64_t per_frame,
                                int32_t n_id, hipStream_t stream);

int bya_masked_combine(void* x, const void* feat, const void* r, const void* af, int32_t mode, float alpha,
                       int32_t batch, int32_t n_id, int64_t N, int32_t D, int64_t x_row, int64_t x_batch_stride,
                       int64_t r_batch_stride, hipStream_t stream);

int bya_routed_mix(const void* feat, const void* r, const void* af, void* z, float* wsum, int32_t mode, int32_t batch,
                   int32_t n_id, int64_t N, int32_t D, int64_t r_batch_stride, hipStream_t stream);

int bya_patchify(const void* x, void* cols, int32_t batch, int32_t frames, int32_t channels, int32_t H, int32_t W,
                 hipStream_t stream);
int bya_unpatchify(const void* y, void* out, int32_t batch, int32_t frames, int32_t channels, int32_t H, int32_t W,
                   hipStream_t stream);

int bya_act_add(const void* x, const void* r, void* y, int64_t n, int32_t act, hipStream_t stream);
int bya_act_add_plan(const void* x, const void* r, const void* y, int64_t n, int32_t act,
                     bya_step_plan_info* plan);

int bya_rowgemm512(const void* X, const void* W, const float* colsum, const float* cvec, const void* res, void* C,
                   int32_t M, int32_t N, int32_t ldx, int32_t ldc, int32_t ldres, int32_t ln, float eps, int32_t act,
                   int32_t nsplit, hipStream_t stream);
#define BYA_ROWGEMM_CHUNK_BALANCED 0
#define BYA_ROWGEMM_W_STATIONARY 1
typedef struct bya_rowgemm512_plan_info {
    int32_t form;
    int32_t ln, res, act;
    int32_t grid;
    int32_t crosses_row_block;
    int64_t work_items;
} bya_rowgemm512_plan_info;
int bya_rowgemm512_plan(const void* X, const void* W, const float* colsum, const float* cvec, const void* res, const void* C,
                        int32_t M, int32_t N, int32_t ldx, int32_t ldc, int32_t ldres, int32_t ln, int32_t act,
                        bya_rowgemm512_plan_info* plan);

int bya_router_group_attn(const void* X, const void* Wqkv, const float* colsum, const float* cvec, void* O,
                          int32_t M, int32_t ldx, int32_t ldo, int32_t L, int64_t n_outer, int64_t n_inner,
                          int64_t outer_stride, int64_t seq_stride, float eps, float scale, hipStream_t stream);
typedef struct bya_router_group_attn_plan_info {
    int32_t P, G, wide;
    int32_t blocks;
    int64_t tiles;
} bya_router_group_attn_plan_info;
int bya_router_group_attn_plan(const void* X, const void* Wqkv, const float* colsum, const float* cvec, const void* O,
                               int32_t M, int32_t ldx, int32_t ldo, int32_t L, int64_t n_outer, int64_t n_inner,
                               int64_t outer_stride, int64_t seq_stride, bya_router_group_attn_plan_info* plan);

int bya_router_mlp_fused(const void* X, const void* W1, const float* colsum1, const float* cvec1, const void* W2,
                         const float* cvec2, void* C, int32_t M, int32_t ldx, int32_t ldc, float eps, int32_t tiles_pass0,
                         hipStream_t stream);
int bya_router_group_attn_out(const void* X, const void* Wqkv, const float* colsum, const float* cvec, const void* Wo,
                              const float* cvec_o, void* C, int32_t M, int32_t ldx, int32_t ldc, int32_t L, int64_t n_outer,
                              int64_t n_inner, int64_t outer_stride, int64_t seq_stride, float eps, float scale,
                              int32_t tiles_pass0, hipStream_t stream);
typedef struct bya_router_chain_plan_info {
    int32_t tiles, tp0, grid, passes, tiles_last, wgs_last;
} bya_router_chain_plan_info;
int bya_router_mlp_fused_plan(const void* X, const void* W1, const float* colsum1, const float* cvec1, const void* W2,
                              const float* cvec2, const void* C, int32_t M, int32_t ldx, int32_t ldc, int32_t tiles_pass0,
                              bya_router_chain_plan_info* plan);
int bya_router_group_attn_out_plan(const void* X, const void* Wqkv, const float* colsum, const float* cvec, const void* Wo,
                                   const float* cvec_o, const void* C, int32_t M, int32_t ldx, int32_t ldc, int32_t L,
                                   int64_t n_outer, int64_t n_inner, int64_t outer_stride, int64_t seq_stride,
                                   int32_t tiles_pass0, bya_router_chain_plan_info* plan);

typedef struct bya_sched_coef {
    float guidance, sqrt_alpha, sqrt_beta, k_sample, k_denoised, k_noise, k_cur, k_old;
} bya_sched_coef;

int bya_cfg_scheduler_step(const void* pred, int32_t n_pred, int64_t pred_stride, const void* sample,
                           const float* old_x0, const void* noise, void* prev_sample, float* x0_out,
                           int64_t n, const bya_sched_coef* coef, hipStream_t stream);
int bya_cfg_scheduler_step_plan(const void* pred, int32_t n_pred, int64_t pred_stride, const void* sample,
                                const void* prev_sample, int64_t n, const bya_sched_coef* coef,
                                bya_step_plan_info* plan);

int bya_masks_to_routing_logits(const void* masks, void* logits, int32_t n_id, int32_t in_frames, int32_t in_h,
                                int32_t in_w, int32_t frames, int32_t h, int32_t w, hipStream_t stream);

int bya_vae_patches(const void* x, const void* cache, void* out, int32_t Ts, int32_t Hs, int32_t Ws, int32_t C, int32_t KT,
                    int32_t stride, int32_t pad, int32_t up, int32_t tmode, int32_t Ho, int32_t Wo, int32_t t0, int32_t nt,
                    int32_t Kpad, hipStream_t stream);
int bya_vae_groupnorm_stats(const void* x, float* sums, float* partial, int64_t rows, int32_t C, int32_t groups,
                            hipStream_t stream);
int bya_vae_norm_act(const void* x, void* y, const float* sums, const void* gamma, const void* beta, const void* zy,
                     const void* zb, int64_t rows, int32_t C, int32_t groups, int32_t act, float eps, int32_t T, int32_t H,
                     int32_t W, int32_t Tz, int32_t hz, int32_t wz, int32_t tmode, int64_t ldz, int32_t out_pad,
                     hipStream_t stream);

int bya_vae_conv3d(const void* xpad, const void* w, const void* bias, const void* res, void* out, int32_t To, int32_t H,
                   int32_t W, int32_t C, int32_t Cout, int32_t KT, int64_t ldw, int64_t ldc, int64_t ldres,
                   hipStream_t stream);

int bya_vae_upsample_pad(const void* x, void* ypad, int32_t T, int32_t H, int32_t W, int32_t C, int32_t tmode,
                         hipStream_t stream);

int bya_allgather_kv(const void* k_local, const void* v_local, void* k_full, void* v_full, int64_t rows_local,
                     int64_t row_elems, void* comm, hipStream_t stream);
int bya_alltoall_router(const void* send, void* recv, const int64_t* send_counts, const int64_t* recv_counts,
                        int32_t world, void* comm, hipStream_t stream);

typedef struct bya_p2p_copy {
    const void* src;
    void* dst;
    int64_t row_bytes;
    int64_t rows;
    int64_t src_pitch, dst_pitch;
    int64_t chunk0;
} bya_p2p_copy;

int bya_p2p_push(const bya_p2p_copy* copies_dev, int32_t n_copies, int64_t total_chunks, void* const* peer_ctrl_dev,
                 int32_t world, int32_t rank, void* ctrl, hipStream_t stream);
int bya_p2p_wait(void* ctrl, int32_t world, void* group_ctrl, int64_t wait_limit_ms, hipStream_t stream);
int bya_p2p_exchange(const bya_p2p_copy* copies_dev, int32_t n_copies, int64_t total_chunks, void* const* peer_ctrl_dev,
                     int32_t world, int32_t rank, void* ctrl, void* group_ctrl, int64_t wait_limit_ms, hipStream_t stream);
int bya_p2p_poison(const void* ctrl_base, int32_t n_channels, void* out, int64_t n_elems, hipStream_t stream);
int bya_p2p_alloc(int64_t bytes, int32_t kind, void** out);
int bya_p2p_free(void* ptr);
int bya_p2p_ipc_export(void* ptr, void* handle64);
int bya_p2p_ipc_import(const void* handle64, void** out);
int bya_p2p_ipc_release(void* ptr);

#if defined(__GNUC__) || defined(__clang__)
#pragma GCC visibility pop
#endif
#ifdef __cplusplus
}
#endif
#endif
```

Baseline: 2.873 steps/s.

## Fold router query projection into keys and face output projection into values

Adds two algebraic reassociations. The router pre-multiplies its small key set by the query projection weight, so scores become one GEMM from normalized queries, followed by a new layernorm-plus-position kernel, and the full per-token query projection GEMM is dropped. The face cross-attention pre-multiplies its values by the output projection, emits scaled softmax probabilities from a new variant of the mix32 kernel, and applies them with a single GEMM into the residual, removing the PV step and the separate output projection over all video tokens. Both paths are on by default for bf16 weights, and they change rounding order in bf16.

```diff
diff --git a/bind_your_avatar_implementation_amd/_hip.py b/bind_your_avatar_implementation_amd/_hip.py
--- a/bind_your_avatar_implementation_amd/_hip.py
+++ b/bind_your_avatar_implementation_amd/_hip.py
@@ -156,6 +156,8 @@
     "bya_attn_workspace_status": [_c.POINTER(_i32), _vp],
     "bya_attn_kv_mix": [_vp, _vp, _vp, _vp, _vp, _vp, _vp, _c.POINTER(AttnMixDesc), _vp],
     "bya_attn_kv_mix_plan": [_vp, _vp, _c.POINTER(AttnMixDesc), _c.POINTER(AttnMixPlan)],
+    "bya_attn_kv_mix_probs": [_vp, _vp, _vp, _vp, _c.POINTER(AttnMixDesc), _vp],
+    "bya_face_fold_values": [_vp, _vp, _vp, _i32, _i32, _i32, _i32, _i64, _i64, _vp],
     "bya_attn_kv_mix_mx": [_vp, _vp, _vp, _vp, _vp, _vp, _vp, _vp, _c.POINTER(AttnMixDesc), _i32, _i64, _i64, _i64, _i64, _vp],
     "bya_attn_kv_mix_mx_plan": [_vp, _vp, _vp, _c.POINTER(AttnMixDesc), _i32, _i64, _i64, _i64, _i64, _c.POINTER(AttnMixPlan)],
     "bya_attn_tiny": [_vp, _vp, _vp, _vp, _i32, _i32, _i64, _i64, _i64, _i64, _i64, _i64, _f32, _vp],
@@ -163,6 +165,8 @@
     "bya_router_scores": [_vp, _vp, _vp, _vp, _vp, _vp, _i32, _i64, _i32, _i32, _f32, _vp],
     "bya_router_scores_plan": [_vp, _vp, _vp, _vp, _vp, _vp, _i32, _i64, _i32, _i32, _c.POINTER(StepPlan)],
     "bya_router_head": [_vp, _vp, _vp, _vp, _i32, _i64, _i32, _vp],
+    "bya_router_fold_keys": [_vp, _vp, _vp, _i32, _i32, _i32, _vp],
+    "bya_router_ln_pos": [_vp, _vp, _vp, _vp, _vp, _i32, _i64, _i32, _f32, _vp],
     "bya_forcing_max_over_frames": [_vp, _vp, _i32, _i64, _i32, _vp],
     "bya_masked_combine": [_vp, _vp, _vp, _vp, _i32, _f32, _i32, _i32, _i64, _i32, _i64, _i64, _i64, _vp],
     "bya_routed_mix": [_vp, _vp, _vp, _vp, _vp, _i32, _i32, _i32, _i64, _i32, _i64, _vp],
diff --git a/bind_your_avatar_implementation_amd/csrc/attn.hip b/bind_your_avatar_implementation_amd/csrc/attn.hip
--- a/bind_your_avatar_implementation_amd/csrc/attn.hip
+++ b/bind_your_avatar_implementation_amd/csrc/attn.hip
@@ -380,6 +380,10 @@
 __global__ __launch_bounds__(256) void attn_kv_mix32_kernel_d128(MixArgs p) {
     extern __shared__ __attribute__((aligned(16))) char smem[];
     attn_mix32_body<128>(p, smem);
+}
+__global__ __launch_bounds__(256) void attn_kv_mix32_probs_kernel_d128(MixArgs p) {
+    extern __shared__ __attribute__((aligned(16))) char smem[];
+    attn_mix32_body<128, false, true>(p, smem);
 }
 
 __global__ __launch_bounds__(256, 2) void attn_kv_mix_kernel_d64(MixArgs p) {
@@ -663,6 +667,22 @@
     return hipGetLastError() == hipSuccess ? BYA_OK : BYA_ERR_LAUNCH;
 }
 
+extern "C" int bya_attn_kv_mix_probs(const void* q, const void* k, const void* r, void* pr, const bya_attn_mix_desc* d,
+                                     hipStream_t stream) {
+    if (!q || !k || !r || !pr || !d) return BYA_ERR_SHAPE;
+    bya_attn_kv_mix_plan_info pl;
+    const int prc = mix_plan_of(pr, d, 0, (uintptr_t)q | (uintptr_t)k, &pl);
+    if (prc != BYA_OK) return prc;
+    if (pl.form != BYA_KV_MIX_MIX32 || d->head_dim != 128 || d->Skv != 32) return BYA_ERR_UNSUPPORTED;
+    if (d->z_row < (int64_t)d->heads * d->n_id * 32) return BYA_ERR_SHAPE;
+    MixArgs a;
+    mix_args_of(q, k, k, r, nullptr, nullptr, d, pl.row_chunks, a);
+    a.z = (bf16_t*)pr; a.z_grp = d->z_grp; a.z_row = d->z_row;
+    const int lds = (d->n_id + 4) * 32 * 128 * 2;
+    BYA_LAUNCH(attn_kv_mix32_probs_kernel_d128, dim3((unsigned)pl.grid), dim3(256), (size_t)lds, stream, a);
+    return hipGetLastError() == hipSuccess ? BYA_OK : BYA_ERR_LAUNCH;
+}
+
 extern "C" int bya_attn_kv_mix_mx_plan(const void* codes, const void* scales, const void* af, const bya_attn_mix_desc* d,
                                       int32_t out_fmt, int64_t c_grp, int64_t c_row, int64_t sc_grp, int64_t sc_row,
                                       bya_attn_kv_mix_plan_info* plan) {
diff --git a/bind_your_avatar_implementation_amd/csrc/attn_mix32.h b/bind_your_avatar_implementation_amd/csrc/attn_mix32.h
--- a/bind_your_avatar_implementation_amd/csrc/attn_mix32.h
+++ b/bind_your_avatar_implementation_amd/csrc/attn_mix32.h
@@ -90,9 +90,11 @@
     }
 }
 
-template <int D, bool MX = false>
+template <int D, bool MX = false, bool PR = false>
 __device__ __forceinline__ void attn_mix32_body(const MixArgs& p, char* smem, const ByaMixMxOut* mx = nullptr) {
+    static_assert(!PR || (D == 128 && !MX), "the probability output exists on the d128 bf16 instance alone");
     constexpr int ROW_BYTES = D * 2, KV_BYTES = 32 * ROW_BYTES, DSTEPS = D / 16, DT = D / 32;
+    constexpr int ID_BYTES = PR ? KV_BYTES : 2 * KV_BYTES;
     const int tid = threadIdx.x, lane = tid & 63;
     const int wave = __builtin_amdgcn_readfirstlane(tid >> 6);
     const int r = lane & 31, hf = lane >> 5;
@@ -104,13 +106,15 @@
     const int t0 = (int)((long long)n32 * chunk / p.nqt), t1 = (int)((long long)n32 * (chunk + 1) / p.nqt);
     const bf16_t* Q = p.q + grp * p.q_grp + (long long)head * D;
     bf16_t* Z = nullptr;
-    if constexpr (!MX) Z = p.z + grp * p.z_grp + (long long)head * D;
+    if constexpr (PR) Z = p.z + grp * p.z_grp + (long long)head * (p.n_id * 32);
+    else if constexpr (!MX) Z = p.z + grp * p.z_grp + (long long)head * D;
 
     for (int id = 0; id < p.n_id; ++id) {
-        stage_kv32<D>(p.k + id * p.k_id + grp * p.k_grp + (long long)head * D, p.k_row, p.Skv - 1, smem + id * 2 * KV_BYTES,
+        stage_kv32<D>(p.k + id * p.k_id + grp * p.k_grp + (long long)head * D, p.k_row, p.Skv - 1, smem + id * ID_BYTES,
                       wave, lane, false);
-        stage_kv32<D>(p.v + id * p.v_id + grp * p.v_grp + (long long)head * D, p.v_row, p.Skv - 1,
-                      smem + id * 2 * KV_BYTES + KV_BYTES, wave, lane, true);
+        if constexpr (!PR)
+            stage_kv32<D>(p.v + id * p.v_id + grp * p.v_grp + (long long)head * D, p.v_row, p.Skv - 1,
+                          smem + id * ID_BYTES + KV_BYTES, wave, lane, true);
     }
     const int g = lane >> 4, li = lane & 15, tq = li >> 2, tp = li & 3;
     uint32_t voff[DT];
@@ -143,11 +147,11 @@
             for (int i = 0; i < p.n_id; ++i) ws += w[i];
             p.wsum[(long long)grp * p.Sq + qrow] = ws;
         }
-        char* zb = smem + p.n_id * 2 * KV_BYTES + wave * KV_BYTES;
+        char* zb = smem + p.n_id * ID_BYTES + wave * KV_BYTES;
         constexpr int CHUNKS = ROW_BYTES / 16;
         f32x16 zacc[DT];
         for (int id = 0; id < p.n_id; ++id) {
-            const uint32_t kb = lds0 + id * 2 * KV_BYTES, vb = kb + KV_BYTES;
+            const uint32_t kb = lds0 + id * ID_BYTES, vb = kb + KV_BYTES;
             bf16x8 kf[DSTEPS];
 #pragma unroll
             for (int s = 0; s < DSTEPS; ++s) kf[s] = lds_read128<0>(kb + koff[s]);
@@ -158,11 +162,13 @@
 #pragma unroll
             for (int s = 0; s < DSTEPS; ++s) sacc = __builtin_amdgcn_mfma_f32_32x32x16_bf16(kf[s], qf[s], sacc, 0, 0, 0);
             VFrag<D> fa, fb;
-            uint32_t vbase[DT];
-#pragma unroll
-            for (int d = 0; d < DT; ++d) vbase[d] = vb + voff[d];
-            v_issue<D, 0>(fa, vbase);
-            v_issue<D, 1>(fb, vbase);
+            if constexpr (!PR) {
+                uint32_t vbase[DT];
+#pragma unroll
+                for (int d = 0; d < DT; ++d) vbase[d] = vb + voff[d];
+                v_issue<D, 0>(fa, vbase);
+                v_issue<D, 1>(fb, vbase);
+            }
             float mx = -INFINITY;
 #pragma unroll
             for (int i = 0; i < 16; ++i) {
@@ -185,10 +191,21 @@
                 for (int e = 0; e < 8; ++e) {
                     const float pv = __builtin_amdgcn_exp2f((sacc[tt * 8 + e] - m_new) * c);
                     psum += pv;
-                    pf[tt][e] = (__bf16)pv;
+                    if constexpr (PR) sacc[tt * 8 + e] = pv;
+                    else pf[tt][e] = (__bf16)pv;
                 }
             const auto lsw = __builtin_amdgcn_permlane32_swap(__float_as_uint(psum), __float_as_uint(psum), false, false);
             const float sc = w[id] / (__uint_as_float(lsw[0]) + __uint_as_float(lsw[1]));
+            if constexpr (PR) {
+#pragma unroll
+                for (int j = 0; j < 4; ++j) {
+                    u32x2 o;
+                    o[0] = pack2bf(sacc[4 * j + 0] * sc, sacc[4 * j + 1] * sc);
+                    o[1] = pack2bf(sacc[4 * j + 2] * sc, sacc[4 * j + 3] * sc);
+                    *reinterpret_cast<u32x2*>(zb + r * 256 + (((4 * id + j) ^ (r & 7)) << 4) + 8 * hf) = o;
+                }
+                continue;
+            }
             f32x16 oacc[DT];
 #pragma unroll
             for (int d = 0; d < DT; ++d)
@@ -202,6 +219,19 @@
             for (int d = 0; d < DT; ++d)
 #pragma unroll
                 for (int i = 0; i < 16; ++i) zacc[d][i] = id == 0 ? fmaf(sc, oacc[d][i], 0.f) : fmaf(sc, oacc[d][i], zacc[d][i]);
+        }
+        if constexpr (PR) {
+            __builtin_amdgcn_fence(__ATOMIC_RELEASE, "wavefront");
+            __builtin_amdgcn_wave_barrier();
+            __builtin_amdgcn_fence(__ATOMIC_ACQUIRE, "wavefront");
+            const int pch = p.n_id * 4;
+            for (int idx = lane; idx < 32 * pch; idx += 64) {
+                const int row = idx / pch, ch = idx % pch;
+                const u32x4 o = *reinterpret_cast<const u32x4*>(zb + row * 256 + ((ch ^ (row & 7)) << 4));
+                if (t * 32 + row < p.Sq) *reinterpret_cast<u32x4*>(Z + (long long)(t * 32 + row) * p.z_row + ch * 8) = o;
+            }
+            __builtin_amdgcn_wave_barrier();
+            continue;
         }
 #pragma unroll
         for (int d = 0; d < DT; ++d)
diff --git a/bind_your_avatar_implementation_amd/csrc/router.hip b/bind_your_avatar_implementation_amd/csrc/router.hip
--- a/bind_your_avatar_implementation_amd/csrc/router.hip
+++ b/bind_your_avatar_implementation_amd/csrc/router.hip
@@ -328,8 +328,115 @@
     }
 }
 
+__global__ __launch_bounds__(256) void router_fold_keys_kernel(const bf16_t* __restrict__ kr, const bf16_t* __restrict__ wt,
+                                                               bf16_t* __restrict__ kt, int rows) {
+    const int lane = threadIdx.x & 63;
+    const int wid = blockIdx.x * 4 + (threadIdx.x >> 6);
+    constexpr int CT = R_QK / 16;
+    if (wid >= R_HEADS * CT) return;
+    const int h = wid / CT, ct = wid % CT;
+    const int c = lane & 15, g = lane >> 4;
+    const bf16_t* wrow = wt + (long long)(ct * 16 + c) * R_QK + h * R_HD + g * 8;
+    bf16x8 wf[4];
+#pragma unroll
+    for (int ks = 0; ks < 4; ++ks) wf[ks] = *reinterpret_cast<const bf16x8*>(wrow + ks * 32);
+    for (int rt = 0; rt < rows / 16; ++rt) {
+        const long long row = rt * 16 + c;
+        const bf16_t* krow = kr + row * R_QK + h * R_HD + g * 8;
+        f32x4 acc = f32x4{0.f, 0.f, 0.f, 0.f};
+#pragma unroll
+        for (int ks = 0; ks < 4; ++ks)
+            acc = __builtin_amdgcn_mfma_f32_16x16x32_bf16(wf[ks], *reinterpret_cast<const bf16x8*>(krow + ks * 32), acc, 0, 0, 0);
+        u32x2 o = {pack2bf(acc[0], acc[1]), pack2bf(acc[2], acc[3])};
+        *reinterpret_cast<u32x2*>(kt + (row * R_HEADS + h) * R_QK + ct * 16 + 4 * g) = o;
+    }
+}
+
+__global__ __launch_bounds__(256) void face_fold_values_kernel(const bf16_t* __restrict__ v, const bf16_t* __restrict__ wo,
+                                                               bf16_t* __restrict__ vw, int rows, int n_out, long long ldv,
+                                                               long long ldvw) {
+    const int lane = threadIdx.x & 63;
+    const int wid = blockIdx.x * 4 + (threadIdx.x >> 6);
+    const int ot_n = n_out / 16;
+    if (wid >= R_HEADS * ot_n) return;
+    const int h = wid / ot_n, ot = wid % ot_n;
+    const int c = lane & 15, g = lane >> 4;
+    const bf16_t* wrow = wo + (long long)(ot * 16 + c) * R_QK + h * R_HD + g * 8;
+    bf16x8 wf[4];
+#pragma unroll
+    for (int ks = 0; ks < 4; ++ks) wf[ks] = *reinterpret_cast<const bf16x8*>(wrow + ks * 32);
+    for (int rt = 0; rt < rows / 16; ++rt) {
+        const bf16_t* vrow = v + (long long)(rt * 16 + c) * ldv + h * R_HD + g * 8;
+        f32x4 acc = f32x4{0.f, 0.f, 0.f, 0.f};
+#pragma unroll
+        for (int ks = 0; ks < 4; ++ks)
+            acc = __builtin_amdgcn_mfma_f32_16x16x32_bf16(*reinterpret_cast<const bf16x8*>(vrow + ks * 32), wf[ks], acc, 0, 0, 0);
+        u32x2 o = {pack2bf(acc[0], acc[1]), pack2bf(acc[2], acc[3])};
+        *reinterpret_cast<u32x2*>(vw + (long long)(ot * 16 + c) * ldvw + h * rows + rt * 16 + 4 * g) = o;
+    }
+}
+
+__global__ __launch_bounds__(256) void router_ln_pos_kernel(const bf16_t* __restrict__ s, const bf16_t* __restrict__ ln_w,
+                                                            const bf16_t* __restrict__ ln_b, const bf16_t* __restrict__ pos,
+                                                            bf16_t* __restrict__ out, long long rows, long long N, float eps) {
+    const int lane = threadIdx.x & 63;
+    const long long row = (long long)blockIdx.x * 4 + (threadIdx.x >> 6);
+    if (row >= rows) return;
+    const long long n = row % N;
+    const int f0 = lane * 8;
+    float x[8], wv[8], bv[8], pv[8], o[8];
+    unpack8(*reinterpret_cast<const u32x4*>(s + row * R_FEAT + f0), x);
+    unpack8(*reinterpret_cast<const u32x4*>(pos + n * R_FEAT + f0), pv);
+    unpack8(*reinterpret_cast<const u32x4*>(ln_w + f0), wv);
+    unpack8(*reinterpret_cast<const u32x4*>(ln_b + f0), bv);
+    float sum = 0.f;
+#pragma unroll
+    for (int e = 0; e < 8; ++e) sum += x[e];
+    const float mean = wave_sum(sum) * (1.0f / R_FEAT);
+    float sq = 0.f;
+#pragma unroll
+    for (int e = 0; e < 8; ++e) { const float d = x[e] - mean; sq += d * d; }
+    const float rstd = rsqrtf(wave_sum(sq) * (1.0f / R_FEAT) + eps);
+#pragma unroll
+    for (int e = 0; e < 8; ++e) o[e] = bf2f(f2bf((x[e] - mean) * rstd * wv[e] + bv[e])) + pv[e];
+    *reinterpret_cast<u32x4*>(out + row * R_FEAT + f0) = pack8(o);
+}
+
 inline int ok() { const hipError_t e = hipGetLastError(); return e == hipSuccess ? BYA_OK : -(1000 + (int)e); }
 
+}
+
+extern "C" int bya_router_fold_keys(const void* kr, const void* wq_t, void* kt, int32_t rows, int32_t heads, int32_t head_dim,
+                                    hipStream_t stream) {
+    if (!kr || !wq_t || !kt || rows <= 0 || rows % 16) return BYA_ERR_SHAPE;
+    if (heads != R_HEADS || head_dim != R_HD) return BYA_ERR_UNSUPPORTED;
+    if (((uintptr_t)kr | (uintptr_t)wq_t | (uintptr_t)kt) & 15) return BYA_ERR_ALIGN;
+    BYA_LAUNCH(router_fold_keys_kernel, dim3(R_HEADS * (R_QK / 16) / 4), dim3(256), 0, stream, (const bf16_t*)kr,
+               (const bf16_t*)wq_t, (bf16_t*)kt, (int)rows);
+    return ok();
+}
+
+extern "C" int bya_face_fold_values(const void* v, const void* wo, void* vw, int32_t rows, int32_t n_out, int32_t heads,
+                                    int32_t head_dim, int64_t ldv, int64_t ldvw, hipStream_t stream) {
+    if (!v || !wo || !vw || rows <= 0 || rows % 16 || n_out <= 0 || n_out % 16) return BYA_ERR_SHAPE;
+    if (heads != R_HEADS || head_dim != R_HD) return BYA_ERR_UNSUPPORTED;
+    if (ldv < R_QK || ldvw < (int64_t)R_HEADS * rows) return BYA_ERR_SHAPE;
+    if ((((uintptr_t)v | (uintptr_t)wo | (uintptr_t)vw) & 15) || ldv % 8 || ldvw % 8) return BYA_ERR_ALIGN;
+    BYA_LAUNCH(face_fold_values_kernel, dim3((unsigned)(R_HEADS * (n_out / 16) / 4)), dim3(256), 0, stream, (const bf16_t*)v,
+               (const bf16_t*)wo, (bf16_t*)vw, (int)rows, (int)n_out, (long long)ldv, (long long)ldvw);
+    return ok();
+}
+
+extern "C" int bya_router_ln_pos(const void* s, const void* ln_w, const void* ln_b, const void* pos_emb, void* out, int32_t n_id,
+                                 int64_t N, int32_t feat, float eps, hipStream_t stream) {
+    if (!s || !ln_w || !ln_b || !pos_emb || !out || n_id <= 0 || N <= 0) return BYA_ERR_SHAPE;
+    if (feat != R_FEAT) return BYA_ERR_UNSUPPORTED;
+    if (((uintptr_t)s | (uintptr_t)ln_w | (uintptr_t)ln_b | (uintptr_t)pos_emb | (uintptr_t)out) & 15) return BYA_ERR_ALIGN;
+    const long long rows = (long long)n_id * N;
+    if ((rows + 3) / 4 > 0x7fffffffLL) return BYA_ERR_SHAPE;
+    BYA_LAUNCH(router_ln_pos_kernel, dim3((unsigned)((rows + 3) / 4)), dim3(256), 0, stream, (const bf16_t*)s, (const bf16_t*)ln_w,
+               (const bf16_t*)ln_b, (const bf16_t*)pos_emb, (bf16_t*)out, rows, (long long)N, eps);
+    return ok();
 }
 
 static int scores_plan_of(const void* qr, const void* kr, const void* ln_w, const void* ln_b, const void* pos_emb, const void* out,
diff --git a/bind_your_avatar_implementation_amd/engine.py b/bind_your_avatar_implementation_amd/engine.py
--- a/bind_your_avatar_implementation_amd/engine.py
+++ b/bind_your_avatar_implementation_amd/engine.py
@@ -105,6 +105,10 @@
             self.SP_OVERLAP_V_MIN_ROWS = 0
         self.router_replicated = os.environ.get("BYA_ROUTER_REPLICATED", "0") == "1"
         self.qkn_epilogue = os.environ.get("BYA_QKN_EPILOGUE", "1") != "0"
+        self.router_fold_keys = (os.environ.get("BYA_ROUTER_FOLD_KEYS", "1") != "0" and not self.fp8_weights
+                                 and self.mx_fmt is None)
+        self.face_fold_values = (os.environ.get("BYA_FACE_FOLD_VALUES", "1") != "0" and self.fused_attn_mix
+                                 and not self.fp8_weights and self.mx_fmt is None)
         self._inv_cache = {}
         self._side = None
         self._ws_key, self._ws = None, None
@@ -194,6 +198,7 @@
             self.r_nk_w, self.r_nk_b = r.norm_k.weight[perm].contiguous(), r.norm_k.bias[perm].contiguous()
             self.r_to_q = [l.weight[:, perm].contiguous() for l in r.to_q]
             self.r_to_k = [l.weight[:, perm].contiguous() for l in r.to_k]
+            self.r_to_q_t = [w.t().contiguous() for w in self.r_to_q] if self.router_fold_keys else None
             self.r_pos = r.pos_emb.reshape(-1, r.feat_dim).contiguous()
             self.r_qkv = []
             for st in r.spatial_temporal_layers:
@@ -447,7 +452,7 @@
         face = face_all.view(n_id, B, nq, -1).transpose(0, 1).contiguous()
         self.last_face_emb = face
 
-        kvs, krs = [], []
+        kvs, krs, kts, vws = [], [], [], []
         face2d = face.view(B * n_id * nq, -1)
         fn = E(*face2d.shape)
         for l, pc in enumerate(m.perceiver_cross_attention):
@@ -461,9 +466,19 @@
             ops.gemm(kn.view(B * n_id, nq, -1), self.r_to_k[l], kr_l.view(B * n_id, nq, -1))
             kvs.append(kv_l.view(B, n_id, nq, -1))
             krs.append(kr_l.view(B, n_id, nq, -1))
+            kt_l = None
+            if self.router_fold_keys:
+                kt_l = ops.router_fold_keys(kr_l, self.r_to_q_t[l], E(B * n_id * nq * 16, inner_p)).view(B, n_id * nq * 16, inner_p)
+            kts.append(kt_l)
+            vw_l = None
+            if self.face_fold_values and nq == 32 and inner_p == 16 * 128:
+                vw_l = E(B, pc.to_out.weight.shape[0], 16 * n_id * nq)
+                for b in range(B):
+                    ops.face_fold_values(kv_l.view(B, n_id * nq, -1)[b, :, inner_p:], pc.to_out.weight, vw_l[b])
+            vws.append(vw_l)
             if after_layer is not None:
                 after_layer(l)
-        return kvs, krs
+        return kvs, krs, kts, vws
 
     def _audio_invariants(self, audio_embeds, T, B, n_id):
         with ops.weight_streaming():
@@ -617,8 +632,8 @@
                     audio_now()
             if use_face:
                 flat_face = list(id_cond[:n_id]) + [t for i in range(n_id) for t in id_vit_hidden[i]]
-                face_kv, router_k = self._cached("face", flat_face,
-                                                 lambda: self._face_invariants(id_cond, id_vit_hidden, B, n_id, after_face_layer))
+                face_kv, router_k, router_kt, face_vw = self._cached(
+                    "face", flat_face, lambda: self._face_invariants(id_cond, id_vit_hidden, B, n_id, after_face_layer))
             audio_now()
             if use_audio:
                 audio_k, audio_v = audio_res[0]
@@ -786,11 +801,19 @@
                                   v_strides=(n_id * ntok * 2 * inner_p, ntok * 2 * inner_p, 2 * inner_p),
                                   o_strides=(n_id * N_loc * inner_p, N_loc * inner_p, inner_p), scale=hd_p ** -0.5)
                 if forced is None:
-                    r_logits = self._router(qp, router_k[ca], ca, B, T, per_frame, n_id, sh, taps, perceiver_attention)
+                    r_logits = self._router(qp, router_k[ca], ca, B, T, per_frame, n_id, sh, taps, perceiver_attention,
+                                            router_kt[ca] if taps is None else None)
                 else:
                     perceiver_attention()
                     r_logits = forced
-                if fuse_face:
+                if fuse_face and face_vw[ca] is not None:
+                    pr = buf("pr_p", B, N_loc, 16 * n_id * ntok)
+                    for b in range(B):
+                        ops.attn_kv_mix_probs(qp[b], kv_l[b], r_logits[b if r_logits.shape[0] > 1 else 0], pr[b], head_dim=hd_p,
+                                              heads=16, n_id=n_id, Sq=N_loc, Skv=ntok, q_strides=(0, inner_p),
+                                              k_strides=(ntok * 2 * inner_p, 0, 2 * inner_p), scale=hd_p ** -0.5)
+                        ops.gemm(pr[b], face_vw[ca][b], xv[b], res=xv[b], alpha=m.local_face_scale)
+                elif fuse_face:
                     kvs_p = (ntok * 2 * inner_p, 0, 2 * inner_p)
 
                     def face_mix(z, mx):
@@ -950,23 +973,31 @@
             return ops.rowgemm512(a, rg[2], x, res=x)
         return ops.gemm(a, lin.weight, x, bias=lin.bias, res=x)
 
-    def _router(self, qp, kr, ca, B, T, per_frame, n_id, sh, taps, overlap):
+    def _router_scores(self, qn, kr, kt, ca, rs, pos, n_id, N_loc):
+        r = self.m.router
+        B, F = qn.shape[0], r.feat_dim
+        if kt is not None:
+            for b in range(B):
+                ops.gemm(qn[b], kt[b], rs[b, 0], split=(F, N_loc * F))
+                ops.router_ln_pos(rs[b], r.norm.weight, r.norm.bias, pos, rs[b], n_id, N_loc, eps=r.norm.eps)
+            return rs
+        qr = ops.gemm(qn, self.r_to_q[ca], self._buf("r_qr", B, N_loc, qn.shape[-1]))
+        for b in range(B):
+            ops.router_scores(qr[b], kr[b].contiguous(), r.norm.weight, r.norm.bias, pos, rs[b], n_id, N_loc, eps=r.norm.eps)
+        return rs
+
+    def _router(self, qp, kr, ca, B, T, per_frame, n_id, sh, taps, overlap, kt=None):
         m, buf = self.m, self._buf
         r = m.router
         N, N_loc = T * per_frame, sh.N_loc
         F = r.feat_dim
         qk = qp.shape[-1]
         if sh.active and n_id * T >= sh.world and per_frame >= sh.world and not self.router_replicated:
-            return self._router_sharded(qp, kr, ca, T, per_frame, n_id, sh, taps, overlap)
+            return self._router_sharded(qp, kr, ca, T, per_frame, n_id, sh, taps, overlap, kt)
         overlap()
         qn = buf("r_qn", B, N_loc, qk)
         ops.layernorm(qp, qn, self.r_nq_w, self.r_nq_b, eps=r.norm_q.eps)
-        qr = ops.gemm(qn, self.r_to_q[ca], buf("r_qr", B, N_loc, qk))
-        rs = buf("r_s_loc", B, n_id, N_loc, F)
-        pos = self.r_pos[sh.v0:sh.v1]
-        for b in range(B):
-            ops.router_scores(qr[b], kr[b].contiguous(), r.norm.weight, r.norm.bias, pos, rs[b], n_id, N_loc,
-                              eps=r.norm.eps)
+        rs = self._router_scores(qn, kr, kt, ca, buf("r_s_loc", B, n_id, N_loc, F), self.r_pos[sh.v0:sh.v1], n_id, N_loc)
         if sh.active:
             rs = sh.gather_video_rows(rs, out=buf("r_s_full", B, n_id, N, F))
         R = B * n_id * N
@@ -996,7 +1027,7 @@
                 taps[f"router{ca}_b{b}"] = logits[b:b + 1].clone()
         return logits if not sh.active else logits[:, sh.v0:sh.v1].contiguous()
 
-    def _router_sharded(self, qp, kr, ca, T, per_frame, n_id, sh, taps, overlap):
+    def _router_sharded(self, qp, kr, ca, T, per_frame, n_id, sh, taps, overlap, kt=None):
         m, buf = self.m, self._buf
         r = m.router
         N, N_loc, F = T * per_frame, sh.N_loc, r.feat_dim
@@ -1005,10 +1036,7 @@
         qk = qp.shape[-1]
         qn = buf("r_qn", 1, N_loc, qk)
         ops.layernorm(qp, qn, self.r_nq_w, self.r_nq_b, eps=r.norm_q.eps)
-        qr = ops.gemm(qn, self.r_to_q[ca], buf("r_qr", 1, N_loc, qk))
-        rs_loc = buf("r_s_loc", 1, n_id, N_loc, F)
-        ops.router_scores(qr[0], kr[0].contiguous(), r.norm.weight, r.norm.bias, self.r_pos[sh.v0:sh.v1], rs_loc[0],
-                          n_id, N_loc, eps=r.norm.eps)
+        rs_loc = self._router_scores(qn, kr, kt, ca, buf("r_s_loc", 1, n_id, N_loc, F), self.r_pos[sh.v0:sh.v1], n_id, N_loc)
         if rp.p2p is not None:
             xa = rp.tokens_to_a(rs_loc[0], sh.v0, T)
         else:
diff --git a/bind_your_avatar_implementation_amd/ops.py b/bind_your_avatar_implementation_amd/ops.py
--- a/bind_your_avatar_implementation_amd/ops.py
+++ b/bind_your_avatar_implementation_amd/ops.py
@@ -1230,6 +1230,33 @@
     return z
 
 
+def attn_kv_mix_probs(q, k, r, pr, *, head_dim, heads, n_id, Sq, Skv, q_strides, k_strides, scale):
+    lib = _hip.load()
+    for t in (q, k, r, pr):
+        assert t.dtype == torch.bfloat16 and t.is_cuda
+    assert r.is_contiguous() and r.numel() == Sq * n_id
+    assert pr.is_contiguous() and tuple(pr.shape) == (Sq, heads * n_id * 32)
+    d = _mix_desc(head_dim, heads, n_id, 1, Sq, Skv, q_strides, k_strides, k_strides, (0, pr.shape[1]), scale)
+    tok = _begin("bya_attn_kv_mix", 2.0 * n_id * heads * Sq * Skv * head_dim)
+    check(lib.bya_attn_kv_mix_probs(_p(q), _p(k), _p(r), _p(pr), ctypes.byref(d), _stream()), "bya_attn_kv_mix_probs")
+    _end(tok)
+    return pr
+
+
+def face_fold_values(v, wo, vw):
+    lib = _hip.load()
+    for t in (v, wo, vw):
+        assert t.dtype == torch.bfloat16 and t.is_cuda and t.stride(-1) == 1
+    rows, qk = v.shape
+    n_out = wo.shape[0]
+    assert wo.is_contiguous() and wo.shape[1] == qk and tuple(vw.shape) == (n_out, 16 * rows)
+    tok = _begin("bya_face_fold_values", 2.0 * rows * qk * n_out)
+    check(lib.bya_face_fold_values(_p(v), _p(wo), _p(vw), rows, n_out, 16, qk // 16, v.stride(0), vw.stride(0), _stream()),
+          "bya_face_fold_values")
+    _end(tok)
+    return vw
+
+
 def attn_tiny(q, k, v, out, L, heads, n_outer, n_inner, outer_stride, seq_stride, ld_qkv, ld_o, scale):
     lib = _hip.load()
     tok = _begin("bya_attn_tiny")
@@ -1256,6 +1283,30 @@
     check(lib.bya_router_scores_plan(a(qr), a(kr), a(ln_w), a(ln_b), a(pos_emb), a(out), n_id, N, 16, 32, ctypes.byref(p)),
           "bya_router_scores_plan")
     return _step_plan(p, _hip.ROUTER_SCORES_KERNELS[p.kernel])
+
+
+def router_fold_keys(kr, wq_t, kt):
+    lib = _hip.load()
+    for t in (kr, wq_t, kt):
+        assert t.is_contiguous() and t.dtype == torch.bfloat16
+    rows, qk = kr.shape
+    assert tuple(wq_t.shape) == (qk, qk) and tuple(kt.shape) == (rows * 16, qk)
+    tok = _begin("bya_router_fold_keys", 2.0 * rows * qk * qk // 16)
+    check(lib.bya_router_fold_keys(_p(kr), _p(wq_t), _p(kt), rows, 16, qk // 16, _stream()), "bya_router_fold_keys")
+    _end(tok)
+    return kt
+
+
+def router_ln_pos(s, ln_w, ln_b, pos_emb, out, n_id, N, eps=1e-5):
+    lib = _hip.load()
+    for t in (s, ln_w, ln_b, pos_emb, out):
+        assert t.is_contiguous() and t.dtype == torch.bfloat16
+    assert s.numel() == out.numel() == n_id * N * 512 and pos_emb.numel() >= N * 512
+    tok = _begin("bya_router_scores")
+    check(lib.bya_router_ln_pos(_p(s), _p(ln_w), _p(ln_b), _p(pos_emb), _p(out), n_id, N, s.shape[-1], float(eps), _stream()),
+          "bya_router_ln_pos")
+    _end(tok)
+    return out
 
 
 def router_head(x, w, b, r, n_id, N):
diff --git a/include/bya.h b/include/bya.h
--- a/include/bya.h
+++ b/include/bya.h
@@ -293,6 +293,10 @@
     int32_t big_lds;
 } bya_attn_kv_mix_plan_info;
 int bya_attn_kv_mix_plan(const void* z, const void* af, const bya_attn_mix_desc* desc, bya_attn_kv_mix_plan_info* plan);
+int bya_attn_kv_mix_probs(const void* q, const void* k, const void* r, void* pr, const bya_attn_mix_desc* desc,
+                          hipStream_t stream);
+int bya_face_fold_values(const void* v, const void* wo, void* vw, int32_t rows, int32_t n_out, int32_t heads, int32_t head_dim,
+                         int64_t ldv, int64_t ldvw, hipStream_t stream);
 
 int bya_attn_kv_mix_mx(const void* q, const void* k, const void* v, const void* r, const void* af, void* codes, void* scales,
                        float* wsum, const bya_attn_mix_desc* desc, int32_t out_fmt, int64_t c_grp, int64_t c_row,
@@ -328,6 +332,11 @@
                            bya_step_plan_info* plan);
 int bya_router_head(const void* x, const void* w, const void* b, void* r, int32_t n_id, int64_t N, int32_t D,
                     hipStream_t stream);
+
+int bya_router_fold_keys(const void* kr, const void* wq_t, void* kt, int32_t rows, int32_t heads, int32_t head_dim,
+                         hipStream_t stream);
+int bya_router_ln_pos(const void* s, const void* ln_w, const void* ln_b, const void* pos_emb, void* out, int32_t n_id,
+                      int64_t N, int32_t feat, float eps, hipStream_t stream);
 
 int bya_forcing_max_over_frames(const void* forcing, void* out, int32_t frames, int64_t per_frame,
                                 int32_t n_id, hipStream_t stream);
```

After: 2.901 steps/s (median of 6 runs). No clear change (+1.0%).
